# nomic-ai/contrastors

Measured on AMD Instinct MI355X. Metric: query-doc pairs/sec (whole node), nomic-bert-2048 seq128 global-batch 16384, higher is better.
Workload: dtype bf16

## Files before the change

contrastors_amd/_C.py:

```python
from __future__ import annotations

import ctypes as C
import os
from pathlib import Path

_PKG = Path(__file__).resolve().parent
LIB_PATH = Path(os.environ.get("CONTRASTORS_HIP_LIB", _PKG / "lib" / "libcontrastors_hip.so"))

CX_OK = 0
_ERR = {-1: "CX_ERR_SHAPE", -2: "CX_ERR_ALIGN", -3: "CX_ERR_ARG", -4: "CX_ERR_LAUNCH"}

vp = C.c_void_p
i32 = C.c_int
i64 = C.c_long
f32 = C.c_float
u64 = C.c_ulonglong
u32 = C.c_uint


class CxLayerWeights(C.Structure):
    _fields_ = (
        [(n, vp) for n in ("Wqkv", "Wout", "Wfc1", "Wfc2", "WqkvT", "WoutT", "Wfc1T", "Wfc2T")]
        + [(n, vp) for n in ("bqkv", "bout", "bfc1", "bfc2")]
        + [(n, vp) for n in ("ln1_g", "ln1_b", "ln2_g", "ln2_b")]
        + [(n, vp) for n in ("gWqkv", "gWout", "gWfc1", "gWfc2")]
        + [(n, vp) for n in ("gbqkv", "gbout", "gbfc1", "gbfc2")]
        + [(n, vp) for n in ("gln1_g", "gln1_b", "gln2_g", "gln2_b")]
    )


class CxEncoderDesc(C.Structure):
    _fields_ = [
        ("n_layer", i32), ("d", i32), ("n_head", i32), ("d_inner", i32), ("gated", i32),
        ("vocab", i32), ("max_pos", i32), ("padding_idx", i32),
        ("ln_eps", f32), ("softmax_scale", f32),
        ("word_emb", vp), ("type_emb", vp), ("pos_emb", vp),
        ("emb_ln_g", vp), ("emb_ln_b", vp),
        ("gword_emb", vp), ("gtype_emb", vp), ("gpos_emb", vp), ("gemb_ln_g", vp), ("gemb_ln_b", vp),
        ("rot_cos", vp), ("rot_sin", vp),
        ("layers", C.POINTER(CxLayerWeights)),
        ("pool_mode", i32), ("normalize", i32),
        ("prenorm", i32),
        ("lnf_g", vp), ("lnf_b", vp), ("glnf_g", vp), ("glnf_b", vp),
        ("Wpatch", vp), ("bpatch", vp), ("cls_token", vp), ("vit_pos", vp),
        ("gWpatch", vp), ("gbpatch", vp), ("gcls_token", vp), ("gvit_pos", vp),
        ("patch_dim", i32),
        ("resid_pdrop", f32), ("embd_pdrop", f32), ("attn_pdrop", f32),
        ("mlp_act", i32), ("lnpre_g", vp), ("lnpre_b", vp), ("glnpre_g", vp), ("glnpre_b", vp),
    ]


class CxChunkBuffers(C.Structure):
    _fields_ = [("T_cap", i64)] + [
        (n, vp)
        for n in (
            "h0", "emb_mean", "emb_rstd", "qkv", "ctx", "lse", "z1", "h1", "mean1", "rstd1", "yg", "act", "z2",
            "h2", "mean2", "rstd2", "pool_norm", "g_a", "g_b", "g_c", "g_wide", "g_act", "tr_a", "tr_b", "delta",
            "ws_f32",
        )
    ] + [("ws_floats", i64)] + [(n, vp) for n in ("zf", "hf", "meanf", "rstdf", "patch_in", "patch_proj")] + [("checkpoint", i32), ("drop_active", i32), ("drop_seed", C.c_ulonglong), ("drop_offset", C.c_ulonglong), ("g_d", vp), ("layer_events", C.POINTER(vp)), ("zpre", vp), ("ckpt_keep", i32), ("patch_keep", vp), ("patch_inv", vp), ("n_keep", i32), ("n_patch_all", i32)]



class CxVitSubLN(C.Structure):
    _fields_ = [(n, vp) for n in ("norm_g", "norm_b", "gnorm_g", "gnorm_b")]


class CxVitExt(C.Structure):
    _fields_ = [("rope_cos", vp), ("rope_sin", vp), ("n_rope", i32), ("n_prefix", i32), ("no_final_ln", i32),
                ("subln_eps", f32), ("sub_ln", C.POINTER(CxVitSubLN)), ("z", vp), ("zmean", vp), ("zrstd", vp),
                ("yg_wide", vp)]


_SIGS = {
    "cx_abi_version": (i32, []),
    "cx_build_info": (C.c_char_p, []),
    "cx_error_string": (C.c_char_p, [i32]),
    "cx_gemm_bf16_nt": (i32, [vp, vp, vp, vp, i32, i32, i32, i32, i32, i32, i32, i32, f32, vp]),
    "cx_gemm_bf16_nt_accum": (i32, [vp, vp, vp, vp, i64, i32, i32, i32, i32, i32, vp]),
    "cx_gemm_bf16_tn_accum": (i32, [vp, vp, vp, vp, i64, i32, i32, i32, i32, i32, vp]),
    "cx_prof_gemm_config": (i32, [i32, i32]),
    "cx_prof_gemm_collect": (i32, [C.POINTER(C.c_double), C.POINTER(C.c_double), C.POINTER(i64), C.POINTER(i64)]),
    "cx_calib_mfma_bf16": (i32, [vp, i32, i32, vp, vp, vp]),
    "cx_calib_copy": (i32, [vp, vp, i64, vp]),
    "cx_transpose_bf16": (i32, [vp, vp, i32, i32, i32, i32, i32, vp]),
    "cx_cast_f32_to_bf16": (i32, [vp, vp, i64, vp]),
    "cx_cast_transpose_f32_to_bf16": (i32, [vp, vp, i32, i32, vp]),
    "cx_cast_transpose_f32_to_bf16_batched": (i32, [vp, i32, i32, vp]),
    "cx_cast_bf16_to_f32": (i32, [vp, vp, i64, vp]),
    "cx_layernorm_fwd": (i32, [vp, vp, vp, vp, vp, vp, vp, vp, i32, i32, f32, vp]),
    "cx_layernorm_bwd": (i32, [vp, vp, vp, vp, vp, vp, vp, vp, vp, vp, vp, i64, i32, i32, vp]),
    "cx_layernorm_bwd_pooled": (i32, [vp, vp, vp, vp, i32, i32, i32, vp, vp, vp, vp, vp, vp, vp, vp, vp, i64, i32, i32, vp]),
    "cx_layernorm_bwd_colsum": (i32, [vp, vp, vp, vp, vp, vp, vp, vp, vp, vp, vp, vp, i64, i32, i32, vp]),
    "cx_dropout_add_layernorm_fwd": (i32, [vp, vp, vp, vp, vp, vp, vp, vp, i32, i32, f32, f32, C.c_ulonglong, C.c_ulonglong,
                                           C.c_uint, vp]),
    "cx_dropout_add_layernorm_bwd": (i32, [vp, vp, vp, vp, vp, vp, vp, vp, vp, vp, vp, i64, i32, i32, f32, C.c_ulonglong,
                                           C.c_ulonglong, C.c_uint, vp]),
    "cx_dropout_add_layernorm_bwd_colsum": (i32, [vp, vp, vp, vp, vp, vp, vp, vp, vp, vp, vp, vp, i64, i32, i32, f32, C.c_ulonglong,
                                                  C.c_ulonglong, C.c_uint, vp]),
    "cx_dropout_scale": (i32, [vp, i64, f32, C.c_ulonglong, C.c_ulonglong, C.c_uint, vp]),
    "cx_layernorm_fwd_mixed": (i32, [vp, vp, vp, vp, vp, vp, vp, vp, i32, i32, f32, i32, vp]),
    "cx_layernorm_bwd_mixed": (i32, [vp, vp, vp, vp, vp, vp, vp, vp, vp, vp, i32, i32, i32, vp]),
    "cx_embed_ln_fwd": (i32, [vp, vp, vp, vp, vp, vp, vp, vp, vp, vp, i32, i32, i32, f32, vp]),
    "cx_embed_ln_bwd": (i32, [vp] * 15 + [i32, i32, i32, i32, vp]),
    "cx_embed_ln_bwd_sorted": (i32, [vp] * 15 + [i32, i32, i32, i32, i32, vp, vp, vp, vp]),
    "cx_swiglu_fwd": (i32, [vp, vp, i32, i32, i32, vp]),
    "cx_swiglu_bwd": (i32, [vp, vp, vp, i32, i32, i32, vp]),
    "cx_gemm_bf16_swiglu": (i32, [vp, vp, vp, vp, i32, i32, i32, i32, i32, i32, i32, vp]),
    "cx_gemm_bf16_nt_residual": (i32, [vp, vp, vp, vp, vp, i32, i32, i32, i32, i32, i32, i32, vp]),
    "cx_gemm_bf16_swiglu_bwd": (i32, [vp, vp, vp, vp, i32, i32, i32, i32, i32, i32, vp]),
    "cx_gemm_bf16_nt_splitk": (i32, [vp, vp, vp, vp, vp, vp, i64, i32, i32, i32, i32, i32, i32, i32, vp]),
    "cx_gemm_bf16_swiglu_gate": (i32, [vp, vp, vp, vp, i32, i32, i32, i32, i32, i32, i32, vp]),
    "cx_gemm_bf16_swiglu_bwd_gate": (i32, [vp, vp, vp, vp, vp, i32, i32, i32, i32, i32, i32, i32, vp]),
    "cx_swiglu_bwd_gate": (i32, [vp, vp, vp, vp, i32, i32, vp]),
    "cx_gemm_bf16_bias_gelu": (i32, [vp, vp, vp, vp, vp, i32, i32, i32, i32, i32, i32, i32, vp]),
    "cx_gemm_bf16_bias_act": (i32, [vp, vp, vp, vp, vp, i32, i32, i32, i32, i32, i32, i32, i32, vp]),
    "cx_bias_gelu_fwd": (i32, [vp, vp, vp, i32, i32, vp]),
    "cx_bias_gelu_bwd": (i32, [vp, vp, vp, vp, i32, i32, vp]),
    "cx_bias_grad": (i32, [vp, vp, i32, i32, i32, vp]),
    "cx_bias_gelu_bwd_colsum": (i32, [vp, vp, vp, vp, vp, i32, i32, vp]),
    "cx_bias_act_fwd": (i32, [vp, vp, vp, i32, i32, i32, vp]),
    "cx_bias_act_bwd_colsum": (i32, [vp, vp, vp, vp, vp, i32, i32, i32, vp]),
    "cx_gemm_bf16_act_bwd": (i32, [vp, vp, vp, vp, vp, vp, i64, i32, i32, i32, i32, i32, i32, i32, i32, vp]),
    "cx_attn_varlen_fwd": (i32, [vp, vp, vp, vp, vp, vp, i32, i32, i32, i32, f32, vp]),
    "cx_attn_varlen_bwd": (i32, [vp] * 9 + [i32, i32, i32, i32, f32, vp]),
    "cx_attn_varlen_bwd_prerotated": (i32, [vp] * 9 + [i32, i32, i32, i32, f32, vp]),
    "cx_attn_varlen_dropout_fwd": (i32, [vp] * 6 + [i32, i32, i32, i32, f32, f32, u64, u64, u32, vp]),
    "cx_attn_varlen_dropout_bwd": (i32, [vp] * 9 + [i32, i32, i32, i32, f32, f32, u64, u64, u32, vp]),
    "cx_ipc_alloc": (i32, [C.POINTER(vp), i64, i32]),
    "cx_ipc_free": (i32, [vp]),
    "cx_ipc_export": (i32, [vp, vp]),
    "cx_ipc_open": (i32, [vp, C.POINTER(vp)]),
    "cx_ipc_close": (i32, [vp]),
    "cx_xgmi_push": (i32, [vp, vp, i64, i64, i32, vp]),
    "cx_xgmi_scatter": (i32, [vp, vp, i32, i64, i32, vp]),
    "cx_xgmi_signal_wait": (i32, [vp, vp, i32, i32, u32, i64, vp, vp]),
    "cx_sum_slots_f32": (i32, [vp, vp, i64, i32, vp]),
    "cx_attn_varlen_kvpacked_fwd": (i32, [vp] * 6 + [i32, i32, i32, i32, i32, f32, vp]),
    "cx_attn_varlen_kvpacked_bwd": (i32, [vp] * 10 + [i32, i32, i32, i32, i32, f32, vp]),
    "cx_rotary_qkv_inplace": (i32, [vp, vp, vp, vp, i32, i32, i32, i32, i32, vp]),
    "cx_rotary_apply": (i32, [vp, i64, vp, vp, vp, i32, i32, i32, i32, i32, vp]),
    "cx_pool_normalize_fwd": (i32, [vp, vp, vp, vp, i32, i32, i32, i32, vp]),
    "cx_pool_normalize_bwd": (i32, [vp, vp, vp, vp, vp, i32, i32, i32, i32, vp]),
    "cx_vit_patchify": (i32, [vp, i32, vp, i32, i32, i32, i32, i32, vp]),
    "cx_vit_assemble_fwd": (i32, [vp, vp, vp, vp, i32, i32, i32, vp]),
    "cx_vit_assemble_bwd": (i32, [vp, vp, vp, vp, i32, i32, i32, vp]),
    "cx_vit_patchify_gather": (i32, [vp, i32, vp, i32, i32, i32, i32, i32, vp, i32, vp]),
    "cx_vit_assemble_fwd_gather": (i32, [vp, vp, vp, vp, i32, i32, i32, vp, vp]),
    "cx_vit_assemble_bwd_gather": (i32, [vp, vp, vp, vp, i32, i32, i32, vp, i32, vp]),
    "cx_vit_forward": (i32, [C.POINTER(CxEncoderDesc), C.POINTER(CxChunkBuffers), vp, i32, vp, i32, i32, i32, i32, i32,
                             i32, vp, vp]),
    "cx_vit_backward": (i32, [C.POINTER(CxEncoderDesc), C.POINTER(CxChunkBuffers), vp, i32, i32, vp, vp, vp]),
    "cx_vit_forward_hidden": (i32, [C.POINTER(CxEncoderDesc), C.POINTER(CxChunkBuffers), vp, i32, vp, i32, i32, i32, i32, i32,
                                    i32, vp, vp]),
    "cx_vit_backward_hidden": (i32, [C.POINTER(CxEncoderDesc), C.POINTER(CxChunkBuffers), vp, i32, i32, vp, vp]),
    "cx_rope2d_qkv_inplace": (i32, [vp, vp, vp, vp, i32, i32, i32, i32, i32, i32, vp]),
    "cx_swiglu_subln_fwd": (i32, [vp, vp, vp, vp, vp, vp, vp, vp, i32, i32, f32, vp]),
    "cx_swiglu_subln_bwd": (i32, [vp] * 11 + [i64, i32, i32, vp]),
    "cx_vit_forward_ex": (i32, [C.POINTER(CxEncoderDesc), C.POINTER(CxChunkBuffers), C.POINTER(CxVitExt), vp, i32, vp, i32, i32,
                                i32, i32, i32, i32, vp, vp]),
    "cx_vit_backward_ex": (i32, [C.POINTER(CxEncoderDesc), C.POINTER(CxChunkBuffers), C.POINTER(CxVitExt), vp, i32, i32, vp, vp,
                                 vp]),
    "cx_vit_forward_hidden_ex": (i32, [C.POINTER(CxEncoderDesc), C.POINTER(CxChunkBuffers), C.POINTER(CxVitExt), vp, i32, vp, i32,
                                       i32, i32, i32, i32, i32, vp, vp]),
    "cx_vit_backward_hidden_ex": (i32, [C.POINTER(CxEncoderDesc), C.POINTER(CxChunkBuffers), C.POINTER(CxVitExt), vp, i32, i32,
                                        vp, vp]),
    "cx_xent_fwd": (i32, [vp, i32, vp, vp, vp, i32, i32, i64, f32, i64, vp]),
    "cx_xent_bwd": (i32, [vp, vp, i32, vp, vp, vp, i32, i32, i64, i64, f32, i64, vp]),
    "cx_grad_sq_norm": (i32, [vp, i64, vp, vp]),
    "cx_adamw_clip_step": (i32, [vp, vp, vp, vp, i64, f32, f32, f32, f32, f32, i64, vp, f32, vp]),
    "cx_ema_update": (i32, [vp, vp, i64, f32, vp]),
    "cx_infonce_ws_floats": (i64, [i32, i32]),
    "cx_infonce_fwd": (i32, [vp, vp, vp, f32, vp, vp, vp, i32, i32, i32, i32, i32, vp]),
    "cx_infonce_argmax_ws_floats": (i64, [i32, i32]),
    "cx_infonce_fwd_argmax": (i32, [vp, vp, vp, f32, vp, vp, vp, vp, i32, i32, i32, i32, i32, vp]),
    "cx_infonce_bwd": (i32, [vp, vp, vp, vp, f32, f32, vp, vp, vp, vp, vp, vp, vp, i32, i32, i32, i32, i32, vp]),
    "cx_search_ws_bytes": (i64, [i32, i64, i32, i32]),
    "cx_search_topk": (i32, [vp, vp, i32, i64, i32, i64, i64, i32, vp, vp, vp, i32, vp, vp, vp, vp]),
    "cx_infonce_fp8_ws_floats": (i64, [i32, i32]),
    "cx_infonce_fp8_fwd": (i32, [vp, vp, vp, f32, vp, vp, vp, vp, vp, vp, vp, i32, i32, i32, i32, i32, vp]),
    "cx_infonce_fp8_bwd": (i32, [vp, vp, vp, vp, f32, f32, vp, vp, vp, vp, vp, vp, vp, vp, vp, i64, vp, vp, vp, i32, i32, i32,
                                 i32, i32, vp]),
    "cx_sgemm_nt": (i32, [vp, vp, vp, i32, i32, i32, i32, i32, i32, vp]),
    "cx_transpose_f32": (i32, [vp, vp, i32, i32, i32, i32, vp]),
    "cx_encoder_forward": (i32, [C.POINTER(CxEncoderDesc), C.POINTER(CxChunkBuffers), vp, vp, vp, i32, i32, i32,
                                 i32, i32, vp, vp]),
    "cx_encoder_forward_hidden": (i32, [C.POINTER(CxEncoderDesc), C.POINTER(CxChunkBuffers), vp, vp, vp, i32, i32, i32,
                                        i32, i32, vp, vp]),
    "cx_encoder_backward_hidden": (i32, [C.POINTER(CxEncoderDesc), C.POINTER(CxChunkBuffers), vp, vp, vp, i32, i32, i32,
                                         i32, vp, vp, vp, vp]),
    "cx_encoder_backward": (i32, [C.POINTER(CxEncoderDesc), C.POINTER(CxChunkBuffers), vp, vp, vp, i32, i32, i32,
                                  i32, vp, vp, vp, vp, vp]),
}

_DEV_SIGS = {
    "cx_gemm_set_variant": (None, [i32]),
    "cx_gemm_get_variant": (i32, []),
    "cx_gemm_set_debug": (None, [i32]),
    "cx_gemm_set_trace": (None, [vp]),
    "cx_gemm_v6_ablate": (None, [i32]),
    "cx_gemm_v6_trace": (None, [vp]),
    "cx_gemm_v7_mode": (None, [i32]),
    "cx_gemm_v7_trace": (None, [vp]),
    "cx_gemm_v7_occupancy": (i32, []),
    "cx_gemm_v7_ablate": (None, [i32]),
    "cx_gemm_v7_flags": (None, [i32]),
    "cx_gemm_v7_period": (None, [i32]),
    "cx_gemm_set_glds": (None, [i32]),
    "cx_gemm_get_glds": (i32, []),
    "cx_attn_set_bwd_s128": (None, [i32]),
    "cx_attn_set_prio": (None, [i32]),
    "cx_attn_set_fwd_s128": (None, [i32]),
    "cx_attn_set_fwd_long": (None, [i32]),
    "cx_attn_set_bwd_long": (None, [i32]),
    "cx_probe_mfma_layout": (i32, [vp, vp]),
    "cx_probe_ds_read_tr16": (i32, [vp, vp, vp]),
    "cx_probe_mfma_rate": (i32, [vp, i32, i32, i32, vp, vp, vp]),
    "cx_attn_dropout_keep_mask": (i32, [vp, i32, i32, i32, f32, u64, u64, u32, vp]),
    "cx_probe_rmw": (i32, [vp, i64, i32, i32, i32, vp]),
    "cx_probe_mfma_rate16": (i32, [vp, i32, i32, i32, vp, vp, vp]),
    "cx_probe_dma_bw": (i32, [vp, i64, i64, i64, i32, i32, i32, i32, vp, vp]),
}

EXPORTED_SYMBOLS = tuple(_SIGS)
DEV_EXPORTED_SYMBOLS = tuple(_DEV_SIGS)
DEV_LIB_PATH = Path(os.environ.get("CONTRASTORS_HIP_DEV_LIB", _PKG / "lib" / "libcontrastors_hip_dev.so"))

_lib = None
_dev_lib = None


def lib() -> C.CDLL:
    global _lib
    if _lib is None:
        if not LIB_PATH.exists():
            raise ImportError(
                f"{LIB_PATH} not found: build it with `python -m contrastors_amd.build` "
                "(hipcc --offload-arch=gfx950).  There is no CPU fallback."
            )
        import torch

        h = C.CDLL(str(LIB_PATH))
        for name, (res, args) in _SIGS.items():
            fn = getattr(h, name)
            fn.restype = res
            fn.argtypes = args
        _lib = h
    return _lib


def dev_lib() -> C.CDLL:
    global _dev_lib
    if _dev_lib is None:
        if not DEV_LIB_PATH.exists():
            raise ImportError(f"{DEV_LIB_PATH} not found: build it with `python -m contrastors_amd.build`")
        import torch

        h = C.CDLL(str(DEV_LIB_PATH))
        for name, (res, args) in {**_SIGS, **_DEV_SIGS}.items():
            fn = getattr(h, name)
            fn.restype = res
            fn.argtypes = args
# ... 18 lines not shown
```

contrastors_amd/csrc/engine.hip:

```cpp
#include <hip/hip_runtime.h>
#include "../../include/contrastors_hip.h"

namespace {

#define CX_TRY(expr)              \
    do {                          \
        int rc__ = (expr);        \
        if (rc__ != CX_OK) return rc__; \
    } while (0)

inline long round_up(long v, long m) { return (v + m - 1) / m * m; }

inline int mark_grads_done(const CxChunkBuffers* buf, int idx, void* stream) {
    if (!buf->layer_events || !buf->layer_events[idx]) return CX_OK;
    return hipEventRecord((hipEvent_t)buf->layer_events[idx], (hipStream_t)stream) == hipSuccess ? CX_OK : CX_ERR_LAUNCH;
}

struct Slots {
    const CxChunkBuffers* b;
    const CxEncoderDesc* e;
    long T_cap;
    int d, I, wfc1;
    int mode;
    int first_kept;
    bool kept(int s) const { return mode == 1 || (mode == 2 && s >= first_kept); }
    int sl(int s) const { return mode == 1 ? s : (mode == 2 && s >= first_kept) ? 1 + s - first_kept : 0; }
    int sl_in(int s) const { return mode == 0 ? 0 : s; }
    uint16_t* qkv(int s) const { return b->qkv + (size_t)sl(s) * T_cap * 3 * d; }
    uint16_t* ctx(int s) const { return b->ctx + (size_t)sl(s) * T_cap * d; }
    float* lse(int s) const { return b->lse + (size_t)sl(s) * T_cap * e->n_head; }
    uint16_t* z1(int s) const { return b->z1 + (size_t)(e->prenorm ? sl_in(s) : sl(s)) * T_cap * d; }
    uint16_t* h1(int s) const { return b->h1 + (size_t)sl(s) * T_cap * d; }
    float* mean1(int s) const { return b->mean1 + (size_t)sl(s) * T_cap; }
    float* rstd1(int s) const { return b->rstd1 + (size_t)sl(s) * T_cap; }
    uint16_t* yg(int s) const { return b->yg + (size_t)sl(s) * T_cap * I; }
    uint16_t* act(int s) const { return b->act + (size_t)sl(s) * T_cap * I; }
    uint16_t* z2(int s) const { return b->z2 + (size_t)sl(s) * T_cap * d; }
    uint16_t* h2(int s) const { return b->h2 + (size_t)(e->prenorm ? sl(s) : sl_in(s)) * T_cap * d; }
    float* mean2(int s) const { return b->mean2 + (size_t)sl(s) * T_cap; }
    float* rstd2(int s) const { return b->rstd2 + (size_t)sl(s) * T_cap; }
    uint16_t* ez(const CxVitExt* x, int s) const { return x->z + (size_t)sl(s) * T_cap * I; }
    float* ezmean(const CxVitExt* x, int s) const { return x->zmean + (size_t)sl(s) * T_cap; }
    float* ezrstd(const CxVitExt* x, int s) const { return x->zrstd + (size_t)sl(s) * T_cap; }
};

inline bool ext_rope(const CxVitExt* x) { return x && x->rope_cos; }
inline bool ext_subln(const CxVitExt* x) { return x && x->sub_ln; }
inline bool ext_no_lnf(const CxVitExt* x) { return x && x->no_final_ln; }
int check_ext(const CxVitExt* x, const CxEncoderDesc* e, const CxChunkBuffers* b) {
    if (!x) return CX_OK;
    if (x->rope_cos && (!x->rope_sin || x->n_rope <= 0 || x->n_prefix < 0)) return CX_ERR_ARG;
    if (x->sub_ln) {
        if (!e->gated || !x->z || !x->zmean || !x->zrstd || (!x->yg_wide && !b->g_wide)) return CX_ERR_ARG;
        for (int l = 0; l < e->n_layer; ++l)
            if (!x->sub_ln[l].norm_g || !x->sub_ln[l].norm_b) return CX_ERR_ARG;
    }
    return CX_OK;
}

Slots make_slots(const CxEncoderDesc* enc, const CxChunkBuffers* buf, int save) {
    const int L = enc->n_layer;
    int keep = buf->ckpt_keep < 0 ? 0 : buf->ckpt_keep > L ? L : buf->ckpt_keep;
    return Slots{buf, enc, buf->T_cap, enc->d, enc->d_inner, enc->gated ? 2 * enc->d_inner : enc->d_inner,
                 save ? (buf->checkpoint ? 2 : 1) : 0, L - keep};
}

int check_desc(const CxEncoderDesc* e, const CxChunkBuffers* b, int T) {
    if (!e || !b || !e->layers) return CX_ERR_ARG;
    if (e->n_layer <= 0 || e->d <= 0 || e->n_head <= 0) return CX_ERR_ARG;
    if (e->d != e->n_head * 64) return CX_ERR_SHAPE;
    if ((e->d % 64) != 0 || (e->d_inner % 64) != 0) return CX_ERR_SHAPE;
    if (b->T_cap < round_up(T, 64)) return CX_ERR_SHAPE;
    return CX_OK;
}

int wgrad_split(int out_f, int in_f, long Tp) {
    const long tiles = (long)((out_f + 127) / 128) * ((in_f + 127) / 128);
    const long nk = Tp / 64;
    long s = (512 + tiles - 1) / tiles;
    if (s > nk / 2) s = nk / 2;
    if (s < 1) s = 1;
    return (int)s;
}

int wgrad(const uint16_t* dY, int out_f, const uint16_t* X, int in_f, float* gW, const CxChunkBuffers* b, int T,
          void* stream) {
    if (!gW) return CX_OK;
    const int rc = cx_gemm_bf16_tn_accum(dY, X, gW, b->ws_f32, b->ws_floats, T, out_f, in_f, out_f, in_f, stream);
    if (rc != CX_ERR_SHAPE) return rc;
    if (!b->tr_a || !b->tr_b) return CX_ERR_ARG;
    const int Tp = (int)round_up(T, 64);
    CX_TRY(cx_transpose_bf16(dY, b->tr_a, T, out_f, out_f, Tp, Tp, stream));
    CX_TRY(cx_transpose_bf16(X, b->tr_b, T, in_f, in_f, Tp, Tp, stream));
    return cx_gemm_bf16_nt_accum(b->tr_a, b->tr_b, gW, b->ws_f32, b->ws_floats, out_f, in_f, Tp, Tp, Tp, stream);
}

int proj_residual(const uint16_t* x, const uint16_t* W, const float* bias, const uint16_t* residual, uint16_t* out, int T,
                  int N, int K, bool* folded, void* stream, const CxChunkBuffers* buf = nullptr) {
    *folded = false;
    if (buf && buf->ws_f32 && (long)((T + 255) / 256) * ((N + 255) / 256) <= 64 && K >= 1536) {
        const int rc = cx_gemm_bf16_nt_splitk(x, W, out, bias, residual, buf->ws_f32, buf->ws_floats, T, N, K, K, K, N, N, stream);
        if (rc != CX_ERR_SHAPE) {
            *folded = residual != nullptr && rc == CX_OK;
            return rc;
        }
    }
    if (residual) {
        const int rc = cx_gemm_bf16_nt_residual(x, W, out, bias, residual, T, N, K, K, K, N, N, stream);
        if (rc != CX_ERR_SHAPE) {
            *folded = rc == CX_OK;
            return rc;
        }
    }
    return cx_gemm_bf16_nt(x, W, out, bias, T, N, K, K, K, N, 0, 1, 1.f, stream);
}

bool gelu_fused_shape(int T, int N, int K) {
    return T > 0 && (K % 64) == 0 && (N % 8) == 0;
}

struct BlockRunner {
    const CxEncoderDesc* enc;
    const CxChunkBuffers* buf;
    const Slots& s;
    const int32_t* cu_seqlens;
    int Bc, T, max_seqlen;
    void* stream;
    const CxVitExt* ext = nullptr;

    int mlp_up(const CxLayerWeights& w, const uint16_t* x, int l, bool keep) const {
        const int d = enc->d, I = enc->d_inner;
        if (ext_subln(ext)) {
            uint16_t* yg = ext->yg_wide ? ext->yg_wide : buf->g_wide;
            CX_TRY(cx_gemm_bf16_nt(x, w.Wfc1, yg, w.bfc1, T, 2 * I, d, d, d, 2 * I, 0, 1, 1.f, stream));
            const CxVitSubLN& n = ext->sub_ln[l];
            return cx_swiglu_subln_fwd(yg, n.norm_g, n.norm_b, keep ? s.yg(l) : nullptr, s.act(l), s.ez(ext, l), s.ezmean(ext, l),
                                       s.ezrstd(ext, l), T, I, ext->subln_eps, stream);
        }
        if (enc->gated) {
            return cx_gemm_bf16_swiglu_gate(x, w.Wfc1, keep ? s.yg(l) : nullptr, s.act(l), T, I, d, d, d, I, I, stream);
        }
        const int rc = cx_gemm_bf16_bias_act(x, w.Wfc1, w.bfc1, keep ? s.yg(l) : nullptr, s.act(l), T, s.wfc1, d, d, d, s.wfc1,
                                             I, enc->mlp_act, stream);
        if (rc != CX_ERR_SHAPE) return rc;
        CX_TRY(cx_gemm_bf16_nt(x, w.Wfc1, s.yg(l), nullptr, T, s.wfc1, d, d, d, s.wfc1, 0, 1, 1.f, stream));
        return cx_bias_act_fwd(s.yg(l), w.bfc1, s.act(l), T, I, enc->mlp_act, stream);
    }
    int mlp(const CxLayerWeights& w, const uint16_t* x, int l, uint16_t* out, const uint16_t* residual, bool keep,
            bool* folded) const {
        CX_TRY(mlp_up(w, x, l, keep));
        return proj_residual(ext_subln(ext) ? s.ez(ext, l) : s.act(l), w.Wfc2, w.bfc2, residual, out, T, enc->d, enc->d_inner, folded, stream, buf);
    }
    int attn(const CxLayerWeights& w, const uint16_t* x, int l, uint16_t* out, const uint16_t* residual, bool* folded) const {
        const int d = enc->d;
        CX_TRY(cx_gemm_bf16_nt(x, w.Wqkv, s.qkv(l), w.bqkv, T, 3 * d, d, d, d, 3 * d, 0, 1, 1.f, stream));
        if (ext_rope(ext))
            CX_TRY(cx_rope2d_qkv_inplace(s.qkv(l), cu_seqlens, ext->rope_cos, ext->rope_sin, ext->n_rope, Bc, enc->n_head, T,
                                         ext->n_prefix, 1, stream));
        if (buf->drop_active && enc->attn_pdrop > 0.f) {
            CX_TRY(cx_attn_varlen_dropout_fwd(s.qkv(l), cu_seqlens, enc->rot_cos, enc->rot_sin, s.ctx(l), s.lse(l), Bc,
                                              enc->n_head, T, max_seqlen, enc->softmax_scale, enc->attn_pdrop, buf->drop_seed,
                                              buf->drop_offset, (unsigned)(2 * enc->n_layer + 1 + l), stream));
        } else if (enc->rot_cos && max_seqlen > 128) {
            CX_TRY(cx_rotary_qkv_inplace(s.qkv(l), cu_seqlens, enc->rot_cos, enc->rot_sin, Bc, enc->n_head, T, max_seqlen, 1,
                                         stream));
            CX_TRY(cx_attn_varlen_fwd(s.qkv(l), cu_seqlens, nullptr, nullptr, s.ctx(l), s.lse(l), Bc, enc->n_head, T, max_seqlen,
                                      enc->softmax_scale, stream));
        } else {
            CX_TRY(cx_attn_varlen_fwd(s.qkv(l), cu_seqlens, enc->rot_cos, enc->rot_sin, s.ctx(l), s.lse(l), Bc, enc->n_head, T,
                                      max_seqlen, enc->softmax_scale, stream));
        }
        return proj_residual(s.ctx(l), w.Wout, w.bout, residual, out, T, d, d, folded, stream);
    }
    int post_block(int l, const uint16_t* h_in, bool keep) const {
        const CxLayerWeights& w = enc->layers[l];
        const int d = enc->d;
        bool f1 = false, f2 = false;
        if (drop()) {
            const float p = enc->resid_pdrop;
            CX_TRY(attn(w, h_in, l, s.z1(l), nullptr, &f1));
            CX_TRY(cx_dropout_add_layernorm_fwd(s.z1(l), h_in, w.ln1_g, w.ln1_b, s.h1(l), keep ? s.z1(l) : nullptr, s.mean1(l),
                                                s.rstd1(l), T, d, enc->ln_eps, p, buf->drop_seed, buf->drop_offset, 2 * l, stream));
            CX_TRY(mlp(w, s.h1(l), l, s.z2(l), nullptr, keep, &f2));
            return cx_dropout_add_layernorm_fwd(s.z2(l), s.h1(l), w.ln2_g, w.ln2_b, s.h2(l), keep ? s.z2(l) : nullptr, s.mean2(l),
                                                s.rstd2(l), T, d, enc->ln_eps, p, buf->drop_seed, buf->drop_offset, 2 * l + 1,
                                                stream);
        }
        CX_TRY(attn(w, h_in, l, s.z1(l), h_in, &f1));
        CX_TRY(cx_layernorm_fwd(s.z1(l), f1 ? nullptr : h_in, w.ln1_g, w.ln1_b, s.h1(l), (keep && !f1) ? s.z1(l) : nullptr,
                                s.mean1(l), s.rstd1(l), T, d, enc->ln_eps, stream));
        CX_TRY(mlp(w, s.h1(l), l, s.z2(l), s.h1(l), keep, &f2));
        return cx_layernorm_fwd(s.z2(l), f2 ? nullptr : s.h1(l), w.ln2_g, w.ln2_b, s.h2(l), (keep && !f2) ? s.z2(l) : nullptr,
                                s.mean2(l), s.rstd2(l), T, d, enc->ln_eps, stream);
    }
    bool drop() const { return buf->drop_active && enc->resid_pdrop > 0.f; }
    int pre_block(int l, const uint16_t* x, const uint16_t* r, bool r_folded, bool keep, bool up_only, const uint16_t** x_out,
                  const uint16_t** r_out, bool* folded_out) const {
        const CxLayerWeights& w = enc->layers[l];
        const int d = enc->d, L = enc->n_layer;
        CX_TRY(cx_layernorm_fwd(x, r, w.ln1_g, w.ln1_b, s.h1(l), (r_folded && x == s.z1(l)) ? nullptr : s.z1(l), s.mean1(l),
                                s.rstd1(l), T, d, enc->ln_eps, stream));
        bool f1 = false, f2 = false;
        CX_TRY(attn(w, s.h1(l), l, s.z2(l), s.z1(l), &f1));
        CX_TRY(cx_layernorm_fwd(s.z2(l), f1 ? nullptr : s.z1(l), w.ln2_g, w.ln2_b, s.h2(l), f1 ? nullptr : s.z2(l), s.mean2(l),
                                s.rstd2(l), T, d, enc->ln_eps, stream));
        if (up_only) return mlp_up(w, s.h2(l), l, keep);
        uint16_t* nxt = (l + 1 < L) ? s.z1(l + 1) : buf->zf;
        CX_TRY(mlp(w, s.h2(l), l, nxt, s.z2(l), keep, &f2));
        *x_out = nxt;
        *r_out = f2 ? nullptr : s.z2(l);
        *folded_out = f2;
        return CX_OK;
    }
};

int blocks_forward(const CxEncoderDesc* enc, const CxChunkBuffers* buf, const Slots& s, const uint16_t* h0,
                   const int32_t* cu_seqlens, int Bc, int T, int max_seqlen, int save, const uint16_t** h_final,
                   void* stream, const CxVitExt* ext = nullptr) {
    const int d = enc->d, L = enc->n_layer;
    const BlockRunner run{enc, buf, s, cu_seqlens, Bc, T, max_seqlen, stream, ext};
    if (!enc->prenorm) {
        const uint16_t* h_in = h0;
        for (int l = 0; l < L; ++l) {
            CX_TRY(run.post_block(l, h_in, save != 0 && s.kept(l)));
            h_in = s.h2(l);
        }
        *h_final = h_in;
        return CX_OK;
    }
    if (!buf->zf || !buf->hf || !buf->meanf || !buf->rstdf || (!ext_no_lnf(ext) && (!enc->lnf_g || !enc->lnf_b))) return CX_ERR_ARG;
    if (buf->drop_active && enc->resid_pdrop > 0.f) return CX_ERR_ARG;
    const uint16_t* x = h0;
    const uint16_t* r = nullptr;
    bool r_folded = false;
    for (int l = 0; l < L; ++l) {
        CX_TRY(run.pre_block(l, x, r, r_folded, save != 0 && s.kept(l), false, &x, &r, &r_folded));
        if (save == 2 && !r_folded) return CX_ERR_SHAPE;
    }
    if (ext_no_lnf(ext)) {
        if (!r_folded || x != buf->zf) return CX_ERR_SHAPE;
        *h_final = buf->zf;
        return CX_OK;
    }
    CX_TRY(cx_layernorm_fwd(x, r, enc->lnf_g, enc->lnf_b, buf->hf, r_folded ? nullptr : buf->zf, buf->meanf, buf->rstdf, T,
                            d, enc->ln_eps, stream));
    *h_final = buf->hf;
    return CX_OK;
}

int check_bwd_buffers(const CxChunkBuffers* buf) {
    return (!buf->g_a || !buf->g_b || !buf->g_c || !buf->g_wide || !buf->g_act || !buf->delta ||
            !buf->ws_f32) ? CX_ERR_ARG : CX_OK;
}

int clear_pad_rows(const CxEncoderDesc* enc, const CxChunkBuffers* buf, const Slots& s, int T, void* stream,
                   const CxVitExt* ext = nullptr) {
    const int Tp = (int)round_up(T, 64);
    if (Tp == T) return CX_OK;
    const int d = enc->d, I = enc->d_inner, L = enc->n_layer;
    auto clear = [&](uint16_t* base, int width) {
        return hipMemsetAsync(base + (size_t)T * width, 0, (size_t)(Tp - T) * width * sizeof(uint16_t),
                              (hipStream_t)stream) == hipSuccess ? CX_OK : CX_ERR_LAUNCH;
    };
    CX_TRY(clear(buf->g_a, d));
    CX_TRY(clear(buf->g_b, d));
    CX_TRY(clear(buf->g_c, d));
    if (buf->g_d) CX_TRY(clear(buf->g_d, d));
    CX_TRY(clear(buf->g_wide, 3 * d));
    CX_TRY(clear(buf->g_wide, s.wfc1));
    CX_TRY(clear(buf->h0, d));
    for (int l = 0; l < L; ++l) {
        CX_TRY(clear(s.act(l), I));
        CX_TRY(clear(s.h1(l), d));
        CX_TRY(clear(s.ctx(l), d));
        CX_TRY(clear(s.h2(l), d));
        if (ext_subln(ext)) CX_TRY(clear(s.ez(ext, l), I));
    }
    return CX_OK;
}

struct PooledGrad {
    const float* demb;
    const float* emb;
    const float* norm;
    int pool_mode, normalize;
};

int blocks_backward(const CxEncoderDesc* enc, const CxChunkBuffers* buf, const Slots& s, const int32_t* cu_seqlens, int Bc,
                    int T, int max_seqlen, const PooledGrad* pg, const uint16_t** da_out, const uint16_t** db_out, void* stream,
                    const CxVitExt* ext = nullptr) {
    const int d = enc->d, I = enc->d_inner, H = enc->n_head, L = enc->n_layer;
    auto mlp_bwd = [&](const CxLayerWeights& w, int l, const uint16_t* dm, const uint16_t* mlp_in, const uint16_t* add,
                       bool* folded, bool bias_done) -> int {
        if (w.gbfc2 && !bias_done) CX_TRY(cx_bias_grad(dm, w.gbfc2, T, d, d, stream));
        if (ext_subln(ext)) {
            CX_TRY(wgrad(dm, d, s.ez(ext, l), I, w.gWfc2, buf, T, stream));
            CX_TRY(cx_gemm_bf16_nt(dm, w.Wfc2T, buf->g_act, nullptr, T, I, d, d, d, I, 0, 1, 1.f, stream));
            const CxVitSubLN& n = ext->sub_ln[l];
            CX_TRY(cx_swiglu_subln_bwd(buf->g_act, s.act(l), s.yg(l), s.ezmean(ext, l), s.ezrstd(ext, l), n.norm_g, buf->g_wide,
                                       n.gnorm_g, n.gnorm_b, w.gbfc1, buf->ws_f32, buf->ws_floats, T, I, stream));
            CX_TRY(wgrad(buf->g_wide, s.wfc1, mlp_in, d, w.gWfc1, buf, T, stream));
            return proj_residual(buf->g_wide, w.Wfc1T, nullptr, add, buf->g_b, T, d, s.wfc1, folded, stream, buf);
        }
        CX_TRY(wgrad(dm, d, s.act(l), I, w.gWfc2, buf, T, stream));
        int fused = CX_ERR_SHAPE;
        if (enc->gated)
            fused = cx_gemm_bf16_swiglu_bwd_gate(dm, w.Wfc2T, s.act(l), s.yg(l), buf->g_wide, T, I, d, d, d, I, s.wfc1, stream);
#ifndef CX_AB_R5_ROUTES
        if (!enc->gated && gelu_fused_shape(T, s.wfc1, d))
            fused = cx_gemm_bf16_act_bwd(dm, w.Wfc2T, s.yg(l), buf->g_wide, w.gbfc1, buf->ws_f32, buf->ws_floats, T, I, d, d, d, I, I,
                                         enc->mlp_act, stream);
#endif
        if (fused != CX_ERR_SHAPE) {
            CX_TRY(fused);
        } else {
            CX_TRY(cx_gemm_bf16_nt(dm, w.Wfc2T, buf->g_act, nullptr, T, I, d, d, d, I, 0, 1, 1.f, stream));
        }
        if (enc->gated) {
            if (fused == CX_ERR_SHAPE)
                CX_TRY(cx_swiglu_bwd_gate(buf->g_act, s.act(l), s.yg(l), buf->g_wide, T, I, stream));
        } else if (fused == CX_ERR_SHAPE) {
            CX_TRY(cx_bias_act_bwd_colsum(buf->g_act, s.yg(l), gelu_fused_shape(T, s.wfc1, d) ? nullptr : w.bfc1, buf->g_wide,
                                          w.gbfc1, T, I, enc->mlp_act, stream));
        }
        CX_TRY(wgrad(buf->g_wide, s.wfc1, mlp_in, d, w.gWfc1, buf, T, stream));
        return proj_residual(buf->g_wide, w.Wfc1T, nullptr, add, buf->g_b, T, d, s.wfc1, folded, stream, buf);
    };
    auto attn_bwd = [&](const CxLayerWeights& w, int l, const uint16_t* dx, const uint16_t* attn_in, const uint16_t* add,
                        bool* folded, bool bias_done) -> int {
        if (w.gbout && !bias_done) CX_TRY(cx_bias_grad(dx, w.gbout, T, d, d, stream));
        CX_TRY(wgrad(dx, d, s.ctx(l), d, w.gWout, buf, T, stream));
        CX_TRY(cx_gemm_bf16_nt(dx, w.WoutT, buf->g_b, nullptr, T, d, d, d, d, d, 0, 1, 1.f, stream));
        if (buf->drop_active && enc->attn_pdrop > 0.f) {
            CX_TRY(cx_attn_varlen_dropout_bwd(buf->g_b, s.qkv(l), s.ctx(l), s.lse(l), cu_seqlens, enc->rot_cos, enc->rot_sin,
                                              buf->delta, buf->g_wide, Bc, H, T, max_seqlen, enc->softmax_scale, enc->attn_pdrop,
                                              buf->drop_seed, buf->drop_offset, (unsigned)(2 * enc->n_layer + 1 + l), stream));
        } else if (enc->rot_cos && max_seqlen > 128) {
            CX_TRY(cx_attn_varlen_bwd_prerotated(buf->g_b, s.qkv(l), s.ctx(l), s.lse(l), cu_seqlens, enc->rot_cos, enc->rot_sin,
                                                 buf->delta, buf->g_wide, Bc, H, T, max_seqlen, enc->softmax_scale, stream));
        } else {
            CX_TRY(cx_attn_varlen_bwd(buf->g_b, s.qkv(l), s.ctx(l), s.lse(l), cu_seqlens, enc->rot_cos, enc->rot_sin,
                                      buf->delta, buf->g_wide, Bc, H, T, max_seqlen, enc->softmax_scale, stream));
        }
        if (ext_rope(ext))
            CX_TRY(cx_rope2d_qkv_inplace(buf->g_wide, cu_seqlens, ext->rope_cos, ext->rope_sin, ext->n_rope, Bc, H, T, ext->n_prefix,
                                         -1, stream));
        if (w.gbqkv) CX_TRY(cx_bias_grad(buf->g_wide, w.gbqkv, T, 3 * d, 3 * d, stream));
        CX_TRY(wgrad(buf->g_wide, 3 * d, attn_in, d, w.gWqkv, buf, T, stream));
        return proj_residual(buf->g_wide, w.WqkvT, nullptr, add, buf->g_b, T, d, 3 * d, folded, stream, buf);
    };
    auto ln_bwd = [&](const uint16_t* a, const uint16_t* b2, const uint16_t* z, const float* g, const float* mean,
                      const float* rstd, const uint16_t* dz_extra, uint16_t* dz, float* gg, float* gb, float* gbias,
                      bool* done) -> int {
        *done = false;
        if (gbias) {
            const int rc = cx_layernorm_bwd_colsum(a, b2, z, g, mean, rstd, dz_extra, dz, gg, gb, gbias, buf->ws_f32,
                                                   buf->ws_floats, T, d, stream);
            if (rc != CX_ERR_ARG) {
                *done = rc == CX_OK;
                return rc;
            }
        }
        return cx_layernorm_bwd(a, b2, z, g, mean, rstd, dz_extra, dz, gg, gb, buf->ws_f32, buf->ws_floats, T, d, stream);
    };
    const BlockRunner run{enc, buf, s, cu_seqlens, Bc, T, max_seqlen, stream, ext};
    if (!enc->prenorm) {
        const uint16_t* da = buf->g_a;
        const uint16_t* db = nullptr;
        for (int l = L - 1; l >= 0; --l) {
            const CxLayerWeights& w = enc->layers[l];
            const uint16_t* h_in = (l == 0) ? buf->h0 : s.h2(l - 1);
            if (!s.kept(l)) CX_TRY(run.post_block(l, h_in, true));
            if (run.drop()) {
                if (!buf->g_d) return CX_ERR_ARG;
                const float p = enc->resid_pdrop;
                bool f1 = false, f2 = false;
#ifdef CX_AB_R5_ROUTES
                const bool cs = false;
#else
                const bool cs = buf->ws_f32 && buf->ws_floats >= 3L * d * 256;
#endif
                CX_TRY(cx_dropout_add_layernorm_bwd_colsum(da, db, s.z2(l), w.ln2_g, s.mean2(l), s.rstd2(l), buf->g_c, buf->g_d, w.gln2_g,
                                                           w.gln2_b, cs ? w.gbfc2 : nullptr, buf->ws_f32, buf->ws_floats, T, d, p,
                                                           buf->drop_seed, buf->drop_offset, 2 * l + 1, stream));
                CX_TRY(mlp_bwd(w, l, buf->g_d, s.h1(l), buf->g_c, &f1, cs));
                CX_TRY(cx_dropout_add_layernorm_bwd_colsum(f1 ? buf->g_b : buf->g_c, f1 ? nullptr : buf->g_b, s.z1(l), w.ln1_g, s.mean1(l),
                                                           s.rstd1(l), buf->g_a, buf->g_d, w.gln1_g, w.gln1_b, cs ? w.gbout : nullptr,
                                                           buf->ws_f32, buf->ws_floats, T, d, p, buf->drop_seed, buf->drop_offset, 2 * l,
                                                           stream));
// ... 350 lines not shown
```

contrastors_amd/csrc/gemm_api.hip:

```cpp
#include "cx_common.h"
#include "../../include/contrastors_hip.h"
#include "gemm_params.h"
#include <mutex>

namespace {

constexpr int BK = 64;

__global__ __launch_bounds__(256) void splitk_reduce_kernel(const float* __restrict__ part, float* __restrict__ out, long n4,
                                                            long slab, int splits) {
    const long stride = (long)gridDim.x * blockDim.x;
    for (long i = (long)blockIdx.x * blockDim.x + threadIdx.x; i < n4; i += stride) {
        float4 a = reinterpret_cast<const float4*>(out)[i];
        for (int s = 0; s < splits; ++s) {
            const float4 v = reinterpret_cast<const float4*>(part + s * slab)[i];
            a.x += v.x; a.y += v.y; a.z += v.z; a.w += v.w;
        }
        reinterpret_cast<float4*>(out)[i] = a;
    }
}

int reduce_slabs(const float* ws, float* out, long slab, int split, hipStream_t s) {
    const long n4 = slab / 4;
    long g = (n4 + 255) / 256;
// ... 13 lines not shown
        if (score > best_score + 1e-9) {
            best_score = score;
            best = s;
        }
    }
    return best;
}

struct GemmProf {
    std::mutex mu;
    bool enabled = false;
    int stride = 1;
    long launches = 0;
    static constexpr int CAP = 8192;
    hipEvent_t ev0[CAP], ev1[CAP];
    double flop[CAP];
    int created = 0, used = 0;
} g_prof;

struct ProfScope {
    int slot = -1;
    hipStream_t s;
    ProfScope(double flop, hipStream_t stream) : s(stream) {
        if (!g_prof.enabled) return;
        std::lock_guard<std::mutex> lk(g_prof.mu);
        if ((g_prof.launches % g_prof.stride) == 0 && g_prof.used < GemmProf::CAP) {
            const int sl = g_prof.used;
            if (sl >= g_prof.created) {
                if (hipEventCreate(&g_prof.ev0[sl]) != hipSuccess || hipEventCreate(&g_prof.ev1[sl]) != hipSuccess) return;
                g_prof.created = sl + 1;
            }
            slot = g_prof.used++;
            g_prof.flop[slot] = flop;
            (void)hipEventRecord(g_prof.ev0[slot], s);
        }
        ++g_prof.launches;
    }
    ~ProfScope() {
        if (slot >= 0) (void)hipEventRecord(g_prof.ev1[slot], s);
    }
};

GemmParams base_params(const uint16_t* X, const uint16_t* W, void* Out, const float* bias, int M, int N, int K, int ldx,
                       int ldw, int ldo) {
    GemmParams p = {};
    p.X = X; p.W = W; p.Out = Out; p.bias = bias;
    p.M = M; p.N = N; p.K = K; p.ldx = ldx; p.ldw = ldw; p.ldo = ldo;
    p.split_k = 1; p.alpha = 1.f;
    return p;
}

}

extern "C" {

int cx_gemm_bf16_nt(const uint16_t* X, const uint16_t* W, void* Out, const float* bias, int M, int N, int K, int ldx,
                    int ldw, int ldo, int out_mode, int split_k, float alpha, void* stream) {
    if (M <= 0 || N <= 0) return CX_OK;
    if (K <= 0 || (K % BK) != 0 || (N % 4) != 0) return CX_ERR_SHAPE;
    if ((ldx % 8) != 0 || (ldw % 8) != 0 || (ldo % 4) != 0) return CX_ERR_ALIGN;
    if (out_mode < 0 || out_mode > 1) return CX_ERR_ARG;
    (void)split_k;
    GemmParams p = base_params(X, W, Out, bias, M, N, K, ldx, ldw, ldo);
    p.alpha = alpha;
    ProfScope prof(2.0 * (double)M * (double)N * (double)K, (hipStream_t)stream);
    hipError_t e;
    if (out_mode == 0 && (N % 8) == 0 && (ldo % 8) == 0)
        e = cx_launch_gemm_v6(p, GEMM_EPI_NONE, (hipStream_t)stream);
    else
        e = cx_launch_gemm_v5(p, 0, out_mode == 0 ? GEMM_OUT_BF16 : GEMM_OUT_F32, GEMM_EPI_NONE, (hipStream_t)stream);
    return e == hipSuccess ? CX_OK : CX_ERR_LAUNCH;
}

int cx_gemm_bf16_nt_accum(const uint16_t* X, const uint16_t* W, float* Out, float* ws, long ws_floats, int M, int N, int K,
                          int ldx, int ldw, void* stream) {
    if (M <= 0 || N <= 0) return CX_OK;
    if (K <= 0 || (K % BK) != 0 || (N % 4) != 0) return CX_ERR_SHAPE;
    if ((ldx % 8) != 0 || (ldw % 8) != 0) return CX_ERR_ALIGN;
    if (!ws || !Out) return CX_ERR_ARG;
    const long slab = (long)M * N;
    if (ws_floats < slab) return CX_ERR_SHAPE;
    const long tiles = (long)((M + 255) / 256) * ((N + 255) / 256), nk = K / BK;
    long max_split = nk / 4;
    if (max_split > ws_floats / slab) max_split = ws_floats / slab;
    if (max_split > 16) max_split = 16;
    GemmParams p = base_params(X, W, ws, nullptr, M, N, K, ldx, ldw, N);
    p.split_k = (int)choose_split(tiles, max_split);
    if (p.split_k > nk) p.split_k = (int)nk;
    if (cx_launch_gemm_v5(p, 0, GEMM_OUT_F32_PARTIAL, GEMM_EPI_NONE, (hipStream_t)stream) != hipSuccess) return CX_ERR_LAUNCH;
    return reduce_slabs(ws, Out, slab, p.split_k, (hipStream_t)stream);
}

int cx_gemm_bf16_tn_accum(const uint16_t* dY, const uint16_t* A, float* G, float* ws, long ws_floats, int T, int O, int I,
                          int ld_dy, int ld_a, void* stream) {
    if (T <= 0 || O <= 0 || I <= 0) return CX_OK;
    if ((O % 256) != 0 || (I % 256) != 0) return CX_ERR_SHAPE;
    if ((ld_dy % 8) != 0 || (ld_a % 8) != 0) return CX_ERR_ALIGN;
    if (!ws || !G) return CX_ERR_ARG;
    const long slab = (long)O * I;
    if (ws_floats < slab) return CX_ERR_SHAPE;
    const int Tp = (T + BK - 1) / BK * BK;
    GemmParams p = base_params(dY, A, ws, nullptr, O, I, Tp, ld_dy, ld_a, I);
    const long tiles = (long)(O / 256) * (I / 256), nk = Tp / BK;
    long max_split = nk / 4;
    if (max_split > ws_floats / slab) max_split = ws_floats / slab;
    if (max_split > 32) max_split = 32;
    p.split_k = (int)choose_split(tiles, max_split);
    {
        ProfScope prof(2.0 * (double)T * (double)O * (double)I, (hipStream_t)stream);
        if (cx_launch_gemm_v6_tn(p, (hipStream_t)stream) != hipSuccess) return CX_ERR_LAUNCH;
    }
    return reduce_slabs(ws, G, slab, p.split_k, (hipStream_t)stream);
}

int cx_gemm_bf16_swiglu(const uint16_t* X, const uint16_t* W, uint16_t* YG, uint16_t* Act, int M, int I, int K, int ldx,
                        int ldw, int ld_yg, int ld_act, void* stream) {
    if (M <= 0 || I <= 0) return CX_OK;
    if (K <= 0 || (K % BK) != 0 || (I % 32) != 0) return CX_ERR_SHAPE;
    if ((ldx % 8) != 0 || (ldw % 8) != 0 || (ld_yg % 4) != 0 || (ld_act % 4) != 0) return CX_ERR_ALIGN;
    if (!Act) return CX_ERR_ARG;
    GemmParams p = base_params(X, W, YG, nullptr, M, 2 * I, K, ldx, ldw, ld_yg);
    p.Out2 = Act; p.ldo2 = ld_act;
    ProfScope prof(2.0 * (double)M * (double)(2 * I) * (double)K, (hipStream_t)stream);
    const hipError_t e = ((ld_yg % 8) == 0 && (ld_act % 8) == 0)
                             ? cx_launch_gemm_v6(p, GEMM_EPI_SWIGLU, (hipStream_t)stream)
                             : cx_launch_gemm_v5(p, 0, GEMM_OUT_BF16, GEMM_EPI_SWIGLU, (hipStream_t)stream);
    return e == hipSuccess ? CX_OK : CX_ERR_LAUNCH;
}

int cx_gemm_bf16_swiglu_gate(const uint16_t* X, const uint16_t* W, uint16_t* G, uint16_t* Act, int M, int I, int K, int ldx,
                             int ldw, int ld_g, int ld_act, void* stream) {
    if (M <= 0 || I <= 0) return CX_OK;
    if (K <= 0 || (K % BK) != 0 || (I % 32) != 0 || (ld_g % 8) != 0 || (ld_act % 8) != 0) return CX_ERR_SHAPE;
    if ((ldx % 8) != 0 || (ldw % 8) != 0) return CX_ERR_ALIGN;
    if (!Act) return CX_ERR_ARG;
    GemmParams p = base_params(X, W, G, nullptr, M, 2 * I, K, ldx, ldw, ld_g);
    p.Out2 = Act; p.ldo2 = ld_act;
    ProfScope prof(2.0 * (double)M * (double)(2 * I) * (double)K, (hipStream_t)stream);
    return cx_launch_gemm_v6(p, GEMM_EPI_SWIGLU_G, (hipStream_t)stream) == hipSuccess ? CX_OK : CX_ERR_LAUNCH;
}

int cx_gemm_bf16_nt_residual(const uint16_t* X, const uint16_t* W, uint16_t* Out, const float* bias, const uint16_t* Residual,
                             int M, int N, int K, int ldx, int ldw, int ldo, int ldr, void* stream) {
    if (M <= 0 || N <= 0) return CX_OK;
    if (!Residual || !Out) return CX_ERR_ARG;
    if (K <= 0 || (K % 64) != 0 || (N % 8) != 0 || (ldo % 8) != 0 || (ldr % 8) != 0) return CX_ERR_SHAPE;
    if ((ldx % 8) != 0 || (ldw % 8) != 0) return CX_ERR_ALIGN;
    GemmParams p = base_params(X, W, Out, bias, M, N, K, ldx, ldw, ldo);
    p.Out2 = const_cast<uint16_t*>(Residual); p.ldo2 = ldr;
    ProfScope prof(2.0 * (double)M * (double)N * (double)K, (hipStream_t)stream);
    return cx_launch_gemm_v6(p, GEMM_EPI_NONE, (hipStream_t)stream) == hipSuccess ? CX_OK : CX_ERR_LAUNCH;
}

int cx_gemm_bf16_bias_gelu(const uint16_t* X, const uint16_t* W, const float* bias, uint16_t* Pre, uint16_t* Act, int M, int N,
                           int K, int ldx, int ldw, int ld_pre, int ld_act, void* stream) {
    return cx_gemm_bf16_bias_act(X, W, bias, Pre, Act, M, N, K, ldx, ldw, ld_pre, ld_act, 0, stream);
}

int cx_gemm_bf16_bias_act(const uint16_t* X, const uint16_t* W, const float* bias, uint16_t* Pre, uint16_t* Act, int M, int N,
                          int K, int ldx, int ldw, int ld_pre, int ld_act, int act, void* stream) {
    if (M <= 0 || N <= 0) return CX_OK;
    if (!Act || (act != 0 && act != 1)) return CX_ERR_ARG;
    if (K <= 0 || (K % 64) != 0 || (N % 8) != 0 || (ld_act % 8) != 0 || (Pre && (ld_pre % 8) != 0)) return CX_ERR_SHAPE;
    if ((ldx % 8) != 0 || (ldw % 8) != 0) return CX_ERR_ALIGN;
    GemmParams p = base_params(X, W, Pre, bias, M, N, K, ldx, ldw, ld_pre);
    p.Out2 = Act; p.ldo2 = ld_act;
    p.act = act;
    ProfScope prof(2.0 * (double)M * (double)N * (double)K, (hipStream_t)stream);
    return cx_launch_gemm_v6(p, act == 1 ? GEMM_EPI_QGELU : GEMM_EPI_GELU, (hipStream_t)stream) == hipSuccess ? CX_OK : CX_ERR_LAUNCH;
}

int cx_gemm_bf16_swiglu_bwd(const uint16_t* dY, const uint16_t* W, const uint16_t* YG, uint16_t* dYG, int M, int I, int K,
                            int ldx, int ldw, int ld_yg, void* stream) {
    if (M <= 0 || I <= 0) return CX_OK;
    if (!dY || !W || !YG || !dYG) return CX_ERR_ARG;
    if (K <= 0 || (K % 64) != 0 || (I % 256) != 0 || (ld_yg % 8) != 0 || ld_yg < 2 * I) return CX_ERR_SHAPE;
    if ((ldx % 8) != 0 || (ldw % 8) != 0) return CX_ERR_ALIGN;
    GemmParams p = base_params(dY, W, dYG, nullptr, M, I, K, ldx, ldw, ld_yg);
    p.Out2 = const_cast<uint16_t*>(YG); p.ldo2 = ld_yg;
    ProfScope prof(2.0 * (double)M * (double)I * (double)K, (hipStream_t)stream);
    return cx_launch_gemm_v6(p, GEMM_EPI_SWIGLU_BWD, (hipStream_t)stream) == hipSuccess ? CX_OK : CX_ERR_LAUNCH;
}

int cx_gemm_bf16_swiglu_bwd_gate(const uint16_t* dY, const uint16_t* W, const uint16_t* Act, const uint16_t* G, uint16_t* dYG,
                                 int M, int I, int K, int ldx, int ldw, int ld_ag, int ld_dyg, void* stream) {
    if (M <= 0 || I <= 0) return CX_OK;
    if (!dY || !W || !Act || !G || !dYG) return CX_ERR_ARG;
    if (K <= 0 || (K % 64) != 0 || (I % 256) != 0 || (ld_dyg % 8) != 0 || ld_dyg < 2 * I || (ld_ag % 8) != 0 || ld_ag < I)
        return CX_ERR_SHAPE;
    if ((ldx % 8) != 0 || (ldw % 8) != 0) return CX_ERR_ALIGN;
    GemmParams p = base_params(dY, W, dYG, nullptr, M, I, K, ldx, ldw, ld_dyg);
    p.Out2 = const_cast<uint16_t*>(Act); p.ldo2 = ld_ag;
    p.In3 = G;
    ProfScope prof(2.0 * (double)M * (double)I * (double)K, (hipStream_t)stream);
    return cx_launch_gemm_v6(p, GEMM_EPI_SWIGLU_BWD_AG, (hipStream_t)stream) == hipSuccess ? CX_OK : CX_ERR_LAUNCH;
}

int cx_gemm_bf16_act_bwd(const uint16_t* dY, const uint16_t* W, const uint16_t* Pre, uint16_t* dPre, float* dbias, float* ws,
                         long ws_floats, int M, int N, int K, int ldx, int ldw, int ld_pre, int ld_dpre, int act, void* stream) {
    if (M <= 0 || N <= 0) return CX_OK;
    if (!dY || !W || !Pre || !dPre || (act != 0 && act != 1)) return CX_ERR_ARG;
    if (K <= 0 || (K % 64) != 0 || (N % 8) != 0 || (ld_pre % 8) != 0 || (ld_dpre % 8) != 0) return CX_ERR_SHAPE;
    if ((ldx % 8) != 0 || (ldw % 8) != 0) return CX_ERR_ALIGN;
    const int nblocks = (M + 127) / 128;
    if (dbias && (!ws || ws_floats < (long)nblocks * N)) return CX_ERR_SHAPE;
    GemmParams p = base_params(dY, W, dPre, nullptr, M, N, K, ldx, ldw, ld_dpre);
    p.Out2 = const_cast<uint16_t*>(Pre); p.ldo2 = ld_pre;
    p.act = act;
    p.colsum_part = dbias ? ws : nullptr;
    {
        ProfScope prof(2.0 * (double)M * (double)N * (double)K, (hipStream_t)stream);
        if (cx_launch_gemm_v6(p, GEMM_EPI_ACT_BWD, (hipStream_t)stream) != hipSuccess) return CX_ERR_LAUNCH;
    }
    if (dbias && cx_launch_colsum_part_reduce(ws, dbias, nblocks, N, (hipStream_t)stream) != hipSuccess) return CX_ERR_LAUNCH;
    return CX_OK;
}

int cx_prof_gemm_config(int enable, int stride) {
    std::lock_guard<std::mutex> lk(g_prof.mu);
    g_prof.enabled = enable != 0;
    g_prof.stride = stride > 0 ? stride : 1;
    g_prof.launches = 0;
    g_prof.used = 0;
    return CX_OK;
}

int cx_prof_gemm_collect(double* total_ms, double* total_flop, long* launches_timed, long* launches_total) {
    std::lock_guard<std::mutex> lk(g_prof.mu);
    double ms = 0.0, fl = 0.0;
    for (int i = 0; i < g_prof.used; ++i) {
        if (hipEventSynchronize(g_prof.ev1[i]) != hipSuccess) return CX_ERR_LAUNCH;
        float t = 0.f;
        if (hipEventElapsedTime(&t, g_prof.ev0[i], g_prof.ev1[i]) != hipSuccess) return CX_ERR_LAUNCH;
        ms += t;
        fl += g_prof.flop[i];
    }
    if (total_ms) *total_ms = ms;
    if (total_flop) *total_flop = fl;
    if (launches_timed) *launches_timed = g_prof.used;
    if (launches_total) *launches_total = g_prof.launches;
    return CX_OK;
}

}

#include "gemm_splitk_small.inc"
```

contrastors_amd/csrc/gemm_bf16.hip:

```cpp
#include "cx_common.h"
#include "../../include/contrastors_hip.h"
#include "gemm_params.h"

namespace {

constexpr int BM = 128, BN = 128, BK = 64;
constexpr int TILE_BYTES = 128 * BK * 2;

typedef __attribute__((address_space(3))) void* lds_void_ptr;
typedef const __attribute__((address_space(1))) void* glb_void_ptr;

enum OutMode { OUT_BF16 = GEMM_OUT_BF16, OUT_F32 = GEMM_OUT_F32, OUT_F32_ATOMIC = GEMM_OUT_F32_ATOMIC };

struct StageRegs { uint4 r0, r1, r2, r3; };

CX_DEVICE uint4 stage_load(const bf16_t* __restrict__ base, int ld, int row0, int nrows, int k0, int tid, int p) {
    const int r = p * 32 + (tid >> 3);
    int gr = row0 + r;
    gr = gr < nrows ? gr : nrows - 1;
    return *reinterpret_cast<const uint4*>(base + (size_t)gr * ld + k0 + (tid & 7) * 8);
}

template <bool GLDS>
CX_DEVICE void stage_tile(const bf16_t* __restrict__ base, int ld, int row0, int nrows, int k0, char* lds_tile,
// ... 613 lines not shown
                if (hipEventCreate(&g_prof.ev0[slot]) != hipSuccess || hipEventCreate(&g_prof.ev1[slot]) != hipSuccess)
                    return CX_ERR_LAUNCH;
                g_prof.created = slot + 1;
            }
            g_prof.flop[slot] = 2.0 * (double)M * (double)N * (double)K;
            (void)hipEventRecord(g_prof.ev0[slot], (hipStream_t)stream);
        }
        ++g_prof.launches;
    }
    hipError_t e = v5 ? cx_launch_gemm_v5(p, 0, out_mode, GEMM_EPI_NONE, (hipStream_t)stream)
                   : v2 ? launch_v2(p, out_mode, (hipStream_t)stream)
                      : (g_use_glds ? launch_mode<true>(p, out_mode, (hipStream_t)stream)
                                    : launch_mode<false>(p, out_mode, (hipStream_t)stream));
    if (slot >= 0) (void)hipEventRecord(g_prof.ev1[slot], (hipStream_t)stream);
    return e == hipSuccess ? CX_OK : CX_ERR_LAUNCH;
}

int cx_gemm_bf16_nt_accum(const uint16_t* X, const uint16_t* W, float* Out, float* ws, long ws_floats, int M, int N,
                          int K, int ldx, int ldw, void* stream) {
    if (M <= 0 || N <= 0) return CX_OK;
    if (K <= 0 || (K % BK) != 0 || (N % 4) != 0) return CX_ERR_SHAPE;
    if (!ws || !Out) return CX_ERR_ARG;
    const long slab = (long)M * N;
    if (ws_floats < slab) return CX_ERR_SHAPE;
    const bool v5 = (g_variant >= 3) && g_use_glds;
    const bool v2 = (g_variant == 2) && g_use_glds;
    const long tiles = v5 ? (long)((M + 255) / 256) * ((N + 255) / 256)
                     : v2 ? (long)((M + V2_BM - 1) / V2_BM) * ((N + V2_BN - 1) / V2_BN)
                          : (long)((M + BM - 1) / BM) * ((N + BN - 1) / BN);
    const long nk = K / BK;
    long max_split = nk / 4;
    if (max_split > ws_floats / slab) max_split = ws_floats / slab;
    if (max_split > 16) max_split = 16;
    long split = choose_split(tiles, max_split, (v2 || v5) ? 256 : 512);
    int rc;
    if (v5) {
        GemmParams p;
        p.X = X; p.W = W; p.Out = ws; p.bias = nullptr;
        p.M = M; p.N = N; p.K = K; p.ldx = ldx; p.ldw = ldw; p.ldo = N;
        p.tiles_m = p.tiles_n = 0; p.split_k = (int)split; p.alpha = 1.f; p.dbg = g_dbg; p.Out2 = nullptr; p.ldo2 = 0; p.sup_m = p.sup_n = 0;
        split = p.split_k;
        const hipError_t he = cx_launch_gemm_v5(p, 0, GEMM_OUT_F32_PARTIAL, GEMM_EPI_NONE, (hipStream_t)stream);
        rc = he == hipSuccess ? CX_OK : CX_ERR_LAUNCH;
    } else if (v2) {
        GemmParams p;
        p.X = X; p.W = W; p.Out = ws; p.bias = nullptr;
        p.M = M; p.N = N; p.K = K; p.ldx = ldx; p.ldw = ldw; p.ldo = N;
        p.tiles_m = (M + V2_BM - 1) / V2_BM; p.tiles_n = (N + V2_BN - 1) / V2_BN;
        p.split_k = (int)split; p.alpha = 1.f; p.dbg = g_dbg; p.Out2 = nullptr; p.ldo2 = 0; p.sup_m = p.sup_n = 0;
        rc = launch_v2(p, OUT_F32_PARTIAL, (hipStream_t)stream) == hipSuccess ? CX_OK : CX_ERR_LAUNCH;
    } else {
        rc = CX_OK;
        for (long s = 0; s < split && rc == CX_OK; ++s) {
            const long k0 = nk * s / split * BK, k1 = nk * (s + 1) / split * BK;
            rc = cx_gemm_bf16_nt(X + k0, W + k0, ws + s * slab, nullptr, M, N, (int)(k1 - k0), ldx, ldw, N, OUT_F32, 1,
                                 1.f, stream);
        }
    }
    if (rc != CX_OK) return rc;
    const long n4 = slab / 4;
    long g = (n4 + 255) / 256;
    if (g > 2048) g = 2048;
    hipLaunchKernelGGL(splitk_reduce_kernel, dim3((int)g), dim3(256), 0, (hipStream_t)stream, ws, Out, n4, slab,
                       (int)split);
    return hipGetLastError() == hipSuccess ? CX_OK : CX_ERR_LAUNCH;
}

int cx_gemm_bf16_tn_accum(const uint16_t* dY, const uint16_t* A, float* G, float* ws, long ws_floats, int T, int O, int I,
                          int ld_dy, int ld_a, void* stream) {
    if (T <= 0 || O <= 0 || I <= 0) return CX_OK;
    if ((O % V2_BM) != 0 || (I % V2_BN) != 0) return CX_ERR_SHAPE;
    const bool use_v5 = (g_variant == 5) && (I % 256) == 0;
    if ((ld_dy % 8) != 0 || (ld_a % 8) != 0) return CX_ERR_ALIGN;
    if (!ws || !G) return CX_ERR_ARG;
    const long slab = (long)O * I;
    if (ws_floats < slab) return CX_ERR_SHAPE;
    const int Tp = (T + BK - 1) / BK * BK;
    GemmParams p;
    p.X = dY; p.W = A; p.Out = ws; p.bias = nullptr;
    p.M = O; p.N = I; p.K = Tp; p.ldx = ld_dy; p.ldw = ld_a; p.ldo = I;
    p.tiles_m = O / V2_BM; p.tiles_n = use_v5 ? I / 256 : I / V2_BN;
    const long tiles = (long)p.tiles_m * p.tiles_n, nk = Tp / BK;
    long max_split = nk / 4;
    if (max_split > ws_floats / slab) max_split = ws_floats / slab;
    if (max_split > 32) max_split = 32;
    const long split = choose_split(tiles, max_split);
    p.split_k = (int)split; p.alpha = 1.f; p.dbg = g_dbg; p.Out2 = nullptr; p.ldo2 = 0; p.sup_m = p.sup_n = 0;
    static bool attr_set = false;
    if (!attr_set) {
        if (hipFuncSetAttribute(reinterpret_cast<const void*>(&gemm_bf16_tn_kernel),
                                hipFuncAttributeMaxDynamicSharedMemorySize, V2_NSTAGE * V2_STAGE) != hipSuccess)
            return CX_ERR_LAUNCH;
        attr_set = true;
    }
    int slot = -1;
    if (g_prof.enabled) {
        if ((g_prof.launches % g_prof.stride) == 0 && g_prof.used < GemmProf::CAP) {
            slot = g_prof.used++;
            if (slot >= g_prof.created) {
                if (hipEventCreate(&g_prof.ev0[slot]) != hipSuccess || hipEventCreate(&g_prof.ev1[slot]) != hipSuccess)
                    return CX_ERR_LAUNCH;
                g_prof.created = slot + 1;
            }
            g_prof.flop[slot] = 2.0 * (double)T * (double)O * (double)I;
            (void)hipEventRecord(g_prof.ev0[slot], (hipStream_t)stream);
        }
        ++g_prof.launches;
    }
    if (use_v5) {
        if (cx_launch_gemm_v5(p, 1, GEMM_OUT_F32_PARTIAL, GEMM_EPI_NONE, (hipStream_t)stream) != hipSuccess) return CX_ERR_LAUNCH;
    } else {
        hipLaunchKernelGGL(gemm_bf16_tn_kernel, dim3((int)(tiles * split)), dim3(512), V2_NSTAGE * V2_STAGE,
                           (hipStream_t)stream, p);
    }
    if (slot >= 0) (void)hipEventRecord(g_prof.ev1[slot], (hipStream_t)stream);
    if (hipGetLastError() != hipSuccess) return CX_ERR_LAUNCH;
    const long n4 = slab / 4;
    long g = (n4 + 255) / 256;
    if (g > 2048) g = 2048;
    hipLaunchKernelGGL(splitk_reduce_kernel, dim3((int)g), dim3(256), 0, (hipStream_t)stream, ws, G, n4, slab, (int)split);
    return hipGetLastError() == hipSuccess ? CX_OK : CX_ERR_LAUNCH;
}

int cx_gemm_bf16_swiglu(const uint16_t* X, const uint16_t* W, uint16_t* YG, uint16_t* Act, int M, int I, int K, int ldx,
                        int ldw, int ld_yg, int ld_act, void* stream) {
    if (M <= 0 || I <= 0) return CX_OK;
    if (K <= 0 || (K % BK) != 0 || (I % 32) != 0) return CX_ERR_SHAPE;
    if ((ldx % 8) != 0 || (ldw % 8) != 0 || (ld_yg % 4) != 0 || (ld_act % 4) != 0) return CX_ERR_ALIGN;
    if (!Act) return CX_ERR_ARG;
    GemmParams p;
    p.X = X; p.W = W; p.Out = YG; p.bias = nullptr;
    p.M = M; p.N = 2 * I; p.K = K; p.ldx = ldx; p.ldw = ldw; p.ldo = ld_yg;
    p.tiles_m = p.tiles_n = 0; p.split_k = 1; p.alpha = 1.f; p.dbg = g_dbg;
    p.Out2 = Act; p.ldo2 = ld_act; p.sup_m = p.sup_n = 0;
    int slot = -1;
    if (g_prof.enabled) {
        if ((g_prof.launches % g_prof.stride) == 0 && g_prof.used < GemmProf::CAP) {
            slot = g_prof.used++;
            if (slot >= g_prof.created) {
                if (hipEventCreate(&g_prof.ev0[slot]) != hipSuccess || hipEventCreate(&g_prof.ev1[slot]) != hipSuccess)
                    return CX_ERR_LAUNCH;
                g_prof.created = slot + 1;
            }
            g_prof.flop[slot] = 2.0 * (double)M * (double)(2 * I) * (double)K;
            (void)hipEventRecord(g_prof.ev0[slot], (hipStream_t)stream);
        }
        ++g_prof.launches;
    }
    hipError_t e = cx_launch_gemm_v5(p, 0, GEMM_OUT_BF16, GEMM_EPI_SWIGLU, (hipStream_t)stream);
    if (slot >= 0) (void)hipEventRecord(g_prof.ev1[slot], (hipStream_t)stream);
    return e == hipSuccess ? CX_OK : CX_ERR_LAUNCH;
}

int cx_gemm_bf16_nt_residual(const uint16_t* X, const uint16_t* W, uint16_t* Out, const float* bias,
                             const uint16_t* Residual, int M, int N, int K, int ldx, int ldw, int ldo, int ldr,
                             void* stream) {
    if (M <= 0 || N <= 0) return CX_OK;
    if (!Residual || !Out) return CX_ERR_ARG;
    if (K <= 0 || (K % 64) != 0 || (N % 8) != 0 || (ldo % 8) != 0 || (ldr % 8) != 0) return CX_ERR_SHAPE;
    if ((ldx % 8) != 0 || (ldw % 8) != 0) return CX_ERR_ALIGN;
    if (cx_gemm_get_variant() != 6) return CX_ERR_SHAPE;
    GemmParams p;
    p.X = X; p.W = W; p.Out = Out; p.bias = bias;
    p.M = M; p.N = N; p.K = K; p.ldx = ldx; p.ldw = ldw; p.ldo = ldo;
    p.tiles_m = p.tiles_n = 0; p.split_k = 1; p.alpha = 1.f; p.dbg = g_dbg;
    p.Out2 = const_cast<uint16_t*>(Residual); p.ldo2 = ldr; p.sup_m = p.sup_n = 0; p.trace = nullptr;
    int slot = -1;
    if (g_prof.enabled) {
        if ((g_prof.launches % g_prof.stride) == 0 && g_prof.used < GemmProf::CAP) {
            slot = g_prof.used++;
            if (slot >= g_prof.created) {
                if (hipEventCreate(&g_prof.ev0[slot]) != hipSuccess || hipEventCreate(&g_prof.ev1[slot]) != hipSuccess)
                    return CX_ERR_LAUNCH;
                g_prof.created = slot + 1;
            }
            g_prof.flop[slot] = 2.0 * (double)M * (double)N * (double)K;
            (void)hipEventRecord(g_prof.ev0[slot], (hipStream_t)stream);
        }
        ++g_prof.launches;
    }
    const hipError_t e = cx_launch_gemm_v6(p, GEMM_EPI_NONE, (hipStream_t)stream);
    if (slot >= 0) (void)hipEventRecord(g_prof.ev1[slot], (hipStream_t)stream);
    return e == hipSuccess ? CX_OK : CX_ERR_LAUNCH;
}

int cx_gemm_bf16_bias_gelu(const uint16_t* X, const uint16_t* W, const float* bias, uint16_t* Pre, uint16_t* Act, int M,
                           int N, int K, int ldx, int ldw, int ld_pre, int ld_act, void* stream) {
    return cx_gemm_bf16_bias_act(X, W, bias, Pre, Act, M, N, K, ldx, ldw, ld_pre, ld_act, 0, stream);
}

int cx_gemm_bf16_bias_act(const uint16_t* X, const uint16_t* W, const float* bias, uint16_t* Pre, uint16_t* Act, int M,
                          int N, int K, int ldx, int ldw, int ld_pre, int ld_act, int act, void* stream) {
    if (M <= 0 || N <= 0) return CX_OK;
    if (!Act || (act != 0 && act != 1)) return CX_ERR_ARG;
    if (K <= 0 || (K % 64) != 0 || (N % 8) != 0 || (ld_act % 8) != 0 || (Pre && (ld_pre % 8) != 0)) return CX_ERR_SHAPE;
    if ((ldx % 8) != 0 || (ldw % 8) != 0) return CX_ERR_ALIGN;
    if (cx_gemm_get_variant() != 6) return CX_ERR_SHAPE;
    GemmParams p;
    p.X = X; p.W = W; p.Out = Pre; p.bias = bias;
    p.M = M; p.N = N; p.K = K; p.ldx = ldx; p.ldw = ldw; p.ldo = ld_pre;
    p.tiles_m = p.tiles_n = 0; p.split_k = 1; p.alpha = 1.f; p.dbg = g_dbg;
    p.Out2 = Act; p.ldo2 = ld_act; p.sup_m = p.sup_n = 0; p.trace = nullptr;
    p.act = act;
    int slot = -1;
    if (g_prof.enabled) {
        if ((g_prof.launches % g_prof.stride) == 0 && g_prof.used < GemmProf::CAP) {
            slot = g_prof.used++;
            if (slot >= g_prof.created) {
                if (hipEventCreate(&g_prof.ev0[slot]) != hipSuccess || hipEventCreate(&g_prof.ev1[slot]) != hipSuccess)
                    return CX_ERR_LAUNCH;
                g_prof.created = slot + 1;
            }
            g_prof.flop[slot] = 2.0 * (double)M * (double)N * (double)K;
            (void)hipEventRecord(g_prof.ev0[slot], (hipStream_t)stream);
        }
        ++g_prof.launches;
    }
    const hipError_t e = cx_launch_gemm_v6(p, act == 1 ? GEMM_EPI_QGELU : GEMM_EPI_GELU, (hipStream_t)stream);
    if (slot >= 0) (void)hipEventRecord(g_prof.ev1[slot], (hipStream_t)stream);
    return e == hipSuccess ? CX_OK : CX_ERR_LAUNCH;
}

int cx_gemm_bf16_swiglu_bwd(const uint16_t* dY, const uint16_t* W, const uint16_t* YG, uint16_t* dYG, int M, int I, int K,
                            int ldx, int ldw, int ld_yg, void* stream) {
    if (M <= 0 || I <= 0) return CX_OK;
    if (!dY || !W || !YG || !dYG) return CX_ERR_ARG;
    if (K <= 0 || (K % 64) != 0 || (I % 256) != 0 || (ld_yg % 8) != 0 || ld_yg < 2 * I) return CX_ERR_SHAPE;
    if ((ldx % 8) != 0 || (ldw % 8) != 0) return CX_ERR_ALIGN;
    if (cx_gemm_get_variant() != 6) return CX_ERR_SHAPE;
    GemmParams p;
    p.X = dY; p.W = W; p.Out = dYG; p.bias = nullptr;
    p.M = M; p.N = I; p.K = K; p.ldx = ldx; p.ldw = ldw; p.ldo = ld_yg;
    p.tiles_m = p.tiles_n = 0; p.split_k = 1; p.alpha = 1.f; p.dbg = g_dbg;
    p.Out2 = const_cast<uint16_t*>(YG); p.ldo2 = ld_yg; p.sup_m = p.sup_n = 0; p.trace = nullptr;
    int slot = -1;
    if (g_prof.enabled) {
        if ((g_prof.launches % g_prof.stride) == 0 && g_prof.used < GemmProf::CAP) {
            slot = g_prof.used++;
            if (slot >= g_prof.created) {
                if (hipEventCreate(&g_prof.ev0[slot]) != hipSuccess || hipEventCreate(&g_prof.ev1[slot]) != hipSuccess)
                    return CX_ERR_LAUNCH;
                g_prof.created = slot + 1;
            }
            g_prof.flop[slot] = 2.0 * (double)M * (double)I * (double)K;
            (void)hipEventRecord(g_prof.ev0[slot], (hipStream_t)stream);
        }
        ++g_prof.launches;
    }
    const hipError_t e = cx_launch_gemm_v6(p, GEMM_EPI_SWIGLU_BWD, (hipStream_t)stream);
    if (slot >= 0) (void)hipEventRecord(g_prof.ev1[slot], (hipStream_t)stream);
    return e == hipSuccess ? CX_OK : CX_ERR_LAUNCH;
}

int cx_prof_gemm_config(int enable, int stride) {
    g_prof.enabled = enable != 0;
    g_prof.stride = stride > 0 ? stride : 1;
    g_prof.launches = 0;
    g_prof.used = 0;
    return CX_OK;
}

int cx_prof_gemm_collect(double* total_ms, double* total_flop, long* launches_timed, long* launches_total) {
    double ms = 0.0, fl = 0.0;
    for (int i = 0; i < g_prof.used; ++i) {
        if (hipEventSynchronize(g_prof.ev1[i]) != hipSuccess) return CX_ERR_LAUNCH;
        float t = 0.f;
        if (hipEventElapsedTime(&t, g_prof.ev0[i], g_prof.ev1[i]) != hipSuccess) return CX_ERR_LAUNCH;
        ms += t;
        fl += g_prof.flop[i];
    }
    if (total_ms) *total_ms = ms;
    if (total_flop) *total_flop = fl;
    if (launches_timed) *launches_timed = g_prof.used;
    if (launches_total) *launches_total = g_prof.launches;
    return CX_OK;
}

}

int cx_gemm_bf16_swiglu_gate(const uint16_t* X, const uint16_t* W, uint16_t* G, uint16_t* Act, int M, int I, int K, int ldx,
                             int ldw, int ld_g, int ld_act, void* stream) {
    if (M <= 0 || I <= 0) return CX_OK;
    if (K <= 0 || (K % BK) != 0 || (I % 32) != 0 || (ld_g % 8) != 0 || (ld_act % 8) != 0) return CX_ERR_SHAPE;
    if ((ldx % 8) != 0 || (ldw % 8) != 0) return CX_ERR_ALIGN;
    if (!Act) return CX_ERR_ARG;
    GemmParams p;
    p.X = X; p.W = W; p.Out = G; p.bias = nullptr;
    p.M = M; p.N = 2 * I; p.K = K; p.ldx = ldx; p.ldw = ldw; p.ldo = ld_g;
    p.tiles_m = p.tiles_n = 0; p.split_k = 1; p.alpha = 1.f; p.dbg = 0; p.act = 0;
    p.Out2 = Act; p.ldo2 = ld_act; p.In3 = nullptr; p.sup_m = p.sup_n = 0; p.trace = nullptr;
    return cx_launch_gemm_v6(p, GEMM_EPI_SWIGLU_G, (hipStream_t)stream) == hipSuccess ? CX_OK : CX_ERR_LAUNCH;
}

int cx_gemm_bf16_swiglu_bwd_gate(const uint16_t* dY, const uint16_t* W, const uint16_t* Act, const uint16_t* G, uint16_t* dYG,
                                 int M, int I, int K, int ldx, int ldw, int ld_ag, int ld_dyg, void* stream) {
    if (M <= 0 || I <= 0) return CX_OK;
    if (!dY || !W || !Act || !G || !dYG) return CX_ERR_ARG;
    if (K <= 0 || (K % 64) != 0 || (I % 256) != 0 || (ld_dyg % 8) != 0 || ld_dyg < 2 * I || (ld_ag % 8) != 0 || ld_ag < I)
        return CX_ERR_SHAPE;
    if ((ldx % 8) != 0 || (ldw % 8) != 0) return CX_ERR_ALIGN;
    GemmParams p;
    p.X = dY; p.W = W; p.Out = dYG; p.bias = nullptr;
    p.M = M; p.N = I; p.K = K; p.ldx = ldx; p.ldw = ldw; p.ldo = ld_dyg;
    p.tiles_m = p.tiles_n = 0; p.split_k = 1; p.alpha = 1.f; p.dbg = 0; p.act = 0;
    p.Out2 = const_cast<uint16_t*>(Act); p.ldo2 = ld_ag; p.In3 = G; p.sup_m = p.sup_n = 0; p.trace = nullptr;
    return cx_launch_gemm_v6(p, GEMM_EPI_SWIGLU_BWD_AG, (hipStream_t)stream) == hipSuccess ? CX_OK : CX_ERR_LAUNCH;
// ... 24 lines not shown
```

contrastors_amd/csrc/gemm_bf16_v6.hip:

```cpp
#include "cx_common.h"
#include "../../include/contrastors_hip.h"
#include "gemm_params.h"
#include <type_traits>

namespace {

#ifndef CX_V6_HI_EARLY
#define CX_V6_HI_EARLY 1
#endif
#ifndef CX_V6_OPAQUE
#define CX_V6_OPAQUE 1
#endif
#ifndef CX_V6_NT
#define CX_V6_NT 3
#endif
template <int J>
__device__ __forceinline__ void v6_dma_m0(uint32_t slot_base) {
    asm volatile("s_add_u32 m0, %0, %1" ::"s"(slot_base), "n"(J * 4096) : "memory", "scc");
}
__device__ __forceinline__ void v6_dma_ld(uint32_t off, const bf16_t* base) {
    asm volatile("global_load_lds_dwordx4 %0, %1" ::"v"(off), "s"(base) : "memory");
}
template <int J>
__device__ __forceinline__ void v6_dma_full(uint32_t slot_base, uint32_t off, const bf16_t* base) {
    asm volatile("s_add_u32 m0, %0, %1\n\ts_nop 0\n\tglobal_load_lds_dwordx4 %2, %3" ::"s"(slot_base), "n"(J * 4096), "v"(off),
                 "s"(base) : "memory", "scc");
}
typedef unsigned int cx_u32x4 __attribute__((ext_vector_type(4)));
__device__ __forceinline__ void gst_nt(void* ptr, uint4 v) {
    cx_u32x4 t = {v.x, v.y, v.z, v.w};
    __builtin_nontemporal_store(t, reinterpret_cast<cx_u32x4*>(ptr));
}
__device__ __forceinline__ uint4 gld_nt(const void* ptr) {
    const cx_u32x4 t = __builtin_nontemporal_load(reinterpret_cast<const cx_u32x4*>(ptr));
    return make_uint4(t.x, t.y, t.z, t.w);
}
#if CX_V6_NT & 1
#define gst(ptr, v) gst_nt((ptr), (v))
#else
#define gst(ptr, v) (*reinterpret_cast<uint4*>(ptr) = (v))
#endif
#if CX_V6_NT & 2
#define gld(ptr) gld_nt(ptr)
#else
#define gld(ptr) (*reinterpret_cast<const uint4*>(ptr))
#endif

typedef __attribute__((address_space(3))) void* lds_void_ptr;
typedef const __attribute__((address_space(1))) void* glb_void_ptr;

constexpr int BM6 = 256, BN6 = 256, BK6 = 64;
constexpr int XS6 = 32768;
constexpr int LDS6 = 5 * XS6;

struct Frags6 {
    bf16x8_t w[8], x[8];
};

#include "gemm_v6_acc.inc"

template <int I0, int I1, class F>
CX_DEVICE void v6_static_for(F&& f) {
    if constexpr (I0 < I1) {
        f(std::integral_constant<int, I0>{});
        v6_static_for<I0 + 1, I1>(f);
    }
}

template <int EPI, int DBG = 0>
__global__ __launch_bounds__(256, 1) __attribute__((amdgpu_waves_per_eu(1, 1))) void gemm_bf16_v6_kernel(GemmParams p) {
    extern __shared__ __attribute__((aligned(16))) char dsm[];
    constexpr bool IS_SWIGLU_BWD = EPI == GEMM_EPI_SWIGLU_BWD || EPI == GEMM_EPI_SWIGLU_BWD_AG;
    constexpr bool AG = EPI == GEMM_EPI_SWIGLU_BWD_AG;
    constexpr bool SAVEG = EPI == GEMM_EPI_SWIGLU_G;
    long long t_begin = 0, n_ktiles = 0;
    if constexpr (DBG != 0) t_begin = (long long)__builtin_amdgcn_s_memtime();
    long long ph[9] = {0, 0, 0, 0, 0, 0, 0, 0, 0}, t_last = t_begin, kt0_cyc = 0;
#define CX_PH(i_)                                                              \
    do {                                                                       \
        if constexpr ((DBG & 128) != 0) {                                      \
            const long long now_ = (long long)__builtin_amdgcn_s_memtime();    \
            ph[(i_)] += now_ - t_last;                                         \
            t_last = now_;                                                     \
        }                                                                      \
    } while (0)
    const int tid = threadIdx.x;
    const int lane = tid & 63;
    const int wave = __builtin_amdgcn_readfirstlane(tid >> 6);
    const int l15 = lane & 15, g4 = lane >> 4;
    const int wm = wave >> 1, wn = wave & 1;
    const int nk = p.K / BK6;
    const int per_xcd = gridDim.x >> 3;
    const int xcd = blockIdx.x & 7, idx = blockIdx.x >> 3;
    const int gn = p.sup_n > 0 ? p.sup_n : 1, gm = 8 / gn;
    const int xi = xcd / gn, xj = xcd - xi * gn;
    const int m_lo = p.tiles_m * xi / gm, m_hi = p.tiles_m * (xi + 1) / gm;
    const int n_lo = p.tiles_n * xj / gn, n_wd = p.tiles_n * (xj + 1) / gn - n_lo;
    const int nloc = (m_hi - m_lo) * n_wd;
    auto tile_of = [&](int round) {
        const int l = round * per_xcd + idx;
        if (l >= nloc) return -1;
        const int q = l / n_wd;
        return ((m_lo + q) << 8) | (n_lo + (l - q * n_wd));
    };

    uint32_t xoff[8], woff[8];
    const bf16_t* xbase = p.X;
    const bf16_t* wbase = p.W;
    int lx_round = 0, lx_kt = 0, lx_slot = 0;
    int lw_round = 0, lw_kt = 0, lw_slot = 0;
    bool lx_live, lw_live;
    const int first_tile = tile_of(0);
    bool x_clamped = true, w_clamped = true;
    auto x_setup = [&](int tile) {
        const int tm = tile >> 8;
        xbase = p.X + (size_t)tm * BM6 * p.ldx;
        const int rows = p.M - tm * BM6;
        if (rows < BM6 || x_clamped) {
            x_clamped = rows < BM6;
#pragma unroll
            for (int j = 0; j < 8; ++j) {
                const int r = (j * 4 + wave) * 8 + (lane >> 3);
                const int c = (lane & 7) ^ ((r >> 1) & 7);
                const int rr = r < rows ? r : rows - 1;
                xoff[j] = (uint32_t)rr * (uint32_t)p.ldx * 2u + c * 16;
            }
        }
    };
    auto w_setup = [&](int tile) {
        const int tn = tile & 255;
        wbase = p.W + (size_t)tn * BN6 * p.ldw;
        const int rows = p.N - tn * BN6;
        if (rows < BN6 || w_clamped) {
            w_clamped = rows < BN6;
#pragma unroll
            for (int j = 0; j < 8; ++j) {
                const int r = (j * 4 + wave) * 8 + (lane >> 3);
                const int c = (lane & 7) ^ ((r >> 1) & 7);
                const int rr = r < rows ? r : rows - 1;
                woff[j] = (uint32_t)rr * (uint32_t)p.ldw * 2u + c * 16;
            }
        }
    };
    const uint32_t lds0 = (uint32_t)(uintptr_t)(lds_void_ptr)dsm;
    const uint32_t lds_wave = lds0 + wave * 1024;
    uint32_t x_m0 = lds_wave, w_m0 = lds_wave + 3 * XS6;
    auto issue_x_tile = [&]() {
        if constexpr ((DBG & 1) != 0) return;
        v6_dma_full<0>(x_m0, xoff[0], xbase); v6_dma_full<1>(x_m0, xoff[1], xbase); v6_dma_full<2>(x_m0, xoff[2], xbase);
        v6_dma_full<3>(x_m0, xoff[3], xbase); v6_dma_full<4>(x_m0, xoff[4], xbase); v6_dma_full<5>(x_m0, xoff[5], xbase);
        v6_dma_full<6>(x_m0, xoff[6], xbase); v6_dma_full<7>(x_m0, xoff[7], xbase);
    };
    auto issue_w_tile = [&]() {
        if constexpr ((DBG & 1) != 0) return;
        v6_dma_full<0>(w_m0, woff[0], wbase); v6_dma_full<1>(w_m0, woff[1], wbase); v6_dma_full<2>(w_m0, woff[2], wbase);
        v6_dma_full<3>(w_m0, woff[3], wbase); v6_dma_full<4>(w_m0, woff[4], wbase); v6_dma_full<5>(w_m0, woff[5], wbase);
        v6_dma_full<6>(w_m0, woff[6], wbase); v6_dma_full<7>(w_m0, woff[7], wbase);
    };
    auto x_advance = [&]() {
        xbase += BK6;
        lx_slot = lx_slot == 2 ? 0 : lx_slot + 1;
        x_m0 = lds_wave + lx_slot * XS6;
        if (++lx_kt == nk) {
            lx_kt = 0;
            const int t = tile_of(++lx_round);
            lx_live = t >= 0;
            x_setup(lx_live ? t : first_tile);
        }
    };
    auto w_advance = [&]() {
        wbase += BK6;
        lw_slot ^= 1;
        w_m0 = lds_wave + (3 + lw_slot) * XS6;
        if (++lw_kt == nk) {
            lw_kt = 0;
            const int t = tile_of(++lw_round);
            lw_live = t >= 0;
            w_setup(lw_live ? t : first_tile);
        }
    };


    int cp_round = 0;
    int cp_tile = first_tile;
    lx_live = lw_live = cp_tile >= 0;
    if (cp_tile < 0) return;
    x_setup(cp_tile);
    w_setup(cp_tile);
    issue_x_tile();
    x_advance();
    issue_w_tile();
    w_advance();
    issue_x_tile();
    x_advance();
    int xs_slot = 0, ws_slot = 0;

    Frags6 F0, F1;
    auto read_one = [&](Frags6& f, const char* xs, const char* ws, int kk, int i) {
        if constexpr ((DBG & 4) != 0) return;
        if (i < 8)
            f.w[i] = lds_read_frag(ws, tile64_off(wn * 128 + i * 16 + l15, kk * 4 + g4));
        else
            f.x[i - 8] = lds_read_frag(xs, tile64_off(wm * 128 + (i - 8) * 16 + l15, kk * 4 + g4));
    };
    auto mma1 = [&](const Frags6& f, int i) {
        if constexpr ((DBG & 8) != 0) return;
        v6_mfma(i, f.w[i & 7], f.x[i >> 3]);
    };
    auto mma1z = [&](const Frags6& f, int i) {
        if constexpr ((DBG & 8) != 0) return;
        v6_mfma_z(i, f.w[i & 7], f.x[i >> 3]);
    };

#ifndef CX_V6_DMA_SPREAD
#define CX_V6_DMA_SPREAD 4
#endif
#ifndef CX_V6_RD_SPREAD
#define CX_V6_RD_SPREAD 2
#endif
#define CX_SEG(MMA, f, i0, i1, nxt, rxs, rws, rkk, R0, RSP, kind, D0, DSP, J0, ND)                     \
    do {                                                                                              \
        v6_static_for<(i0), (i1)>([&](auto ic_) __attribute__((always_inline)) {                      \
            constexpr int I_ = decltype(ic_)::value;                                                  \
            constexpr bool RD_ = (RSP) > 0 && I_ >= (R0) && (I_ - (R0)) % ((RSP) > 0 ? (RSP) : 1) == 0 && (I_ - (R0)) / ((RSP) > 0 ? (RSP) : 1) < 16; \
            constexpr bool DM_ = (ND) > 0 && I_ >= (D0) && (I_ - (D0)) % (DSP) == 0 && (I_ - (D0)) / (DSP) < (ND); \
            constexpr int J_ = DM_ ? (J0) + (I_ - (D0)) / (DSP) : 0;                                  \
            if constexpr (RD_) read_one(nxt, rxs, rws, rkk, (I_ - (R0)) / ((RSP) > 0 ? (RSP) : 1));   \
            if constexpr (DM_) CX_DMA_M0(kind, J_);                                                   \
            MMA(f, I_);                                                                               \
            if constexpr (DM_) CX_DMA_LD(kind, J_);                                                   \
            __builtin_amdgcn_sched_barrier(0);                                                        \
        });                                                                                           \
    } while (0)
#define CX_DMA_M0(kind, J)                                                       \
    do {                                                                         \
        if constexpr ((kind) == 1 && (DBG & 1) == 0) v6_dma_m0<(J)>(w_m0);        \
        if constexpr ((kind) == 2 && (DBG & 1) == 0) v6_dma_m0<(J)>(x_m0);        \
    } while (0)
#define CX_DMA_LD(kind, J)                                                       \
    do {                                                                         \
        if constexpr ((kind) == 1 && (DBG & 1) == 0) v6_dma_ld(woff[(J)], wbase); \
        if constexpr ((kind) == 2 && (DBG & 1) == 0) v6_dma_ld(xoff[(J)], xbase); \
    } while (0)

    {
        asm volatile("s_waitcnt vmcnt(8)" ::: "memory");
        __builtin_amdgcn_s_barrier();
#pragma unroll
        for (int i = 0; i < 16; ++i) read_one(F0, dsm, dsm + 3 * XS6, 0, i);
    }

    int cp_kt = 0;
    int pxs_slot = 0, pws_slot = 0;
    auto kt_body = [&](auto first) {
        if constexpr (DBG != 0) ++n_ktiles;
        constexpr int RS_ = CX_V6_RD_SPREAD, DS_ = CX_V6_DMA_SPREAD;
        const char* xs = dsm + xs_slot * XS6;
        const char* ws = dsm + (3 + ws_slot) * XS6;
        const int nxs_slot = xs_slot == 2 ? 0 : xs_slot + 1, nws_slot = ws_slot ^ 1;
        if constexpr (decltype(first)::value) {
            CX_SEG(mma1z, F0, 0, 64, F1, xs, ws, 1, RS_ == 2 ? 0 : 1, RS_, 1, RS_ == 2 ? 1 : 17, DS_, 0, 8);
        } else {
            CX_SEG(mma1, F0, 0, 64, F1, xs, ws, 1, RS_ == 2 ? 0 : 1, RS_, 1, RS_ == 2 ? 1 : 17, DS_, 0, 8);
        }
        w_advance();
        CX_SEG(mma1, F1, 0, 32, F0, xs, ws, 0, 0, 0, 2, 0, RS_ == 2 ? 8 : DS_, 0, 4);
        asm volatile("s_waitcnt lgkmcnt(0)" ::: "memory");
        if constexpr ((DBG & 128) != 0) {
            const long long w0_ = (long long)__builtin_amdgcn_s_memtime();
            asm volatile("s_waitcnt vmcnt(4)" ::: "memory");
            const long long w1_ = (long long)__builtin_amdgcn_s_memtime();
            ph[decltype(first)::value ? 0 : 1] += w1_ - w0_;
        } else if constexpr ((DBG & 32) == 0) {
            asm volatile("s_waitcnt vmcnt(4)" ::: "memory");
        }
        if constexpr ((DBG & 2) == 0) __builtin_amdgcn_s_barrier();
        const char* nxs = dsm + nxs_slot * XS6;
        const char* nws = dsm + (3 + nws_slot) * XS6;
        CX_SEG(mma1, F1, 32, 64, F0, nxs, nws, 0, RS_ == 2 ? 32 : 33, RS_, 2, RS_ == 2 ? 33 : 49, RS_ == 2 ? 8 : DS_, 4, 4);
        x_advance();
        if constexpr ((DBG & 128) != 0 && decltype(first)::value) {
            const long long now_ = (long long)__builtin_amdgcn_s_memtime();
            kt0_cyc += now_ - t_last;
        }
        ++cp_kt;
        pxs_slot = xs_slot;
        pws_slot = ws_slot;
        xs_slot = nxs_slot;
        ws_slot = nws_slot;
    };

#pragma unroll 1
    while (cp_tile >= 0) {
        cp_kt = 0;
        kt_body(std::true_type{});
#pragma unroll 1
        while (cp_kt < nk) kt_body(std::false_type{});

        {
            CX_PH(2);
            asm volatile("s_nop 7\n\ts_nop 7\n\ts_nop 7" ::: "memory");
            const int tn = cp_tile & 255, tm = cp_tile >> 8;
            const int m0 = tm * BM6 + wm * 128, n0 = tn * BN6 + wn * 128;
            char* my = ((wave < 2) ? dsm + pxs_slot * XS6 : dsm + (3 + pws_slot) * XS6) + (wave & 1) * 16384;
            constexpr int ROWB = 272;
            auto prow = [&](int q) { return (q >> 1) * 16 + l15; };
            auto pcol = [&](int q) { return (q & 1) * 16 + 4 * g4; };
            auto qoff = [](int q, int rowb) { return (q >> 1) * 16 * rowb + (q & 1) * 32; };
            if constexpr ((DBG & 16) != 0) {
            } else if constexpr (EPI == GEMM_EPI_NONE || EPI == GEMM_EPI_ACT_BWD || EPI == GEMM_EPI_QACT_BWD) {
                constexpr bool ACTB = EPI == GEMM_EPI_ACT_BWD || EPI == GEMM_EPI_QACT_BWD;
                float cs0 = 0.f, cs1 = 0.f, cs2 = 0.f, cs3 = 0.f, cs4 = 0.f, cs5 = 0.f, cs6 = 0.f, cs7 = 0.f;
                constexpr int act_kind = EPI == GEMM_EPI_QACT_BWD ? CX_ACT_QUICK_GELU : CX_ACT_GELU;
                auto mul_grad = [&](uint4& v, const uint4& r) {
#define CX_MG(w_, ca, cb)                                                                              \
    {                                                                                                 \
        const float o0 = bf16lo_to_f32(v.w_) * act_grad(bf16lo_to_f32(r.w_), act_kind);               \
        const float o1 = bf16hi_to_f32(v.w_) * act_grad(bf16hi_to_f32(r.w_), act_kind);               \
        v.w_ = pack_bf16x2(o0, o1);                                                                   \
        ca += bf16lo_to_f32(v.w_);                                                                    \
        cb += bf16hi_to_f32(v.w_);                                                                    \
    }
                    CX_MG(x, cs0, cs1) CX_MG(y, cs2, cs3) CX_MG(z, cs4, cs5) CX_MG(w, cs6, cs7)
#undef CX_MG
                };
                auto flush_colsum = [&]() {
                    if constexpr (ACTB) {
                        float c[8] = {cs0, cs1, cs2, cs3, cs4, cs5, cs6, cs7};
#pragma unroll
                        for (int e = 0; e < 8; ++e) {
                            c[e] += __shfl_xor(c[e], 16, 64);
                            c[e] += __shfl_xor(c[e], 32, 64);
                        }
                        const int n = n0 + (lane & 15) * 8;
                        if (p.colsum_part && lane < 16 && m0 < p.M && n + 8 <= p.N) {
                            float* dst = p.colsum_part + (size_t)(m0 >> 7) * p.N + n;
                            *reinterpret_cast<float4*>(dst) = make_float4(c[0], c[1], c[2], c[3]);
                            *reinterpret_cast<float4*>(dst + 4) = make_float4(c[4], c[5], c[6], c[7]);
                        }
                    }
                };
                const bool add_bias = p.bias != nullptr;
                const bf16_t* resid = reinterpret_cast<const bf16_t*>(p.Out2);
                auto fast_tile = [&](auto with_resid) {
                    constexpr bool RES = decltype(with_resid)::value;
                    const int rrow = lane >> 4, rch = lane & 15;
                    bf16_t* outp = reinterpret_cast<bf16_t*>(p.Out) + (size_t)(m0 + rrow) * p.ldo + n0 + rch * 8;
                    const bf16_t* resp = RES ? resid + (size_t)(m0 + rrow) * p.ldo2 + n0 + rch * 8 : nullptr;
                    const char* rd = my + rrow * ROWB + rch * 16;
                    char* wr = my + prow(0) * ROWB + pcol(0) * 2;
                    uint2 pk[16];
                    auto pack_pass = [&](int b) {
#pragma unroll
                        for (int a = 0; a < 4; ++a) {
                            float blk[16];
                            v6_read_block(4 * b + a, blk);
#pragma unroll
                            for (int q = 0; q < 4; ++q) {
                                pk[a * 4 + q].x = pack_bf16x2(blk[4 * q], blk[4 * q + 1]);
                                pk[a * 4 + q].y = pack_bf16x2(blk[4 * q + 2], blk[4 * q + 3]);
                            }
                        }
                    };
                    auto stage = [&]() {
#pragma unroll
                        for (int a = 0; a < 4; ++a)
#pragma unroll
                            for (int q = 0; q < 4; ++q) *reinterpret_cast<uint2*>(wr + a * 64 + qoff(q, ROWB)) = pk[a * 4 + q];
                    };
                    uint4 r0 = {}, r1 = {}, r2 = {}, r3 = {}, r4 = {}, r5 = {}, r6 = {}, r7 = {};
#define CX_RES_ROWS(b_)                                                                                   \
    r0 = gld(resp + (size_t)((b_) * 32 + 0) * p.ldo2);                          \
    r1 = gld(resp + (size_t)((b_) * 32 + 4) * p.ldo2);                          \
    r2 = gld(resp + (size_t)((b_) * 32 + 8) * p.ldo2);                          \
    r3 = gld(resp + (size_t)((b_) * 32 + 12) * p.ldo2);                         \
    r4 = gld(resp + (size_t)((b_) * 32 + 16) * p.ldo2);                         \
    r5 = gld(resp + (size_t)((b_) * 32 + 20) * p.ldo2);                         \
    r6 = gld(resp + (size_t)((b_) * 32 + 24) * p.ldo2);                         \
    r7 = gld(resp + (size_t)((b_) * 32 + 28) * p.ldo2);
                    auto add_res = [&](uint4& v, const uint4& r) {
                        v.x = pack_bf16x2(bf16lo_to_f32(v.x) + bf16lo_to_f32(r.x), bf16hi_to_f32(v.x) + bf16hi_to_f32(r.x));
                        v.y = pack_bf16x2(bf16lo_to_f32(v.y) + bf16lo_to_f32(r.y), bf16hi_to_f32(v.y) + bf16hi_to_f32(r.y));
                        v.z = pack_bf16x2(bf16lo_to_f32(v.z) + bf16lo_to_f32(r.z), bf16hi_to_f32(v.z) + bf16hi_to_f32(r.z));
                        v.w = pack_bf16x2(bf16lo_to_f32(v.w) + bf16lo_to_f32(r.w), bf16hi_to_f32(v.w) + bf16hi_to_f32(r.w));
                    };
                    auto one_pass = [&](auto bc) {
                        constexpr int b = decltype(bc)::value;
                        uint4 v0 = *reinterpret_cast<const uint4*>(rd + 0 * ROWB), v1 = *reinterpret_cast<const uint4*>(rd + 4 * ROWB),
                              v2 = *reinterpret_cast<const uint4*>(rd + 8 * ROWB), v3 = *reinterpret_cast<const uint4*>(rd + 12 * ROWB),
                              v4 = *reinterpret_cast<const uint4*>(rd + 16 * ROWB), v5 = *reinterpret_cast<const uint4*>(rd + 20 * ROWB),
                              v6 = *reinterpret_cast<const uint4*>(rd + 24 * ROWB), v7 = *reinterpret_cast<const uint4*>(rd + 28 * ROWB);
                        __builtin_amdgcn_sched_barrier(0);
                        if constexpr (b < 3) pack_pass(b + 1);
                        __builtin_amdgcn_sched_barrier(0);
                        if constexpr (RES) {
                            add_res(v0, r0); add_res(v1, r1); add_res(v2, r2); add_res(v3, r3);
                            add_res(v4, r4); add_res(v5, r5); add_res(v6, r6); add_res(v7, r7);
                            if constexpr (b < 3) {
                                __builtin_amdgcn_sched_barrier(0);
                                CX_RES_ROWS(b + 1)
                                __builtin_amdgcn_sched_barrier(0);
                            }
                        }
                        if constexpr (b < 3) stage();
                        bf16_t* o = outp + (size_t)(b * 32) * p.ldo;
                        if constexpr ((DBG & 64) != 0) {
                            const uint4 vs[8] = {v0, v1, v2, v3, v4, v5, v6, v7};
#pragma unroll
                            for (int i = 0; i < 8; ++i) asm volatile("" ::"v"(vs[i].x), "v"(vs[i].y), "v"(vs[i].z), "v"(vs[i].w));
                            asm volatile("" ::"v"(o));
                            return;
                        }
                        gst(o, v0);
                        gst(o + (size_t)4 * p.ldo, v1);
                        gst(o + (size_t)8 * p.ldo, v2);
                        gst(o + (size_t)12 * p.ldo, v3);
                        gst(o + (size_t)16 * p.ldo, v4);
                        gst(o + (size_t)20 * p.ldo, v5);
                        gst(o + (size_t)24 * p.ldo, v6);
                        gst(o + (size_t)28 * p.ldo, v7);
                    };
                    if constexpr (RES) { CX_RES_ROWS(0) }
                    pack_pass(0);
                    stage();
                    one_pass(std::integral_constant<int, 0>{});
                    one_pass(std::integral_constant<int, 1>{});
                    one_pass(std::integral_constant<int, 2>{});
                    one_pass(std::integral_constant<int, 3>{});
#undef CX_RES_ROWS
                };
                auto fast_tile_actb = [&]() {
                    const int rrow = lane >> 4, rch = lane & 15;
                    bf16_t* outp = reinterpret_cast<bf16_t*>(p.Out) + (size_t)(m0 + rrow) * p.ldo + n0 + rch * 8;
                    const bf16_t* resp = resid + (size_t)(m0 + rrow) * p.ldo2 + n0 + rch * 8;
                    const char* rd = my + rrow * ROWB + rch * 16;
                    char* wr = my + prow(0) * ROWB + pcol(0) * 2;
                    auto stage_pass = [&](int b) {
#pragma unroll
                        for (int a = 0; a < 4; ++a) {
                            float blk[16];
                            v6_read_block(4 * b + a, blk);
#pragma unroll
                            for (int q = 0; q < 4; ++q) {
                                uint2 pk2;
                                pk2.x = pack_bf16x2(blk[4 * q], blk[4 * q + 1]);
                                pk2.y = pack_bf16x2(blk[4 * q + 2], blk[4 * q + 3]);
                                *reinterpret_cast<uint2*>(wr + a * 64 + qoff(q, ROWB)) = pk2;
                            }
                            __builtin_amdgcn_sched_barrier(0);
                        }
                    };
                    uint4 r0, r1, r2, r3;
#define CX_PRE_ROWS(hh_)                                                        \
    r0 = gld(resp + (size_t)((hh_) * 16 + 0) * p.ldo2);                         \
    r1 = gld(resp + (size_t)((hh_) * 16 + 4) * p.ldo2);                         \
    r2 = gld(resp + (size_t)((hh_) * 16 + 8) * p.ldo2);                         \
    r3 = gld(resp + (size_t)((hh_) * 16 + 12) * p.ldo2);
                    auto half_pass = [&](auto hc) {
                        constexpr int hh = decltype(hc)::value;
                        constexpr int h = hh & 1;
                        uint4 v0 = *reinterpret_cast<const uint4*>(rd + (h * 16 + 0) * ROWB), v1 = *reinterpret_cast<const uint4*>(rd + (h * 16 + 4) * ROWB),
                              v2 = *reinterpret_cast<const uint4*>(rd + (h * 16 + 8) * ROWB), v3 = *reinterpret_cast<const uint4*>(rd + (h * 16 + 12) * ROWB);
                        __builtin_amdgcn_sched_barrier(0);
                        mul_grad(v0, r0); __builtin_amdgcn_sched_barrier(0);
                        mul_grad(v1, r1); __builtin_amdgcn_sched_barrier(0);
                        mul_grad(v2, r2); __builtin_amdgcn_sched_barrier(0);
                        mul_grad(v3, r3); __builtin_amdgcn_sched_barrier(0);
                        if constexpr (hh < 7) { CX_PRE_ROWS(hh + 1) }
                        __builtin_amdgcn_sched_barrier(0);
                        bf16_t* o = outp + (size_t)(hh * 16) * p.ldo;
                        gst(o, v0);
                        gst(o + (size_t)4 * p.ldo, v1);
                        gst(o + (size_t)8 * p.ldo, v2);
                        gst(o + (size_t)12 * p.ldo, v3);
                        if constexpr (h == 1 && hh < 7) stage_pass((hh >> 1) + 1);
                    };
                    CX_PRE_ROWS(0)
                    stage_pass(0);
                    half_pass(std::integral_constant<int, 0>{}); half_pass(std::integral_constant<int, 1>{});
                    half_pass(std::integral_constant<int, 2>{}); half_pass(std::integral_constant<int, 3>{});
                    half_pass(std::integral_constant<int, 4>{}); half_pass(std::integral_constant<int, 5>{});
                    half_pass(std::integral_constant<int, 6>{}); half_pass(std::integral_constant<int, 7>{});
#undef CX_PRE_ROWS
                };
                const bool fast = p.alpha == 1.f && !add_bias && m0 + 128 <= p.M && n0 + 128 <= p.N;
                auto store_tile = [&](auto plain) {
#pragma unroll
                    for (int b = 0; b < 4; ++b) {
                        uint4 r0 = {}, r1 = {}, r2 = {}, r3 = {}, r4 = {}, r5 = {}, r6 = {}, r7 = {};
                        if (resid) {
#define CX_RES_LOAD(ps, dst)                                                                              \
    {                                                                                                 \
        int m_ = m0 + b * 32 + (ps) * 4 + (lane >> 4);                                                \
        m_ = m_ < p.M ? m_ : p.M - 1;                                                                 \
        int n_ = n0 + (lane & 15) * 8;                                                                \
        n_ = n_ + 8 <= p.N ? n_ : 0;                                                                  \
        dst = gld(resid + (size_t)m_ * p.ldo2 + n_);                      \
    }
                            CX_RES_LOAD(0, r0) CX_RES_LOAD(1, r1) CX_RES_LOAD(2, r2) CX_RES_LOAD(3, r3)
                            CX_RES_LOAD(4, r4) CX_RES_LOAD(5, r5) CX_RES_LOAD(6, r6) CX_RES_LOAD(7, r7)
#undef CX_RES_LOAD
                        }
#pragma unroll
                        for (int a = 0; a < 4; ++a) {
                            float blk[16];
                            v6_read_block(4 * b + a, blk);
#pragma unroll
                            for (int q = 0; q < 4; ++q) {
                                const int nl = a * 32 + pcol(q);
                                float v[4];
#pragma unroll
                                for (int e = 0; e < 4; ++e) v[e] = blk[4 * q + e];
                                if constexpr (!decltype(plain)::value) {
#pragma unroll
                                    for (int e = 0; e < 4; ++e) v[e] *= p.alpha;
                                    if (add_bias) {
                                        const int n = n0 + nl;
                                        if (n < p.N) {
                                            const float4 bv = *reinterpret_cast<const float4*>(p.bias + n);
                                            v[0] += bv.x; v[1] += bv.y; v[2] += bv.z; v[3] += bv.w;
                                        }
                                    }
                                }
                                uint2 pk;
                                pk.x = pack_bf16x2(v[0], v[1]);
                                pk.y = pack_bf16x2(v[2], v[3]);
                                *reinterpret_cast<uint2*>(my + prow(q) * ROWB + nl * 2) = pk;
                            }
                        }
#pragma unroll
                        for (int ps = 0; ps < 8; ++ps) {
                            const int row = ps * 4 + (lane >> 4), ch = lane & 15;
                            const int m = m0 + b * 32 + row, n = n0 + ch * 8;
                            uint4 vv = *reinterpret_cast<const uint4*>(my + row * ROWB + ch * 16);
                            if (resid && ACTB) {
                                const uint4 rr = ps == 0 ? r0 : ps == 1 ? r1 : ps == 2 ? r2 : ps == 3 ? r3 : ps == 4 ? r4 : ps == 5 ? r5
                                                 : ps == 6 ? r6 : r7;
                                if (m < p.M && n + 8 <= p.N) mul_grad(vv, rr);
                            } else if (resid) {
                                const uint4 rr = ps == 0 ? r0 : ps == 1 ? r1 : ps == 2 ? r2 : ps == 3 ? r3 : ps == 4 ? r4 : ps == 5 ? r5
                                                 : ps == 6 ? r6 : r7;
                                vv.x = pack_bf16x2(bf16lo_to_f32(vv.x) + bf16lo_to_f32(rr.x), bf16hi_to_f32(vv.x) + bf16hi_to_f32(rr.x));
                                vv.y = pack_bf16x2(bf16lo_to_f32(vv.y) + bf16lo_to_f32(rr.y), bf16hi_to_f32(vv.y) + bf16hi_to_f32(rr.y));
                                vv.z = pack_bf16x2(bf16lo_to_f32(vv.z) + bf16lo_to_f32(rr.z), bf16hi_to_f32(vv.z) + bf16hi_to_f32(rr.z));
                                vv.w = pack_bf16x2(bf16lo_to_f32(vv.w) + bf16lo_to_f32(rr.w), bf16hi_to_f32(vv.w) + bf16hi_to_f32(rr.w));
                            }
                            if (m < p.M && n + 8 <= p.N)
                                gst(reinterpret_cast<bf16_t*>(p.Out) + (size_t)m * p.ldo + n, vv);
                        }
                    }
                };
                if constexpr (ACTB) {
                    if (fast) {
                        fast_tile_actb();
                    } else {
                        store_tile(std::true_type{});
                    }
                    flush_colsum();
                } else if (fast) {
                    if (resid) {
                        fast_tile(std::true_type{});
                    } else {
                        fast_tile(std::false_type{});
                    }
                } else if (p.alpha == 1.f && !add_bias) {
                    store_tile(std::true_type{});
                } else {
                    store_tile(std::false_type{});
                }
            } else if constexpr (IS_SWIGLU_BWD) {
                const bf16_t* yg_in = reinterpret_cast<const bf16_t*>(p.Out2);
                const bf16_t* g_in = reinterpret_cast<const bf16_t*>(p.In3);
                bf16_t* dyg = reinterpret_cast<bf16_t*>(p.Out);
                const int c0 = 2 * n0;
                auto bwd_elem = [&](float yv, float gv, float dv, float& dyo, float& dgo) {
                    if constexpr (AG) {
                        swiglu_bwd_from_act(dv, yv, gv, dyo, dgo);
                    } else {
                        const float sg = __builtin_amdgcn_rcpf(1.f + __builtin_amdgcn_exp2f(-1.4426950408889634f * gv));
                        const float gs = gv * sg;
                        dyo = gs * dv;
                        dgo = (sg + gs * (1.f - sg)) * dv * yv;
                    }
                };
                auto bwd_quad = [&](const float (&yv)[4], const float (&gv)[4], const float* dv, float (&dyo)[4], float (&dgo)[4]) {
                    if constexpr (AG) {
#pragma unroll
                        for (int h = 0; h < 2; ++h) {
                            cx_f2 y2, g2;
                            swiglu_bwd_from_act2(cx_f2{dv[2 * h], dv[2 * h + 1]}, cx_f2{yv[2 * h], yv[2 * h + 1]},
                                                 cx_f2{gv[2 * h], gv[2 * h + 1]}, y2, g2);
                            dyo[2 * h] = y2.x; dyo[2 * h + 1] = y2.y;
                            dgo[2 * h] = g2.x; dgo[2 * h + 1] = g2.y;
                        }
                    } else {
#pragma unroll
                        for (int e = 0; e < 4; ++e) bwd_elem(yv[e], gv[e], dv[e], dyo[e], dgo[e]);
                    }
                };
                auto cell = [&](int row, int colbyte) { return my + row * 512 + ((((colbyte >> 4) ^ row) & 31) << 4) + (colbyte & 15); };
                const bool fast_bwd = m0 + 128 <= p.M && n0 + 128 <= p.N;
                if (fast_bwd) {
                    int lane_e = lane;
#if CX_V6_OPAQUE >= 1
                    asm volatile("" : "+v"(lane_e));
#endif
                    const int lrow = lane_e >> 5, lch = lane_e & 31;
                    const bf16_t* src = AG ? ((lch & 4) ? g_in : yg_in) + (size_t)(m0 + lrow) * p.ldo2 + n0 + (lch >> 3) * 32 + (lch & 3) * 8
                                           : yg_in + (size_t)(m0 + lrow) * p.ldo2 + c0 + lch * 8;
                    bf16_t* dst = dyg + (size_t)(m0 + lrow) * p.ldo + c0 + lch * 8;
                    uint4 t0, t1, t2, t3, t4, t5, t6, t7, t8, t9, t10, t11, t12, t13, t14, t15;
#define CX_L(i, b_) t##i = gld(src + (size_t)((b_) * 32 + (i) * 2) * p.ldo2);
#define CX_LOAD_LO(b_) CX_L(0, b_) CX_L(1, b_) CX_L(2, b_) CX_L(3, b_) CX_L(4, b_) CX_L(5, b_) CX_L(6, b_) CX_L(7, b_)
#define CX_LOAD_HI(b_) CX_L(8, b_) CX_L(9, b_) CX_L(10, b_) CX_L(11, b_) CX_L(12, b_) CX_L(13, b_) CX_L(14, b_) CX_L(15, b_)
#define CX_S(i) *reinterpret_cast<uint4*>(cell((i) * 2 + lrow, lch * 16)) = t##i;
#define CX_STAGE_ALL CX_S(0) CX_S(1) CX_S(2) CX_S(3) CX_S(4) CX_S(5) CX_S(6) CX_S(7) CX_S(8) CX_S(9) CX_S(10) CX_S(11) CX_S(12) CX_S(13) CX_S(14) CX_S(15)
                    auto one_pass = [&](auto bc) {
                        constexpr int b = decltype(bc)::value;
                        int lane_p = lane_e;
#if CX_V6_OPAQUE >= 2
                        asm volatile("" : "+v"(lane_p));
#endif
                        const int lrow = lane_p >> 5, lch = lane_p & 31, l15 = lane_p & 15, g4 = lane_p >> 4;
                        CX_STAGE_ALL
                        __builtin_amdgcn_sched_barrier(0);
                        CX_PH(4);
                        if constexpr (b < 3) { CX_LOAD_LO(b + 1) }
#if CX_V6_HI_EARLY
                        if constexpr (b < 3) { CX_LOAD_HI(b + 1) }
#endif
                        __builtin_amdgcn_sched_barrier(0);
                        CX_PH(5);
#pragma unroll
                        for (int a = 0; a < 4; ++a) {
                            float da[16];
                            v6_read_block(4 * b + a, da);
                            uint2 yy[4], gg[4];
#pragma unroll
                            for (int q = 0; q < 4; ++q) {
                                yy[q] = *reinterpret_cast<const uint2*>(cell((q >> 1) * 16 + l15, (a * 64 + (q & 1) * 16 + 4 * g4) * 2));
                                gg[q] = *reinterpret_cast<const uint2*>(cell((q >> 1) * 16 + l15, (a * 64 + 32 + (q & 1) * 16 + 4 * g4) * 2));
                            }
#pragma unroll
                            for (int q = 0; q < 4; ++q) {
                                char* py = cell((q >> 1) * 16 + l15, (a * 64 + (q & 1) * 16 + 4 * g4) * 2);
                                char* pg = cell((q >> 1) * 16 + l15, (a * 64 + 32 + (q & 1) * 16 + 4 * g4) * 2);
                                const float y[4] = {bf16lo_to_f32(yy[q].x), bf16hi_to_f32(yy[q].x), bf16lo_to_f32(yy[q].y), bf16hi_to_f32(yy[q].y)};
                                const float g[4] = {bf16lo_to_f32(gg[q].x), bf16hi_to_f32(gg[q].x), bf16lo_to_f32(gg[q].y), bf16hi_to_f32(gg[q].y)};
                                float dy[4], dg[4];
                                bwd_quad(y, g, &da[4 * q], dy, dg);
                                uint2 o;
                                o.x = pack_bf16x2(dy[0], dy[1]); o.y = pack_bf16x2(dy[2], dy[3]);
                                *reinterpret_cast<uint2*>(py) = o;
                                o.x = pack_bf16x2(dg[0], dg[1]); o.y = pack_bf16x2(dg[2], dg[3]);
                                *reinterpret_cast<uint2*>(pg) = o;
                            }
                            __builtin_amdgcn_sched_barrier(0);
                        }
#if !CX_V6_HI_EARLY
                        if constexpr (b < 3) { CX_LOAD_HI(b + 1) }
#endif
                        __builtin_amdgcn_sched_barrier(0);
                        CX_PH(6);
#pragma unroll
                        for (int h = 0; h < 4; ++h) {
                            const uint4 v0 = *reinterpret_cast<const uint4*>(cell((h * 4 + 0) * 2 + lrow, lch * 16));
                            const uint4 v1 = *reinterpret_cast<const uint4*>(cell((h * 4 + 1) * 2 + lrow, lch * 16));
                            const uint4 v2 = *reinterpret_cast<const uint4*>(cell((h * 4 + 2) * 2 + lrow, lch * 16));
                            const uint4 v3 = *reinterpret_cast<const uint4*>(cell((h * 4 + 3) * 2 + lrow, lch * 16));
                            bf16_t* o = dst + (size_t)(b * 32 + h * 8) * p.ldo;
                            gst(o, v0);
                            gst(o + (size_t)2 * p.ldo, v1);
                            gst(o + (size_t)4 * p.ldo, v2);
                            gst(o + (size_t)6 * p.ldo, v3);
                        }
                        __builtin_amdgcn_sched_barrier(0);
                        CX_PH(7);
                    };
                    CX_LOAD_LO(0) CX_LOAD_HI(0)
                    __builtin_amdgcn_sched_barrier(0);
                    CX_PH(3);
                    one_pass(std::integral_constant<int, 0>{});
                    one_pass(std::integral_constant<int, 1>{});
                    one_pass(std::integral_constant<int, 2>{});
                    one_pass(std::integral_constant<int, 3>{});
#undef CX_L
#undef CX_LOAD_LO
#undef CX_LOAD_HI
#undef CX_S
#undef CX_STAGE_ALL
                } else
#pragma unroll 1
                for (int b = 0; b < 4; ++b) {
                    int lane_c = lane;
                    asm volatile("" : "+v"(lane_c));
                    const int lrow = lane_c >> 5, lch = lane_c & 31, l15 = lane_c & 15, g4 = lane_c >> 4;
#define CX_YG_LOAD(i)                                                                                   \
    uint4 in##i;                                                                                      \
    {                                                                                                 \
        int m_ = m0 + b * 32 + (i) * 2 + lrow;                                                        \
        m_ = m_ < p.M ? m_ : p.M - 1;                                                                 \
// ... 246 lines not shown
#pragma unroll
                            for (int a = 0; a < 4; ++a)
#pragma unroll
                                for (int q = 0; q < 4; ++q) *reinterpret_cast<uint2*>(wry + a * 64 + qoff(q, ROWB)) = pky[a * 4 + q];
                        }
                        if constexpr (SAVE_G) {
#pragma unroll
                            for (int pr = 0; pr < 2; ++pr)
#pragma unroll
                                for (int q = 0; q < 4; ++q) *reinterpret_cast<uint2*>(wrg + pr * 64 + qoff(q, AROWB)) = pkg[pr * 4 + q];
                        }
#pragma unroll
                        for (int pr = 0; pr < 2; ++pr)
#pragma unroll
                            for (int q = 0; q < 4; ++q) *reinterpret_cast<uint2*>(wra + pr * 64 + qoff(q, AROWB)) = pka[pr * 4 + q];
                    };
                    auto one_pass = [&](auto bc) {
                        constexpr int b = decltype(bc)::value;
                        uint4 v0 = {}, v1 = {}, v2 = {}, v3 = {}, v4 = {}, v5 = {}, v6 = {}, v7 = {};
                        if constexpr (SAVE_YG) {
                            v0 = *reinterpret_cast<const uint4*>(rdy + 0 * ROWB); v1 = *reinterpret_cast<const uint4*>(rdy + 4 * ROWB);
                            v2 = *reinterpret_cast<const uint4*>(rdy + 8 * ROWB); v3 = *reinterpret_cast<const uint4*>(rdy + 12 * ROWB);
                            v4 = *reinterpret_cast<const uint4*>(rdy + 16 * ROWB); v5 = *reinterpret_cast<const uint4*>(rdy + 20 * ROWB);
                            v6 = *reinterpret_cast<const uint4*>(rdy + 24 * ROWB); v7 = *reinterpret_cast<const uint4*>(rdy + 28 * ROWB);
                        }
                        if constexpr (SAVE_G) {
                            v0 = *reinterpret_cast<const uint4*>(rdg + 0 * AROWB); v1 = *reinterpret_cast<const uint4*>(rdg + 8 * AROWB);
                            v2 = *reinterpret_cast<const uint4*>(rdg + 16 * AROWB); v3 = *reinterpret_cast<const uint4*>(rdg + 24 * AROWB);
                        }
                        const uint4 a0 = *reinterpret_cast<const uint4*>(rda + 0 * AROWB), a1 = *reinterpret_cast<const uint4*>(rda + 8 * AROWB),
                                    a2 = *reinterpret_cast<const uint4*>(rda + 16 * AROWB), a3 = *reinterpret_cast<const uint4*>(rda + 24 * AROWB);
                        __builtin_amdgcn_sched_barrier(0);
                        CX_PH(4);
                        if constexpr (b < 3) compute_pass(b + 1);
                        __builtin_amdgcn_sched_barrier(0);
                        CX_PH(5);
                        if constexpr (b < 3) stage();
                        __builtin_amdgcn_sched_barrier(0);
                        CX_PH(6);
                        if constexpr (SAVE_YG) {
                            bf16_t* o = ygp + (size_t)(b * 32) * p.ldo;
                            gst(o, v0);
                            gst(o + (size_t)4 * p.ldo, v1);
                            gst(o + (size_t)8 * p.ldo, v2);
                            gst(o + (size_t)12 * p.ldo, v3);
                            gst(o + (size_t)16 * p.ldo, v4);
                            gst(o + (size_t)20 * p.ldo, v5);
                            gst(o + (size_t)24 * p.ldo, v6);
                            gst(o + (size_t)28 * p.ldo, v7);
                        }
                        if constexpr (SAVE_G) {
                            bf16_t* o = gp + (size_t)(b * 32) * p.ldo;
                            gst(o, v0);
                            gst(o + (size_t)8 * p.ldo, v1);
                            gst(o + (size_t)16 * p.ldo, v2);
                            gst(o + (size_t)24 * p.ldo, v3);
                        }
                        bf16_t* oa = actp + (size_t)(b * 32) * p.ldo2;
                        gst(oa, a0);
                        gst(oa + (size_t)8 * p.ldo2, a1);
                        gst(oa + (size_t)16 * p.ldo2, a2);
                        gst(oa + (size_t)24 * p.ldo2, a3);
                        __builtin_amdgcn_sched_barrier(0);
                        CX_PH(7);
                    };
                    compute_pass(0);
                    stage();
                    __builtin_amdgcn_sched_barrier(0);
                    CX_PH(3);
                    one_pass(std::integral_constant<int, 0>{});
                    one_pass(std::integral_constant<int, 1>{});
                    one_pass(std::integral_constant<int, 2>{});
                    one_pass(std::integral_constant<int, 3>{});
                };
                if (m0 + 128 <= p.M && n0 + 128 <= p.N) {
                    if (p.Out) {
                        fast_swiglu(std::true_type{});
                    } else {
                        fast_swiglu(std::false_type{});
                    }
                } else
#pragma unroll
                for (int b = 0; b < 4; ++b) {
#pragma unroll
                    for (int pr = 0; pr < 2; ++pr) {
                        float yb[16], gb[16];
                        v6_read_block(4 * b + 2 * pr, yb);
                        v6_read_block(4 * b + 2 * pr + 1, gb);
                        if (p.Out) {
#pragma unroll
                            for (int q = 0; q < 4; ++q) {
                                uint2 pk;
                                if constexpr (SAVEG) {
                                    pk.x = pack_bf16x2(gb[4 * q], gb[4 * q + 1]);
                                    pk.y = pack_bf16x2(gb[4 * q + 2], gb[4 * q + 3]);
                                    *reinterpret_cast<uint2*>(my + prow(q) * AROWB + (pr * 32 + pcol(q)) * 2) = pk;
                                } else {
                                    pk.x = pack_bf16x2(yb[4 * q], yb[4 * q + 1]);
                                    pk.y = pack_bf16x2(yb[4 * q + 2], yb[4 * q + 3]);
                                    *reinterpret_cast<uint2*>(my + prow(q) * ROWB + (2 * pr * 32 + pcol(q)) * 2) = pk;
                                    pk.x = pack_bf16x2(gb[4 * q], gb[4 * q + 1]);
                                    pk.y = pack_bf16x2(gb[4 * q + 2], gb[4 * q + 3]);
                                    *reinterpret_cast<uint2*>(my + prow(q) * ROWB + ((2 * pr + 1) * 32 + pcol(q)) * 2) = pk;
                                }
                            }
                        }
#pragma unroll
                        for (int q = 0; q < 4; ++q) {
                            float o[4];
#pragma unroll
                            for (int e = 0; e < 4; ++e) {
                                const float yy = bf16_to_f32(f32_to_bf16(yb[4 * q + e]));
                                const float gg = bf16_to_f32(f32_to_bf16(gb[4 * q + e]));
                                o[e] = gg * yy * __builtin_amdgcn_rcpf(1.f + __expf(-gg));
                            }
                            uint2 pk;
                            pk.x = pack_bf16x2(o[0], o[1]); pk.y = pack_bf16x2(o[2], o[3]);
                            *reinterpret_cast<uint2*>(mya + prow(q) * AROWB + (pr * 32 + pcol(q)) * 2) = pk;
                        }
                    }
                    if (p.Out) {
                        if constexpr (SAVEG) {
#pragma unroll
                            for (int ps = 0; ps < 4; ++ps) {
                                const int row = ps * 8 + (lane >> 3), ch = lane & 7;
                                const int m = m0 + b * 32 + row;
                                const int col = (n0 >> 1) + ch * 8;
                                const uint4 vv = *reinterpret_cast<const uint4*>(my + row * AROWB + ch * 16);
                                if (m < p.M && 2 * col < p.N)
                                    gst(reinterpret_cast<bf16_t*>(p.Out) + (size_t)m * p.ldo + col, vv);
                            }
                        } else {
#pragma unroll
                            for (int ps = 0; ps < 8; ++ps) {
                                const int row = ps * 4 + (lane >> 4), ch = lane & 15;
                                const int m = m0 + b * 32 + row, n = n0 + ch * 8;
                                const uint4 vv = *reinterpret_cast<const uint4*>(my + row * ROWB + ch * 16);
                                if (m < p.M && n < p.N)
                                    gst(reinterpret_cast<bf16_t*>(p.Out) + (size_t)m * p.ldo + n, vv);
                            }
                        }
                    }
#pragma unroll
                    for (int ps = 0; ps < 4; ++ps) {
                        const int row = ps * 8 + (lane >> 3), ch = lane & 7;
                        const int m = m0 + b * 32 + row;
                        const int col = (n0 >> 1) + ch * 8;
                        const uint4 vv = *reinterpret_cast<const uint4*>(mya + row * AROWB + ch * 16);
                        if (m < p.M && 2 * col < p.N)
                            gst(reinterpret_cast<bf16_t*>(p.Out2) + (size_t)m * p.ldo2 + col, vv);
                    }
                }
            }
            cp_tile = tile_of(++cp_round);
            {
                asm volatile("" : "=v"(F0.w[0]), "=v"(F0.w[1]), "=v"(F0.w[2]), "=v"(F0.w[3]), "=v"(F0.w[4]), "=v"(F0.w[5]), "=v"(F0.w[6]), "=v"(F0.w[7]));
                asm volatile("" : "=v"(F0.x[0]), "=v"(F0.x[1]), "=v"(F0.x[2]), "=v"(F0.x[3]), "=v"(F0.x[4]), "=v"(F0.x[5]), "=v"(F0.x[6]), "=v"(F0.x[7]));
                if constexpr (IS_SWIGLU_BWD) {
                    asm volatile("" : "=v"(xoff[0]), "=v"(xoff[1]), "=v"(xoff[2]), "=v"(xoff[3]), "=v"(xoff[4]), "=v"(xoff[5]), "=v"(xoff[6]), "=v"(xoff[7]));
                    asm volatile("" : "=v"(woff[0]), "=v"(woff[1]), "=v"(woff[2]), "=v"(woff[3]), "=v"(woff[4]), "=v"(woff[5]), "=v"(woff[6]), "=v"(woff[7]));
                    x_clamped = w_clamped = true;
                    x_setup(lx_live ? tile_of(lx_round) : first_tile);
                    xbase += lx_kt * BK6;
                    w_setup(lw_live ? tile_of(lw_round) : first_tile);
                    wbase += lw_kt * BK6;
                }
                if (cp_tile >= 0) {
#pragma unroll
                    for (int i = 0; i < 16; ++i) read_one(F0, dsm + xs_slot * XS6, dsm + (3 + ws_slot) * XS6, 0, i);
                }
            }
            __builtin_amdgcn_s_barrier();
            CX_PH(8);
        }
    }
#undef CX_PH
#undef CX_DMA_M0
#undef CX_DMA_LD
    asm volatile("s_waitcnt vmcnt(0)" ::: "memory");
    if constexpr (DBG != 0) {
        if (p.trace && tid == 0) {
            p.trace[16 * blockIdx.x] = (long long)__builtin_amdgcn_s_memtime() - t_begin;
            p.trace[16 * blockIdx.x + 1] = n_ktiles;
            if constexpr ((DBG & 128) != 0) {
#pragma unroll
                for (int i = 2; i < 9; ++i) p.trace[16 * blockIdx.x + i] = ph[i];
                p.trace[16 * blockIdx.x + 9] = ph[0];
                p.trace[16 * blockIdx.x + 10] = ph[1];
                p.trace[16 * blockIdx.x + 11] = kt0_cyc;
            }
        }
    }
}

template <int EPI, int DBG = 0>
hipError_t launch6(const GemmParams& p, hipStream_t stream) {
    static CxLdsOptIn lds;
    if (!lds.ensure(reinterpret_cast<const void*>(&gemm_bf16_v6_kernel<EPI, DBG>), LDS6)) return hipErrorInvalidValue;
    const int ntiles = p.tiles_m * p.tiles_n;
    const int grid = ntiles < 256 ? (ntiles + 7) / 8 * 8 : 256;
    hipLaunchKernelGGL((gemm_bf16_v6_kernel<EPI, DBG>), dim3(grid), dim3(256), LDS6, stream, p);
    return hipGetLastError();
}

typedef __attribute__((address_space(3))) bf16x4_t* lds_b4_ptr6;
constexpr int TNROW6 = 512;

CX_DEVICE int tn_swz(int t) { return ((t & 3) << 2) ^ (((t >> 3) & 1) << 1); }

__global__ __launch_bounds__(256, 1) __attribute__((amdgpu_waves_per_eu(1, 1))) void gemm_bf16_v6tn_kernel(GemmParams p) {
    extern __shared__ __attribute__((aligned(16))) char dsm[];
    const int tid = threadIdx.x;
    const int lane = tid & 63;
    const int wave = __builtin_amdgcn_readfirstlane(tid >> 6);
    const int l15 = lane & 15, g4 = lane >> 4;
    const int wm = wave >> 1, wn = wave & 1;
    const int nwg = p.tiles_m * p.tiles_n * p.split_k;
    int lid = xcd_remap(blockIdx.x, nwg);
    int tm, tn;
    if (p.tiles_m < p.tiles_n) {
        tm = lid % p.tiles_m;
        lid /= p.tiles_m;
        tn = lid % p.tiles_n;
        lid /= p.tiles_n;
    } else {
        tn = lid % p.tiles_n;
        lid /= p.tiles_n;
        tm = lid % p.tiles_m;
        lid /= p.tiles_m;
    }
    const int sk = lid;
    const int m0 = tm * BM6, n0 = tn * BN6;
    const int nk_total = p.K / BK6;
    const int kt_begin = (int)(((long)nk_total * sk) / p.split_k);
    const int kt_end = (int)(((long)nk_total * (sk + 1)) / p.split_k);
    const int nk = kt_end - kt_begin;
    if (nk <= 0) return;

    uint32_t xo[8], wo[8];
#pragma unroll
    for (int j = 0; j < 8; ++j) {
        const int t = (j * 4 + wave) * 2 + (lane >> 5);
        const int c = (lane & 31) ^ tn_swz(t);
        xo[j] = (uint32_t)t * (uint32_t)p.ldx * 2u + c * 16;
        wo[j] = (uint32_t)t * (uint32_t)p.ldw * 2u + c * 16;
    }
    const bf16_t* xb = p.X + (size_t)kt_begin * BK6 * p.ldx + m0;
    const bf16_t* wb = p.W + (size_t)kt_begin * BK6 * p.ldw + n0;
    const size_t xstep = (size_t)BK6 * p.ldx, wstep = (size_t)BK6 * p.ldw;
    int lx_slot = 0, lw_slot = 0;
    const uint32_t lds0 = (uint32_t)(uintptr_t)(lds_void_ptr)dsm;
    const uint32_t lds_wave = lds0 + wave * 1024;
    uint32_t x_m0 = lds_wave, w_m0 = lds_wave + 3 * XS6;
    auto issue_x_tile = [&]() {
        v6_dma_full<0>(x_m0, xo[0], xb); v6_dma_full<1>(x_m0, xo[1], xb); v6_dma_full<2>(x_m0, xo[2], xb); v6_dma_full<3>(x_m0, xo[3], xb);
        v6_dma_full<4>(x_m0, xo[4], xb); v6_dma_full<5>(x_m0, xo[5], xb); v6_dma_full<6>(x_m0, xo[6], xb); v6_dma_full<7>(x_m0, xo[7], xb);
    };
    auto issue_w_tile = [&]() {
        v6_dma_full<0>(w_m0, wo[0], wb); v6_dma_full<1>(w_m0, wo[1], wb); v6_dma_full<2>(w_m0, wo[2], wb); v6_dma_full<3>(w_m0, wo[3], wb);
        v6_dma_full<4>(w_m0, wo[4], wb); v6_dma_full<5>(w_m0, wo[5], wb); v6_dma_full<6>(w_m0, wo[6], wb); v6_dma_full<7>(w_m0, wo[7], wb);
    };
    auto x_advance = [&](int next) {
        xb += next < nk ? xstep : 0;
        lx_slot = lx_slot == 2 ? 0 : lx_slot + 1;
        x_m0 = lds_wave + lx_slot * XS6;
    };
    auto w_advance = [&](int next) {
        wb += next < nk ? wstep : 0;
        lw_slot ^= 1;
        w_m0 = lds_wave + (3 + lw_slot) * XS6;
    };

    Frags6 F0, F1;
    uint32_t woff[8], xoff[8];
    {
        const int tl = 8 * g4 + (l15 >> 2), fl = 4 * (l15 & 3);
#pragma unroll
        for (int i = 0; i < 8; ++i) {
            const int fw = wn * 128 + i * 16 + fl, fx = wm * 128 + i * 16 + fl;
            woff[i] = tl * TNROW6 + (((fw >> 3) ^ tn_swz(tl)) << 4) + (fw & 4) * 2;
            xoff[i] = tl * TNROW6 + (((fx >> 3) ^ tn_swz(tl)) << 4) + (fx & 4) * 2;
        }
    }
    auto tr_pair = [&](const char* base, int kk) -> bf16x8_t {
        union { bf16x4_t h[2]; bf16x8_t v; } u;
        u.h[0] = __builtin_amdgcn_ds_read_tr16_b64_v4bf16((lds_b4_ptr6)(base + kk * 16384));
        u.h[1] = __builtin_amdgcn_ds_read_tr16_b64_v4bf16((lds_b4_ptr6)(base + kk * 16384 + 2048));
        return u.v;
    };
    auto read_one = [&](Frags6& f, int xslot, int wslot, int kk, int i) {
        if (i < 8)
            f.w[i] = tr_pair(dsm + (3 + wslot) * XS6 + woff[i], kk);
        else
            f.x[i - 8] = tr_pair(dsm + xslot * XS6 + xoff[i - 8], kk);
    };
    auto mma1 = [&](const Frags6& f, int i) { v6_mfma(i, f.w[i & 7], f.x[i >> 3]); };
    auto mma1z = [&](const Frags6& f, int i) { v6_mfma_z(i, f.w[i & 7], f.x[i >> 3]); };
#define CX_DMA_M0(kind, J)                                  \
    do {                                                    \
        if constexpr ((kind) == 1) v6_dma_m0<(J)>(w_m0);     \
        if constexpr ((kind) == 2) v6_dma_m0<(J)>(x_m0);     \
    } while (0)
#define CX_DMA_LD(kind, J)                                  \
    do {                                                    \
        if constexpr ((kind) == 1) v6_dma_ld(wo[(J)], wb);   \
        if constexpr ((kind) == 2) v6_dma_ld(xo[(J)], xb);   \
    } while (0)

    issue_x_tile();
    x_advance(1);
    issue_w_tile();
    w_advance(1);
    issue_x_tile();
    x_advance(2);
    asm volatile("s_waitcnt vmcnt(8)" ::: "memory");
    __builtin_amdgcn_s_barrier();
#pragma unroll
    for (int i = 0; i < 16; ++i) read_one(F0, 0, 0, 0, i);

    int xs_slot = 0, ws_slot = 0;
    auto kt_body = [&](auto first, int t) {
        constexpr int RS_ = CX_V6_RD_SPREAD, DS_ = CX_V6_DMA_SPREAD;
        const int nxs_slot = xs_slot == 2 ? 0 : xs_slot + 1, nws_slot = ws_slot ^ 1;
        if constexpr (decltype(first)::value) {
            CX_SEG(mma1z, F0, 0, 64, F1, xs_slot, ws_slot, 1, RS_ == 2 ? 0 : 1, RS_, 1, RS_ == 2 ? 1 : 17, DS_, 0, 8);
        } else {
            CX_SEG(mma1, F0, 0, 64, F1, xs_slot, ws_slot, 1, RS_ == 2 ? 0 : 1, RS_, 1, RS_ == 2 ? 1 : 17, DS_, 0, 8);
        }
        w_advance(t + 2);
        CX_SEG(mma1, F1, 0, 32, F0, xs_slot, ws_slot, 0, 0, 0, 2, 0, RS_ == 2 ? 8 : DS_, 0, 4);
        asm volatile("s_waitcnt lgkmcnt(0)" ::: "memory");
        asm volatile("s_waitcnt vmcnt(4)" ::: "memory");
        __builtin_amdgcn_s_barrier();
        CX_SEG(mma1, F1, 32, 64, F0, nxs_slot, nws_slot, 0, RS_ == 2 ? 32 : 33, RS_, 2, RS_ == 2 ? 33 : 49, RS_ == 2 ? 8 : DS_, 4, 4);
        x_advance(t + 3);
        xs_slot = nxs_slot;
        ws_slot = nws_slot;
    };
    kt_body(std::true_type{}, 0);
#pragma unroll 1
    for (int t = 1; t < nk; ++t) kt_body(std::false_type{}, t);
#undef CX_SEG
#undef CX_DMA_M0
#undef CX_DMA_LD

    asm volatile("s_waitcnt vmcnt(0)\n\ts_nop 7\n\ts_nop 7\n\ts_nop 7" ::: "memory");
    float* part = reinterpret_cast<float*>(p.Out) + (size_t)sk * p.M * p.ldo;
#pragma unroll
    for (int b = 0; b < 4; ++b) {
        float* rowp = part + (size_t)(m0 + wm * 128 + b * 32 + l15) * p.ldo + n0 + wn * 128 + 4 * g4;
        float* rowq = rowp + (size_t)16 * p.ldo;
#pragma unroll
        for (int a = 0; a < 4; ++a) v6_store_block_f32(4 * b + a, rowp + a * 32, rowq + a * 32);
    }
}

#ifndef CX_V7_POLICY
#define CX_V7_POLICY 1
#endif
#ifndef CX_PRODUCT
int g_v7_mode = -1;
#else
constexpr int g_v7_mode = -1;
#endif
bool v7_takes(const GemmParams& p, int epi) {
    const int mode = g_v7_mode >= 0 ? (g_v7_mode ? 2 : 0) : CX_V7_POLICY;
    if (mode == 0 || !cx_gemm_v7_covers(p, epi)) return false;
    if (mode == 2) return true;
    if (epi == GEMM_EPI_SWIGLU_G) return false;
    const long tiles256 = (long)((p.M + BM6 - 1) / BM6) * ((p.N + BN6 - 1) / BN6);
    return tiles256 <= 400;
}

#ifndef CX_PRODUCT
int g_v6_dbg = 0;
long long* g_v6_trace = nullptr;
int g_v6_force_gn = 0;
#else
constexpr int g_v6_force_gn = 0;
#endif

int cx_gemm_v6_groups(int tiles_m, int tiles_n, int K) {
    if (g_v6_force_gn) return g_v6_force_gn;
    const double xb = (double)tiles_m * 256 * K * 2, wb = (double)tiles_n * 256 * K * 2;
    int best = 1;
    double best_cost = 0;
    for (int gn = 1; gn <= 8; gn *= 2) {
        const int gm = 8 / gn;
        if ((tiles_n % gn) != 0 || (tiles_m % gm) != 0) continue;
        const double slice = wb / gn;
        const double rounds = (double)tiles_m / gm * (tiles_n / gn) / 32.0;
        const double wcost = slice <= 2.5 * 1048576 ? gm * wb : (rounds < 1 ? 1 : rounds) * slice * 8;
        const double cost = gn * xb + wcost;
        if (gn == 1 || cost < best_cost) { best = gn; best_cost = cost; }
    }
    return best;
}

}

#ifndef CX_PRODUCT
void cx_gemm_v6_set_trace(long long* buf) { g_v6_trace = buf; }
void cx_gemm_v6_set_ablate(int mask) { g_v6_dbg = mask; }
void cx_gemm_v6_force_groups(int gn) { g_v6_force_gn = (gn == 1 || gn == 2 || gn == 4 || gn == 8) ? gn : 0; }
void cx_gemm_v7_set_mode(int mode) { g_v7_mode = mode < 0 ? -1 : (mode ? 1 : 0); }
#endif

hipError_t cx_launch_gemm_v6_tn(GemmParams p, hipStream_t stream) {
    static CxLdsOptIn lds;
    if (!lds.ensure(reinterpret_cast<const void*>(&gemm_bf16_v6tn_kernel), LDS6)) return hipErrorInvalidValue;
    p.tiles_m = p.M / BM6;
    p.tiles_n = p.N / BN6;
    hipLaunchKernelGGL(gemm_bf16_v6tn_kernel, dim3(p.tiles_m * p.tiles_n * p.split_k), dim3(256), LDS6, stream, p);
    return hipGetLastError();
}

namespace {
__global__ __launch_bounds__(256) void colsum_part_reduce_kernel(const float* __restrict__ part, float* dst, int nblocks, int N) {
    __shared__ float red[4][64];
    const int col = blockIdx.x * 64 + (threadIdx.x & 63), grp = threadIdx.x >> 6;
    float sacc = 0.f;
    if (col < N) {
#pragma unroll 4
        for (int b = grp; b < nblocks; b += 4) sacc += part[(size_t)b * N + col];
    }
    red[grp][threadIdx.x & 63] = sacc;
    __syncthreads();
    if (grp == 0 && col < N) dst[col] += (red[0][threadIdx.x] + red[1][threadIdx.x]) + (red[2][threadIdx.x] + red[3][threadIdx.x]);
}
}
hipError_t cx_launch_colsum_part_reduce(const float* part, float* dst, int nblocks, int N, hipStream_t stream) {
    hipLaunchKernelGGL(colsum_part_reduce_kernel, dim3((N + 63) / 64), dim3(256), 0, stream, part, dst, nblocks, N);
    return hipGetLastError();
}

hipError_t cx_launch_gemm_v6(GemmParams p, int epi, hipStream_t stream) {
    if (v7_takes(p, epi)) return cx_launch_gemm_v7(p, epi, g_v6_force_gn, stream);
    p.tiles_m = (p.M + BM6 - 1) / BM6;
    p.tiles_n = (p.N + BN6 - 1) / BN6;
    if (p.tiles_n > 256) return hipErrorInvalidValue;
    p.sup_n = cx_gemm_v6_groups(p.tiles_m, p.tiles_n, p.K);
#ifndef CX_PRODUCT
    if (epi == GEMM_EPI_NONE && g_v6_dbg) {
        p.trace = g_v6_trace;
        switch (g_v6_dbg) {
            case 1: return launch6<GEMM_EPI_NONE, 1>(p, stream);
            case 2: return launch6<GEMM_EPI_NONE, 2>(p, stream);
            case 4: return launch6<GEMM_EPI_NONE, 4>(p, stream);
            case 16: return launch6<GEMM_EPI_NONE, 16>(p, stream);
            case 32: return launch6<GEMM_EPI_NONE, 32>(p, stream);
            case 33: return launch6<GEMM_EPI_NONE, 33>(p, stream);
            case 35: return launch6<GEMM_EPI_NONE, 35>(p, stream);
            case 39: return launch6<GEMM_EPI_NONE, 39>(p, stream);
            case 55: return launch6<GEMM_EPI_NONE, 55>(p, stream);
            case 59: return launch6<GEMM_EPI_NONE, 59>(p, stream);
            case 64: return launch6<GEMM_EPI_NONE, 64>(p, stream);
            case 128: return launch6<GEMM_EPI_NONE, 128>(p, stream);
            default: break;
        }
    }
#endif
#ifndef CX_PRODUCT
    if (g_v6_dbg == 128 && (epi == GEMM_EPI_SWIGLU_G || epi == GEMM_EPI_SWIGLU || epi == GEMM_EPI_SWIGLU_BWD_AG)) {
        p.trace = g_v6_trace;
        return epi == GEMM_EPI_SWIGLU_G ? launch6<GEMM_EPI_SWIGLU_G, 128>(p, stream)
               : epi == GEMM_EPI_SWIGLU ? launch6<GEMM_EPI_SWIGLU, 128>(p, stream) : launch6<GEMM_EPI_SWIGLU_BWD_AG, 128>(p, stream);
    }
#endif
    return epi == GEMM_EPI_SWIGLU ? launch6<GEMM_EPI_SWIGLU>(p, stream)
           : epi == GEMM_EPI_SWIGLU_G ? launch6<GEMM_EPI_SWIGLU_G>(p, stream)
           : epi == GEMM_EPI_SWIGLU_BWD_AG ? launch6<GEMM_EPI_SWIGLU_BWD_AG>(p, stream)
           : epi == GEMM_EPI_GELU ? launch6<GEMM_EPI_GELU>(p, stream)
           : epi == GEMM_EPI_QGELU ? launch6<GEMM_EPI_QGELU>(p, stream)
           : epi == GEMM_EPI_SWIGLU_BWD ? launch6<GEMM_EPI_SWIGLU_BWD>(p, stream)
           : epi == GEMM_EPI_ACT_BWD ? (p.act == CX_ACT_QUICK_GELU ? launch6<GEMM_EPI_QACT_BWD>(p, stream) : launch6<GEMM_EPI_ACT_BWD>(p, stream))
                                  : launch6<GEMM_EPI_NONE>(p, stream);
}
```

contrastors_amd/csrc/gemm_params.h:

```cpp
#pragma once
#include <hip/hip_runtime.h>
#include <stdint.h>

enum { GEMM_OUT_BF16 = 0, GEMM_OUT_F32 = 1, GEMM_OUT_F32_ATOMIC = 2, GEMM_OUT_F32_PARTIAL = 3 };
enum { GEMM_EPI_NONE = 0, GEMM_EPI_SWIGLU = 1, GEMM_EPI_GELU = 2, GEMM_EPI_SWIGLU_BWD = 3,
       GEMM_EPI_QGELU = 4,
       GEMM_EPI_SWIGLU_G = 5,
       GEMM_EPI_SWIGLU_BWD_AG = 6,
       GEMM_EPI_QACT_BWD = 8,
       GEMM_EPI_ACT_BWD = 7 };

struct GemmParams {
    const uint16_t* X;
    const uint16_t* W;
    void* Out;
    const float* bias;
    int M, N, K;
    int ldx, ldw, ldo;
    int tiles_m, tiles_n, split_k;
    float alpha;
    int dbg;
    int act;
    void* Out2;
    int ldo2;
    const uint16_t* In3;
    float* colsum_part;
    int sup_m, sup_n;
    long long* trace;
};

hipError_t cx_launch_gemm_v5(GemmParams p, int form, int out_mode, int epi, hipStream_t stream);
hipError_t cx_launch_gemm_v6(GemmParams p, int epi, hipStream_t stream);
void cx_gemm_v6_force_groups(int gn);
void cx_gemm_v6_set_trace(long long* buf);
void cx_gemm_v6_set_ablate(int mask);
hipError_t cx_launch_gemm_v6_tn(GemmParams p, hipStream_t stream);
hipError_t cx_launch_colsum_part_reduce(const float* part, float* dst, int nblocks, int N, hipStream_t stream);
bool cx_gemm_v7_covers(const GemmParams& p, int epi);
hipError_t cx_launch_gemm_v7(GemmParams p, int epi, int force_gn, hipStream_t stream);
void cx_gemm_v7_set_trace(long long* buf);
int cx_gemm_v7_occupancy_query(void);
void cx_gemm_v7_set_ablate(int mask);
void cx_gemm_v7_set_flags(int f);
void cx_gemm_v7_set_period(int cycles);
void cx_gemm_v7_set_mode(int mode);
void cx_gemm_v5_set_persistent(bool on);
void cx_gemm_v5_set_use_v6(bool on);
bool cx_gemm_v5_get_use_v6(void);
void cx_gemm_v5_set_trace(long long* buf);
```

contrastors_amd/csrc/layernorm.hip:

```cpp
#include "cx_common.h"
#include "../../include/contrastors_hip.h"

namespace {

CX_DEVICE void load4_bf16(const bf16_t* p, float (&v)[4]) {
    const uint2 u = *reinterpret_cast<const uint2*>(p);
    v[0] = bf16lo_to_f32(u.x); v[1] = bf16hi_to_f32(u.x);
    v[2] = bf16lo_to_f32(u.y); v[3] = bf16hi_to_f32(u.y);
}
CX_DEVICE void store4_bf16(bf16_t* p, const float (&v)[4]) {
    uint2 u;
    u.x = pack_bf16x2(v[0], v[1]);
    u.y = pack_bf16x2(v[2], v[3]);
    *reinterpret_cast<uint2*>(p) = u;
}
CX_DEVICE void load4_f32(const float* p, float (&v)[4]) {
    const float4 u = *reinterpret_cast<const float4*>(p);
    v[0] = u.x; v[1] = u.y; v[2] = u.z; v[3] = u.w;
}

CX_DEVICE void unpack4_bf16(const uint2 u, float (&v)[4]) {
    v[0] = bf16lo_to_f32(u.x); v[1] = bf16hi_to_f32(u.x);
    v[2] = bf16lo_to_f32(u.y); v[3] = bf16hi_to_f32(u.y);
}
template <int NCH>
CX_DEVICE void fetch_row(const bf16_t* __restrict__ base, int row, int lane, uint2 (&raw)[NCH]) {
#pragma unroll
    for (int i = 0; i < NCH; ++i)
        raw[i] = *reinterpret_cast<const uint2*>(base + (size_t)row * (NCH * 256) + (i * 64 + lane) * 4);
}

template <int NCH>
CX_DEVICE void row_stats(const float (&z)[NCH][4], int d, float eps, float& mean, float& rstd) {
    float s = 0.f;
#pragma unroll
    for (int i = 0; i < NCH; ++i)
#pragma unroll
        for (int e = 0; e < 4; ++e) s += z[i][e];
    mean = wave_sum(s) / (float)d;
    float v = 0.f;
#pragma unroll
    for (int i = 0; i < NCH; ++i)
#pragma unroll
        for (int e = 0; e < 4; ++e) {
            const float c = z[i][e] - mean;
            v += c * c;
        }
    rstd = rsqrtf(wave_sum(v) / (float)d + eps);
}

template <int NCH>
__global__ __launch_bounds__(256) void ln_fwd_kernel(const bf16_t* __restrict__ x0, const bf16_t* __restrict__ res,
                                                     const float* __restrict__ gamma,
                                                     const float* __restrict__ beta, bf16_t* __restrict__ out,
                                                     bf16_t* z_out, float* __restrict__ mean_o,
                                                     float* __restrict__ rstd_o, int rows, float eps) {
    constexpr int D = NCH * 256;
    const int lane = threadIdx.x & 63, wave = threadIdx.x >> 6;
    float g[NCH][4], b[NCH][4];
#pragma unroll
    for (int i = 0; i < NCH; ++i) {
        load4_f32(gamma + (i * 64 + lane) * 4, g[i]);
        load4_f32(beta + (i * 64 + lane) * 4, b[i]);
    }
    const int stride = gridDim.x * 4;
    int row = blockIdx.x * 4 + wave;
    uint2 nx[NCH], nr[NCH];
    if (row < rows) {
        fetch_row<NCH>(x0, row, lane, nx);
        if (res) fetch_row<NCH>(res, row, lane, nr);
    }
    for (; row < rows; row += stride) {
        float z[NCH][4];
#pragma unroll
        for (int i = 0; i < NCH; ++i) {
            unpack4_bf16(nx[i], z[i]);
            if (res) {
                float r[4];
                unpack4_bf16(nr[i], r);
#pragma unroll
                for (int e = 0; e < 4; ++e) z[i][e] += r[e];
            }
        }
        if (row + stride < rows) {
            fetch_row<NCH>(x0, row + stride, lane, nx);
            if (res) fetch_row<NCH>(res, row + stride, lane, nr);
        }
        float mean, rstd;
        row_stats<NCH>(z, D, eps, mean, rstd);
#pragma unroll
        for (int i = 0; i < NCH; ++i) {
            const size_t off = (size_t)row * D + (i * 64 + lane) * 4;
            float o[4];
#pragma unroll
            for (int e = 0; e < 4; ++e) o[e] = (z[i][e] - mean) * rstd * g[i][e] + b[i][e];
            store4_bf16(out + off, o);
            if (z_out) store4_bf16(z_out + off, z[i]);
        }
        if (lane == 0) {
            mean_o[row] = mean;
            rstd_o[row] = rstd;
        }
    }
}

template <int NCH>
CX_DEVICE void store_param_partials(float (&dg)[NCH][4], float (&db)[NCH][4], float* part, float* smem) {
    constexpr int D = NCH * 256;
    const int lane = threadIdx.x & 63, wave = threadIdx.x >> 6;
#pragma unroll
    for (int i = 0; i < NCH; ++i)
#pragma unroll
        for (int e = 0; e < 4; ++e) {
            smem[(0 * 4 + wave) * D + (i * 64 + lane) * 4 + e] = dg[i][e];
            smem[(1 * 4 + wave) * D + (i * 64 + lane) * 4 + e] = db[i][e];
        }
    __syncthreads();
    float* mine = part + (size_t)blockIdx.x * 2 * D;
    for (int c = threadIdx.x; c < 2 * D; c += 256) {
        const int which = c / D, col = c - which * D;
        float sacc = 0.f;
#pragma unroll
        for (int w = 0; w < 4; ++w) sacc += smem[(which * 4 + w) * D + col];
        mine[c] = sacc;
    }
}
template <int NCH>
CX_DEVICE void store_colsum_partials(float (&dc)[NCH][4], float* part3, float* smem) {
    constexpr int D = NCH * 256;
    const int lane = threadIdx.x & 63, wave = threadIdx.x >> 6;
    __syncthreads();
#pragma unroll
    for (int i = 0; i < NCH; ++i)
#pragma unroll
        for (int e = 0; e < 4; ++e) smem[wave * D + (i * 64 + lane) * 4 + e] = dc[i][e];
    __syncthreads();
    float* mine = part3 + (size_t)blockIdx.x * D;
    for (int c = threadIdx.x; c < D; c += 256) mine[c] = smem[c] + smem[D + c] + smem[2 * D + c] + smem[3 * D + c];
}
__global__ __launch_bounds__(256) void colsum_reduce_kernel(const float* __restrict__ part3, float* dst, int nblocks, int D) {
    __shared__ float red[4][64];
    const int col = blockIdx.x * 64 + (threadIdx.x & 63), grp = threadIdx.x >> 6;
    float sacc = 0.f;
    if (col < D) {
#pragma unroll 4
        for (int b = grp; b < nblocks; b += 4) sacc += part3[(size_t)b * D + col];
    }
    red[grp][threadIdx.x & 63] = sacc;
    __syncthreads();
    if (grp == 0 && col < D) dst[col] += red[0][threadIdx.x] + red[1][threadIdx.x] + red[2][threadIdx.x] + red[3][threadIdx.x];
}

__global__ __launch_bounds__(256) void ln_param_reduce_kernel(const float* __restrict__ part, float* dgamma, float* dbeta,
                                                              int nblocks, int D) {
    __shared__ float red[4][64];
    const int col = blockIdx.x * 64 + (threadIdx.x & 63), grp = threadIdx.x >> 6;
    float sacc = 0.f;
    if (col < 2 * D) {
#pragma unroll 4
        for (int b = grp; b < nblocks; b += 4) sacc += part[(size_t)b * 2 * D + col];
    }
    red[grp][threadIdx.x & 63] = sacc;
    __syncthreads();
    if (grp == 0 && col < 2 * D) {
        const float tot = red[0][threadIdx.x] + red[1][threadIdx.x] + red[2][threadIdx.x] + red[3][threadIdx.x];
        float* dst = col < D ? dgamma : dbeta;
        if (dst) dst[col < D ? col : col - D] += tot;
    }
}

template <int NCH>
CX_DEVICE void flush_param_grads(float (&dg)[NCH][4], float (&db)[NCH][4], float* dgamma, float* dbeta,
                                 float* smem ) {
    constexpr int D = NCH * 256;
    const int lane = threadIdx.x & 63, wave = threadIdx.x >> 6;
#pragma unroll
    for (int i = 0; i < NCH; ++i)
#pragma unroll
        for (int e = 0; e < 4; ++e) {
            smem[(0 * 4 + wave) * D + (i * 64 + lane) * 4 + e] = dg[i][e];
            smem[(1 * 4 + wave) * D + (i * 64 + lane) * 4 + e] = db[i][e];
        }
    __syncthreads();
    for (int c = threadIdx.x; c < D; c += 256) {
        float sg = 0.f, sb = 0.f;
#pragma unroll
        for (int w = 0; w < 4; ++w) {
            sg += smem[(0 * 4 + w) * D + c];
            sb += smem[(1 * 4 + w) * D + c];
        }
        if (dgamma) unsafeAtomicAdd(dgamma + c, sg);
        if (dbeta) unsafeAtomicAdd(dbeta + c, sb);
    }
}

template <int NCH, bool CS>
__global__ __launch_bounds__(256, CS ? 3 : 4) void ln_bwd_kernel(const bf16_t* __restrict__ da, const bf16_t* __restrict__ dbb,
                                                     const bf16_t* __restrict__ z, const float* __restrict__ gamma,
                                                     const float* __restrict__ mean_i,
                                                     const float* __restrict__ rstd_i,
                                                     const bf16_t* __restrict__ dz_extra, bf16_t* __restrict__ dz,
                                                     float* dgamma, float* dbeta, float* part, float* part3, int rows) {
    constexpr int D = NCH * 256;
    extern __shared__ __attribute__((aligned(16))) float smem[];
    const int lane = threadIdx.x & 63, wave = threadIdx.x >> 6;
    float g[NCH][4], dg[NCH][4], db[NCH][4], dc[CS ? NCH : 1][4];
#pragma unroll
    for (int i = 0; i < NCH; ++i) {
        load4_f32(gamma + (i * 64 + lane) * 4, g[i]);
#pragma unroll
        for (int e = 0; e < 4; ++e) {
            dg[i][e] = db[i][e] = 0.f;
            if (CS) dc[i][e] = 0.f;
        }
    }
    const int stride = gridDim.x * 4;
    int row = blockIdx.x * 4 + wave;
    uint2 na[NCH], nb[NCH], nz[NCH];
    float nmean = 0.f, nrstd = 0.f;
    if (row < rows) {
        fetch_row<NCH>(da, row, lane, na);
        if (dbb) fetch_row<NCH>(dbb, row, lane, nb);
        fetch_row<NCH>(z, row, lane, nz);
        nmean = mean_i[row];
        nrstd = rstd_i[row];
    }
    for (; row < rows; row += stride) {
        const float mean = nmean, rstd = nrstd;
        float dy[NCH][4], xh[NCH][4];
        float s1 = 0.f, s2 = 0.f;
#pragma unroll
        for (int i = 0; i < NCH; ++i) {
            unpack4_bf16(na[i], dy[i]);
            if (dbb) {
                float t[4];
                unpack4_bf16(nb[i], t);
#pragma unroll
                for (int e = 0; e < 4; ++e) dy[i][e] += t[e];
            }
            float zz[4];
            unpack4_bf16(nz[i], zz);
#pragma unroll
            for (int e = 0; e < 4; ++e) {
                xh[i][e] = (zz[e] - mean) * rstd;
                const float wdy = g[i][e] * dy[i][e];
                s1 += wdy * xh[i][e];
                s2 += wdy;
                dg[i][e] += dy[i][e] * xh[i][e];
                db[i][e] += dy[i][e];
            }
        }
// ... 836 lines not shown
```

include/contrastors_hip.h:

```cpp
#ifndef CONTRASTORS_HIP_H
#define CONTRASTORS_HIP_H

#include <stdint.h>

#ifdef __cplusplus
extern "C" {
#endif

#define CX_OK 0
#define CX_ERR_SHAPE (-1)
#define CX_ERR_ALIGN (-2)
#define CX_ERR_ARG (-3)
#define CX_ERR_LAUNCH (-4)

int cx_abi_version(void);
const char* cx_build_info(void);
const char* cx_error_string(int code);

int cx_gemm_bf16_nt(const uint16_t* X, const uint16_t* W, void* Out, const float* bias, int M, int N, int K, int ldx,
                    int ldw, int ldo, int out_mode, int split_k, float alpha, void* stream);
int cx_gemm_bf16_nt_accum(const uint16_t* X, const uint16_t* W, float* Out, float* ws, long ws_floats, int M, int N,
                          int K, int ldx, int ldw, void* stream);
int cx_gemm_bf16_tn_accum(const uint16_t* dY, const uint16_t* A, float* G, float* ws, long ws_floats, int T, int O, int I,
                          int ld_dy, int ld_a, void* stream);
int cx_prof_gemm_config(int enable, int stride);
int cx_prof_gemm_collect(double* total_ms, double* total_flop, long* launches_timed, long* launches_total);
int cx_calib_mfma_bf16(const void* seed_1024x16B, int iters, int nwg, long long* cycles_nwg_x4, float* sink, void* stream);
int cx_calib_copy(const void* src, void* dst, long bytes, void* stream);

int cx_transpose_bf16(const uint16_t* In, uint16_t* Out, int rows, int cols, int ld_in, int ld_out, int rows_pad,
                      void* stream);
int cx_cast_f32_to_bf16(const float* In, uint16_t* Out, long n, void* stream);
int cx_cast_transpose_f32_to_bf16(const float* In, uint16_t* OutT, int rows, int cols, void* stream);
typedef struct {
    const float* in;
    uint16_t* out_t;
    int rows, cols;
} CxCastJob;
int cx_cast_transpose_f32_to_bf16_batched(const CxCastJob* jobs, int n_jobs, int max_tiles, void* stream);
int cx_cast_bf16_to_f32(const uint16_t* In, float* Out, long n, void* stream);

int cx_layernorm_fwd(const uint16_t* x0, const uint16_t* residual, const float* gamma, const float* beta,
                     uint16_t* out, uint16_t* z_out, float* mean, float* rstd, int rows, int d, float eps,
                     void* stream);
int cx_layernorm_bwd(const uint16_t* dout_a, const uint16_t* dout_b, const uint16_t* z, const float* gamma,
                     const float* mean, const float* rstd, const uint16_t* dz_extra, uint16_t* dz, float* dgamma,
                     float* dbeta, float* ws, long ws_floats, int rows, int d, void* stream);

int cx_layernorm_bwd_pooled(const float* demb, const float* emb, const float* norm, const int32_t* cu_seqlens, int B,
                            int pool_mode, int normalize, const uint16_t* z, const float* gamma, const float* mean,
                            const float* rstd, uint16_t* dz, float* dgamma, float* dbeta, float* dz_colsum, float* ws,
                            long ws_floats, int rows, int d, void* stream);
int cx_layernorm_bwd_colsum(const uint16_t* dout_a, const uint16_t* dout_b, const uint16_t* z, const float* gamma,
                            const float* mean, const float* rstd, const uint16_t* dz_extra, uint16_t* dz, float* dgamma,
                            float* dbeta, float* dz_colsum, float* ws, long ws_floats, int rows, int d, void* stream);

int cx_dropout_add_layernorm_fwd(const uint16_t* x0, const uint16_t* residual, const float* gamma, const float* beta,
                                 uint16_t* out, uint16_t* z_out, float* mean, float* rstd, int rows, int d, float eps,
                                 float p, unsigned long long seed, unsigned long long offset, unsigned int site,
                                 void* stream);
int cx_dropout_add_layernorm_bwd(const uint16_t* dout_a, const uint16_t* dout_b, const uint16_t* z, const float* gamma,
                                 const float* mean, const float* rstd, uint16_t* dz, uint16_t* dx0, float* dgamma,
                                 float* dbeta, float* ws, long ws_floats, int rows, int d, float p,
                                 unsigned long long seed, unsigned long long offset, unsigned int site, void* stream);
int cx_dropout_add_layernorm_bwd_colsum(const uint16_t* dout_a, const uint16_t* dout_b, const uint16_t* z, const float* gamma,
                                        const float* mean, const float* rstd, uint16_t* dz, uint16_t* dx0, float* dgamma, float* dbeta,
                                        float* dx0_colsum, float* ws, long ws_floats, int rows, int d, float p, unsigned long long seed,
                                        unsigned long long offset, unsigned int site, void* stream);
int cx_dropout_scale(uint16_t* x, long n, float p, unsigned long long seed, unsigned long long offset, unsigned int site,
                     void* stream);

int cx_layernorm_fwd_mixed(const void* x0, const void* residual, const float* gamma, const float* beta, void* out,
                           void* z_out, float* mean, float* rstd, int rows, int d, float eps, int flags, void* stream);
int cx_layernorm_bwd_mixed(const void* dout, const void* z, const float* gamma, const float* mean, const float* rstd,
                           const void* dz_extra, void* dx0, void* dres, float* dgamma, float* dbeta, int rows, int d,
                           int flags, void* stream);

int cx_embed_ln_fwd(const int64_t* input_ids, const int32_t* indices, const float* word, const float* type0,
                    const float* pos_emb, const float* gamma, const float* beta, uint16_t* out, float* mean,
                    float* rstd, int T, int S, int d, float eps, void* stream);
int cx_embed_ln_bwd(const uint16_t* dout_a, const uint16_t* dout_b, const int64_t* input_ids,
                    const int32_t* indices, const float* word, const float* type0, const float* pos_emb,
                    const float* gamma, const float* mean, const float* rstd, float* dword, float* dtype0,
                    float* dpos, float* dgamma, float* dbeta, int T, int S, int d, int padding_idx, void* stream);

int cx_embed_ln_bwd_sorted(const uint16_t* dout_a, const uint16_t* dout_b, const int64_t* input_ids,
                           const int32_t* indices, const float* word, const float* type0, const float* pos_emb,
                           const float* gamma, const float* mean, const float* rstd, float* dword, float* dtype0,
                           float* dpos, float* dgamma, float* dbeta, int T, int S, int d, int padding_idx, int vocab,
                           const int32_t* sorted_ids, const int32_t* perm, float* dz_scratch, void* stream);

int cx_swiglu_fwd(const uint16_t* yg, uint16_t* act, int T, int I, int layout, void* stream);
int cx_swiglu_bwd(const uint16_t* dact, const uint16_t* yg, uint16_t* dyg, int T, int I, int layout, void* stream);
int cx_gemm_bf16_nt_residual(const uint16_t* X, const uint16_t* W, uint16_t* Out, const float* bias,
                             const uint16_t* Residual, int M, int N, int K, int ldx, int ldw, int ldo, int ldr,
                             void* stream);
int cx_gemm_bf16_nt_splitk(const uint16_t* X, const uint16_t* W, uint16_t* Out, const float* bias, const uint16_t* Residual,
                           float* ws, long ws_floats, int M, int N, int K, int ldx, int ldw, int ldo, int ldr, void* stream);
int cx_gemm_bf16_swiglu(const uint16_t* X, const uint16_t* W, uint16_t* YG, uint16_t* Act, int M, int I, int K, int ldx,
                        int ldw, int ld_yg, int ld_act, void* stream);
int cx_gemm_bf16_bias_gelu(const uint16_t* X, const uint16_t* W, const float* bias, uint16_t* Pre, uint16_t* Act, int M,
                           int N, int K, int ldx, int ldw, int ld_pre, int ld_act, void* stream);
int cx_gemm_bf16_bias_act(const uint16_t* X, const uint16_t* W, const float* bias, uint16_t* Pre, uint16_t* Act, int M,
                          int N, int K, int ldx, int ldw, int ld_pre, int ld_act, int act, void* stream);
int cx_gemm_bf16_act_bwd(const uint16_t* dY, const uint16_t* W, const uint16_t* Pre, uint16_t* dPre, float* dbias, float* ws,
                         long ws_floats, int M, int N, int K, int ldx, int ldw, int ld_pre, int ld_dpre, int act, void* stream);
int cx_gemm_bf16_swiglu_bwd(const uint16_t* dY, const uint16_t* W, const uint16_t* YG, uint16_t* dYG, int M, int I, int K,
                            int ldx, int ldw, int ld_yg, void* stream);
int cx_gemm_bf16_swiglu_gate(const uint16_t* X, const uint16_t* W, uint16_t* G, uint16_t* Act, int M, int I, int K, int ldx,
                             int ldw, int ld_g, int ld_act, void* stream);
int cx_gemm_bf16_swiglu_bwd_gate(const uint16_t* dY, const uint16_t* W, const uint16_t* Act, const uint16_t* G, uint16_t* dYG,
                                 int M, int I, int K, int ldx, int ldw, int ld_ag, int ld_dyg, void* stream);
int cx_swiglu_bwd_gate(const uint16_t* dact, const uint16_t* act, const uint16_t* gate, uint16_t* dyg, int T, int I,
                       void* stream);
int cx_bias_gelu_fwd(const uint16_t* pre, const float* bias, uint16_t* act, int T, int I, void* stream);
int cx_bias_gelu_bwd(const uint16_t* dact, const uint16_t* pre, const float* bias, uint16_t* dpre, int T, int I,
                     void* stream);
int cx_bias_gelu_bwd_colsum(const uint16_t* dact, const uint16_t* pre, const float* bias, uint16_t* dpre, float* dbias, int T,
                            int I, void* stream);
int cx_bias_act_fwd(const uint16_t* pre, const float* bias, uint16_t* act_out, int T, int I, int act, void* stream);
int cx_bias_act_bwd_colsum(const uint16_t* dact, const uint16_t* pre, const float* bias, uint16_t* dpre, float* dbias, int T,
                           int I, int act, void* stream);
int cx_bias_grad(const uint16_t* dY, float* dbias, int T, int N, int ld, void* stream);

int cx_attn_varlen_fwd(const uint16_t* qkv, const int32_t* cu_seqlens, const float* rot_cos, const float* rot_sin,
                       uint16_t* out, float* lse, int B, int H, int T, int max_seqlen, float softmax_scale,
                       void* stream);
int cx_attn_varlen_bwd(const uint16_t* dout, const uint16_t* qkv, const uint16_t* out, const float* lse,
                       const int32_t* cu_seqlens, const float* rot_cos, const float* rot_sin, float* delta,
                       uint16_t* dqkv, int B, int H, int T, int max_seqlen, float softmax_scale, void* stream);

int cx_attn_varlen_bwd_prerotated(const uint16_t* dout, const uint16_t* qkv_rotated, const uint16_t* out, const float* lse,
                                  const int32_t* cu_seqlens, const float* rot_cos, const float* rot_sin, float* delta,
                                  uint16_t* dqkv, int B, int H, int T, int max_seqlen, float softmax_scale, void* stream);

int cx_attn_varlen_dropout_fwd(const uint16_t* qkv, const int32_t* cu_seqlens, const float* rot_cos, const float* rot_sin,
                               uint16_t* out, float* lse, int B, int H, int T, int max_seqlen, float softmax_scale,
                               float p_drop, unsigned long long seed, unsigned long long offset, unsigned int site,
                               void* stream);
int cx_attn_varlen_dropout_bwd(const uint16_t* dout, const uint16_t* qkv, const uint16_t* out, const float* lse,
                               const int32_t* cu_seqlens, const float* rot_cos, const float* rot_sin, float* delta,
                               uint16_t* dqkv, int B, int H, int T, int max_seqlen, float softmax_scale, float p_drop,
                               unsigned long long seed, unsigned long long offset, unsigned int site, void* stream);

int cx_attn_varlen_kvpacked_fwd(const uint16_t* q, const uint16_t* kv, const int32_t* cu_seqlens_q,
                                const int32_t* cu_seqlens_k, uint16_t* out, float* lse, int B, int H, int Tq,
                                int max_seqlen_q, int max_seqlen_k, float softmax_scale, void* stream);
int cx_attn_varlen_kvpacked_bwd(const uint16_t* dout, const uint16_t* q, const uint16_t* kv, const uint16_t* out,
                                const float* lse, const int32_t* cu_seqlens_q, const int32_t* cu_seqlens_k, float* delta,
                                uint16_t* dq, uint16_t* dkv, int B, int H, int Tq, int max_seqlen_q, int max_seqlen_k,
                                float softmax_scale, void* stream);
int cx_rotary_qkv_inplace(uint16_t* qkv, const int32_t* cu_seqlens, const float* rot_cos, const float* rot_sin,
                          int B, int H, int T, int max_seqlen, int sign, void* stream);

int cx_rotary_apply(uint16_t* x, long tok_stride, const int32_t* cu_seqlens, const float* rot_cos,
                    const float* rot_sin, int B, int H, int T, int max_seqlen, int sign, void* stream);

int cx_pool_normalize_fwd(const uint16_t* h, const int32_t* cu_seqlens, float* emb, float* norm, int B, int d,
                          int mode, int normalize, void* stream);
int cx_pool_normalize_bwd(const float* demb, const float* emb, const float* norm, const int32_t* cu_seqlens,
                          uint16_t* dh, int B, int d, int mode, int normalize, void* stream);

long cx_infonce_ws_floats(int N, int G);
int cx_infonce_fwd(const float* Q, const float* D, const int64_t* labels, float scale, float* ws, float* lse,
                   float* loss_rows, int N, int G, int dim, int ldq, int ldd, void* stream);
long cx_infonce_argmax_ws_floats(int N, int G);
int cx_infonce_fwd_argmax(const float* Q, const float* D, const int64_t* labels, float scale, float* ws, float* lse,
                          float* loss_rows, int32_t* argmax, int N, int G, int dim, int ldq, int ldd, void* stream);
long cx_search_ws_bytes(int M, long N, int k, int nsplit);
int cx_search_topk(const uint16_t* Q, const uint16_t* D, int M, long N, int d, long ldq, long ldd, int k,
                   const int64_t* excl_ptr, const int64_t* excl_ids, const float* below, int nsplit, void* ws,
                   float* out_scores, int64_t* out_ids, void* stream);
int cx_infonce_bwd(const float* Q, const float* D, const int64_t* labels, const float* lse, float scale, float coef,
                   float* Gmat, float* GmatT, float* QT, float* DT, float* dQ, float* dD, float* dscale_accum,
                   int N, int G, int dim, int ldq, int ldd, void* stream);
long cx_infonce_fp8_ws_floats(int N, int G);
int cx_infonce_fp8_fwd(const float* Q, const float* D, const int64_t* labels, float scale, float* ws, uint8_t* Q8,
                       uint8_t* D8, float* sq, float* sd, float* lse, float* loss_rows, int N, int G, int dim, int ldq,
                       int ldd, void* stream);
int cx_infonce_fp8_bwd(const float* Q, const float* D, const int64_t* labels, const float* lse, float scale, float coef,
                       const uint8_t* Q8, const uint8_t* D8, const float* sq, const float* sd, uint16_t* GmT, uint16_t* Qb,
                       uint16_t* QbT, uint16_t* Db, float* gws, long gws_floats, float* dQ, float* dD,
                       float* dscale_accum, int N, int G, int dim, int ldq, int ldd, void* stream);
int cx_sgemm_nt(const float* A, const float* B, float* C, int M, int N, int K, int lda, int ldb, int ldc,
                void* stream);
int cx_transpose_f32(const float* In, float* Out, int rows, int cols, int ld_in, int ld_out, void* stream);

typedef struct CxLayerWeights {
    const uint16_t* Wqkv;
    const uint16_t* Wout;
    const uint16_t* Wfc1;
    const uint16_t* Wfc2;
    const uint16_t* WqkvT;
    const uint16_t* WoutT;
    const uint16_t* Wfc1T;
    const uint16_t* Wfc2T;
    const float* bqkv;
    const float* bout;
    const float* bfc1;
    const float* bfc2;
    const float* ln1_g; const float* ln1_b; const float* ln2_g; const float* ln2_b;
    float* gWqkv; float* gWout; float* gWfc1; float* gWfc2;
    float* gbqkv; float* gbout; float* gbfc1; float* gbfc2;
    float* gln1_g; float* gln1_b; float* gln2_g; float* gln2_b;
} CxLayerWeights;

typedef struct CxEncoderDesc {
    int n_layer, d, n_head, d_inner, gated;
    int vocab, max_pos, padding_idx;
    float ln_eps, softmax_scale;
    const float* word_emb; const float* type_emb; const float* pos_emb;
    const float* emb_ln_g; const float* emb_ln_b;
    float* gword_emb; float* gtype_emb; float* gpos_emb; float* gemb_ln_g; float* gemb_ln_b;
    const float* rot_cos; const float* rot_sin;
    const CxLayerWeights* layers;
    int pool_mode, normalize;
    int prenorm;
    const float* lnf_g; const float* lnf_b;
    float* glnf_g; float* glnf_b;
    const uint16_t* Wpatch;
    const float* bpatch;
    const float* cls_token;
    const float* vit_pos;
    float* gWpatch; float* gbpatch; float* gcls_token; float* gvit_pos;
    int patch_dim;
    float resid_pdrop, embd_pdrop;
    float attn_pdrop;
    int mlp_act;
    const float* lnpre_g; const float* lnpre_b;
    float* glnpre_g; float* glnpre_b;
} CxEncoderDesc;

typedef struct CxChunkBuffers {
    long T_cap;
    uint16_t* h0;
    float* emb_mean; float* emb_rstd;
    uint16_t* qkv;
    uint16_t* ctx;
    float* lse;
    uint16_t* z1;
    uint16_t* h1;
    float* mean1; float* rstd1;
    uint16_t* yg;
    uint16_t* act;
    uint16_t* z2;
    uint16_t* h2;
    float* mean2; float* rstd2;
    float* pool_norm;
    uint16_t* g_a; uint16_t* g_b; uint16_t* g_c;
// ... 122 lines not shown
```

Measured before the change: 4450.

## Fuse LayerNorm into residual GEMM epilogue via per-row-tile completion counters

Adds a GEMM_EPI_RES_LN epilogue to the v6 GEMM. The output-projection GEMM writes z = XW + bias + residual. The last column-tile to finish for each row panel, tracked by atomic counters in the workspace, then computes LayerNorm over the full row and writes h, mean and rstd. In both post-norm and pre-norm blocks this replaces the separate layernorm_fwd launches after the attention and MLP projections, including the next layer's ln1. The goal is to drop the extra launch and the re-read of z from memory. In exchange it adds a memset per call, cross-workgroup synchronization, and a serial LN tail on one workgroup per row panel, and it disables split-K for the attention projection.

```diff
diff --git a/contrastors_amd/_C.py b/contrastors_amd/_C.py
--- a/contrastors_amd/_C.py
+++ b/contrastors_amd/_C.py
@@ -108,6 +108,7 @@
     "cx_swiglu_bwd": (i32, [vp, vp, vp, i32, i32, i32, vp]),
     "cx_gemm_bf16_swiglu": (i32, [vp, vp, vp, vp, i32, i32, i32, i32, i32, i32, i32, vp]),
     "cx_gemm_bf16_nt_residual": (i32, [vp, vp, vp, vp, vp, i32, i32, i32, i32, i32, i32, i32, vp]),
+    "cx_gemm_bf16_nt_residual_layernorm": (i32, [vp] * 11 + [i32] * 7 + [f32, vp]),
     "cx_gemm_bf16_swiglu_bwd": (i32, [vp, vp, vp, vp, i32, i32, i32, i32, i32, i32, vp]),
     "cx_gemm_bf16_nt_splitk": (i32, [vp, vp, vp, vp, vp, vp, i64, i32, i32, i32, i32, i32, i32, i32, vp]),
     "cx_gemm_bf16_swiglu_gate": (i32, [vp, vp, vp, vp, i32, i32, i32, i32, i32, i32, i32, vp]),
diff --git a/contrastors_amd/csrc/engine.hip b/contrastors_amd/csrc/engine.hip
--- a/contrastors_amd/csrc/engine.hip
+++ b/contrastors_amd/csrc/engine.hip
@@ -95,16 +95,41 @@
     return cx_gemm_bf16_nt_accum(b->tr_a, b->tr_b, gW, b->ws_f32, b->ws_floats, out_f, in_f, Tp, Tp, Tp, stream);
 }
 
+struct LnSite {
+    const float* gamma;
+    const float* beta;
+    uint16_t* h;
+    float* mean;
+    float* rstd;
+    float eps;
+    bool done;
+};
+#ifndef CX_LN_FUSE_SITES
+#define CX_LN_FUSE_SITES 3
+#endif
 int proj_residual(const uint16_t* x, const uint16_t* W, const float* bias, const uint16_t* residual, uint16_t* out, int T,
-                  int N, int K, bool* folded, void* stream, const CxChunkBuffers* buf = nullptr) {
+                  int N, int K, bool* folded, void* stream, const CxChunkBuffers* buf = nullptr, LnSite* ln = nullptr,
+                  bool splitk = true) {
     *folded = false;
-    if (buf && buf->ws_f32 && (long)((T + 255) / 256) * ((N + 255) / 256) <= 64 && K >= 1536) {
+    if (ln) ln->done = false;
+    if (splitk && buf && buf->ws_f32 && (long)((T + 255) / 256) * ((N + 255) / 256) <= 64 && K >= 1536) {
         const int rc = cx_gemm_bf16_nt_splitk(x, W, out, bias, residual, buf->ws_f32, buf->ws_floats, T, N, K, K, K, N, N, stream);
         if (rc != CX_ERR_SHAPE) {
             *folded = residual != nullptr && rc == CX_OK;
             return rc;
         }
     }
+#ifndef CX_AB_LN_PAIR
+    if (residual && ln && buf && buf->ws_f32 && buf->ws_floats >= ((long)(T + 255) / 256 + 3) / 4 * 4 &&
+        ((CX_LN_FUSE_SITES) & (K <= 1536 ? 1 : 2)) != 0) {
+        const int rc = cx_gemm_bf16_nt_residual_layernorm(x, W, out, bias, residual, ln->gamma, ln->beta, ln->h, ln->mean, ln->rstd,
+                                                          buf->ws_f32, T, N, K, K, K, N, N, ln->eps, stream);
+        if (rc != CX_ERR_SHAPE) {
+            *folded = ln->done = rc == CX_OK;
+            return rc;
+        }
+    }
+#endif
     if (residual) {
         const int rc = cx_gemm_bf16_nt_residual(x, W, out, bias, residual, T, N, K, K, K, N, N, stream);
         if (rc != CX_ERR_SHAPE) {
@@ -147,11 +172,12 @@
         return cx_bias_act_fwd(s.yg(l), w.bfc1, s.act(l), T, I, enc->mlp_act, stream);
     }
     int mlp(const CxLayerWeights& w, const uint16_t* x, int l, uint16_t* out, const uint16_t* residual, bool keep,
-            bool* folded) const {
+            bool* folded, LnSite* ln = nullptr) const {
         CX_TRY(mlp_up(w, x, l, keep));
-        return proj_residual(ext_subln(ext) ? s.ez(ext, l) : s.act(l), w.Wfc2, w.bfc2, residual, out, T, enc->d, enc->d_inner, folded, stream, buf);
-    }
-    int attn(const CxLayerWeights& w, const uint16_t* x, int l, uint16_t* out, const uint16_t* residual, bool* folded) const {
+        return proj_residual(ext_subln(ext) ? s.ez(ext, l) : s.act(l), w.Wfc2, w.bfc2, residual, out, T, enc->d, enc->d_inner, folded, stream, buf, ln);
+    }
+    int attn(const CxLayerWeights& w, const uint16_t* x, int l, uint16_t* out, const uint16_t* residual, bool* folded,
+             LnSite* ln = nullptr) const {
         const int d = enc->d;
         CX_TRY(cx_gemm_bf16_nt(x, w.Wqkv, s.qkv(l), w.bqkv, T, 3 * d, d, d, d, 3 * d, 0, 1, 1.f, stream));
         if (ext_rope(ext))
@@ -170,7 +196,7 @@
             CX_TRY(cx_attn_varlen_fwd(s.qkv(l), cu_seqlens, enc->rot_cos, enc->rot_sin, s.ctx(l), s.lse(l), Bc, enc->n_head, T,
                                       max_seqlen, enc->softmax_scale, stream));
         }
-        return proj_residual(s.ctx(l), w.Wout, w.bout, residual, out, T, d, d, folded, stream);
+        return proj_residual(s.ctx(l), w.Wout, w.bout, residual, out, T, d, d, folded, stream, buf, ln,  false);
     }
     int post_block(int l, const uint16_t* h_in, bool keep) const {
         const CxLayerWeights& w = enc->layers[l];
@@ -186,27 +212,42 @@
                                                 s.rstd2(l), T, d, enc->ln_eps, p, buf->drop_seed, buf->drop_offset, 2 * l + 1,
                                                 stream);
         }
-        CX_TRY(attn(w, h_in, l, s.z1(l), h_in, &f1));
-        CX_TRY(cx_layernorm_fwd(s.z1(l), f1 ? nullptr : h_in, w.ln1_g, w.ln1_b, s.h1(l), (keep && !f1) ? s.z1(l) : nullptr,
-                                s.mean1(l), s.rstd1(l), T, d, enc->ln_eps, stream));
-        CX_TRY(mlp(w, s.h1(l), l, s.z2(l), s.h1(l), keep, &f2));
+        LnSite ln1{w.ln1_g, w.ln1_b, s.h1(l), s.mean1(l), s.rstd1(l), enc->ln_eps, false};
+        LnSite ln2{w.ln2_g, w.ln2_b, s.h2(l), s.mean2(l), s.rstd2(l), enc->ln_eps, false};
+        CX_TRY(attn(w, h_in, l, s.z1(l), h_in, &f1, &ln1));
+        if (!ln1.done)
+            CX_TRY(cx_layernorm_fwd(s.z1(l), f1 ? nullptr : h_in, w.ln1_g, w.ln1_b, s.h1(l), (keep && !f1) ? s.z1(l) : nullptr,
+                                    s.mean1(l), s.rstd1(l), T, d, enc->ln_eps, stream));
+        CX_TRY(mlp(w, s.h1(l), l, s.z2(l), s.h1(l), keep, &f2, &ln2));
+        if (ln2.done) return CX_OK;
         return cx_layernorm_fwd(s.z2(l), f2 ? nullptr : s.h1(l), w.ln2_g, w.ln2_b, s.h2(l), (keep && !f2) ? s.z2(l) : nullptr,
                                 s.mean2(l), s.rstd2(l), T, d, enc->ln_eps, stream);
     }
     bool drop() const { return buf->drop_active && enc->resid_pdrop > 0.f; }
     int pre_block(int l, const uint16_t* x, const uint16_t* r, bool r_folded, bool keep, bool up_only, const uint16_t** x_out,
-                  const uint16_t** r_out, bool* folded_out) const {
+                  const uint16_t** r_out, bool* folded_out, bool ln1_done = false, bool* next_ln1_done = nullptr) const {
         const CxLayerWeights& w = enc->layers[l];
         const int d = enc->d, L = enc->n_layer;
-        CX_TRY(cx_layernorm_fwd(x, r, w.ln1_g, w.ln1_b, s.h1(l), (r_folded && x == s.z1(l)) ? nullptr : s.z1(l), s.mean1(l),
-                                s.rstd1(l), T, d, enc->ln_eps, stream));
+        if (next_ln1_done) *next_ln1_done = false;
+        if (!(ln1_done && r_folded && x == s.z1(l)))
+            CX_TRY(cx_layernorm_fwd(x, r, w.ln1_g, w.ln1_b, s.h1(l), (r_folded && x == s.z1(l)) ? nullptr : s.z1(l), s.mean1(l),
+                                    s.rstd1(l), T, d, enc->ln_eps, stream));
         bool f1 = false, f2 = false;
-        CX_TRY(attn(w, s.h1(l), l, s.z2(l), s.z1(l), &f1));
-        CX_TRY(cx_layernorm_fwd(s.z2(l), f1 ? nullptr : s.z1(l), w.ln2_g, w.ln2_b, s.h2(l), f1 ? nullptr : s.z2(l), s.mean2(l),
-                                s.rstd2(l), T, d, enc->ln_eps, stream));
+        LnSite ln2{w.ln2_g, w.ln2_b, s.h2(l), s.mean2(l), s.rstd2(l), enc->ln_eps, false};
+        CX_TRY(attn(w, s.h1(l), l, s.z2(l), s.z1(l), &f1, &ln2));
+        if (!ln2.done)
+            CX_TRY(cx_layernorm_fwd(s.z2(l), f1 ? nullptr : s.z1(l), w.ln2_g, w.ln2_b, s.h2(l), f1 ? nullptr : s.z2(l), s.mean2(l),
+                                    s.rstd2(l), T, d, enc->ln_eps, stream));
         if (up_only) return mlp_up(w, s.h2(l), l, keep);
         uint16_t* nxt = (l + 1 < L) ? s.z1(l + 1) : buf->zf;
-        CX_TRY(mlp(w, s.h2(l), l, nxt, s.z2(l), keep, &f2));
+        LnSite ln_next{nullptr, nullptr, nullptr, nullptr, nullptr, enc->ln_eps, false};
+        const bool to_next = next_ln1_done && l + 1 < L;
+        if (to_next) {
+            const CxLayerWeights& wn = enc->layers[l + 1];
+            ln_next = LnSite{wn.ln1_g, wn.ln1_b, s.h1(l + 1), s.mean1(l + 1), s.rstd1(l + 1), enc->ln_eps, false};
+        }
+        CX_TRY(mlp(w, s.h2(l), l, nxt, s.z2(l), keep, &f2, to_next ? &ln_next : nullptr));
+        if (to_next) *next_ln1_done = ln_next.done;
         *x_out = nxt;
         *r_out = f2 ? nullptr : s.z2(l);
         *folded_out = f2;
@@ -233,8 +274,11 @@
     const uint16_t* x = h0;
     const uint16_t* r = nullptr;
     bool r_folded = false;
+    bool ln1_done = false;
     for (int l = 0; l < L; ++l) {
-        CX_TRY(run.pre_block(l, x, r, r_folded, save != 0 && s.kept(l), false, &x, &r, &r_folded));
+        bool next_done = false;
+        CX_TRY(run.pre_block(l, x, r, r_folded, save != 0 && s.kept(l), false, &x, &r, &r_folded, ln1_done, &next_done));
+        ln1_done = next_done;
         if (save == 2 && !r_folded) return CX_ERR_SHAPE;
     }
     if (ext_no_lnf(ext)) {
diff --git a/contrastors_amd/csrc/gemm_api.hip b/contrastors_amd/csrc/gemm_api.hip
--- a/contrastors_amd/csrc/gemm_api.hip
+++ b/contrastors_amd/csrc/gemm_api.hip
@@ -189,6 +189,24 @@
     return cx_launch_gemm_v6(p, GEMM_EPI_NONE, (hipStream_t)stream) == hipSuccess ? CX_OK : CX_ERR_LAUNCH;
 }
 
+int cx_gemm_bf16_nt_residual_layernorm(const uint16_t* X, const uint16_t* W, uint16_t* Z_out, const float* bias,
+                                       const uint16_t* Residual, const float* gamma, const float* beta, uint16_t* H_out,
+                                       float* mean, float* rstd, void* counters, int M, int N, int K, int ldx, int ldw, int ldo,
+                                       int ldr, float eps, void* stream) {
+    if (M <= 0 || N <= 0) return CX_OK;
+    if (!Residual || !Z_out || !gamma || !beta || !H_out || !mean || !rstd || !counters) return CX_ERR_ARG;
+    if (K <= 0 || (K % 64) != 0 || (N % 256) != 0 || N > 1024 || ldo != N || (ldr % 8) != 0) return CX_ERR_SHAPE;
+    if ((ldx % 8) != 0 || (ldw % 8) != 0) return CX_ERR_ALIGN;
+    if ((reinterpret_cast<uintptr_t>(counters) & 15) != 0) return CX_ERR_ALIGN;
+    GemmParams p = base_params(X, W, Z_out, bias, M, N, K, ldx, ldw, ldo);
+    p.Out2 = const_cast<uint16_t*>(Residual); p.ldo2 = ldr;
+    p.ln_gamma = gamma; p.ln_beta = beta; p.ln_out = H_out; p.ln_mean = mean; p.ln_rstd = rstd;
+    p.ln_cnt = static_cast<unsigned int*>(counters); p.ln_eps = eps;
+    if (!cx_gemm_v6_res_ln_covers(p)) return CX_ERR_SHAPE;
+    ProfScope prof(2.0 * (double)M * (double)N * (double)K, (hipStream_t)stream);
+    return cx_launch_gemm_v6(p, GEMM_EPI_RES_LN, (hipStream_t)stream) == hipSuccess ? CX_OK : CX_ERR_LAUNCH;
+}
+
 int cx_gemm_bf16_bias_gelu(const uint16_t* X, const uint16_t* W, const float* bias, uint16_t* Pre, uint16_t* Act, int M, int N,
                            int K, int ldx, int ldw, int ld_pre, int ld_act, void* stream) {
     return cx_gemm_bf16_bias_act(X, W, bias, Pre, Act, M, N, K, ldx, ldw, ld_pre, ld_act, 0, stream);
diff --git a/contrastors_amd/csrc/gemm_bf16.hip b/contrastors_amd/csrc/gemm_bf16.hip
--- a/contrastors_amd/csrc/gemm_bf16.hip
+++ b/contrastors_amd/csrc/gemm_bf16.hip
@@ -789,6 +789,27 @@
     return e == hipSuccess ? CX_OK : CX_ERR_LAUNCH;
 }
 
+int cx_gemm_bf16_nt_residual_layernorm(const uint16_t* X, const uint16_t* W, uint16_t* Z_out, const float* bias,
+                                       const uint16_t* Residual, const float* gamma, const float* beta, uint16_t* H_out,
+                                       float* mean, float* rstd, void* counters, int M, int N, int K, int ldx, int ldw, int ldo,
+                                       int ldr, float eps, void* stream) {
+    if (M <= 0 || N <= 0) return CX_OK;
+    if (!Residual || !Z_out || !gamma || !beta || !H_out || !mean || !rstd || !counters) return CX_ERR_ARG;
+    if (K <= 0 || (K % 64) != 0 || (N % 256) != 0 || N > 1024 || ldo != N || (ldr % 8) != 0) return CX_ERR_SHAPE;
+    if ((ldx % 8) != 0 || (ldw % 8) != 0) return CX_ERR_ALIGN;
+    if ((reinterpret_cast<uintptr_t>(counters) & 15) != 0) return CX_ERR_ALIGN;
+    if (cx_gemm_get_variant() != 6) return CX_ERR_SHAPE;
+    GemmParams p = {};
+    p.X = X; p.W = W; p.Out = Z_out; p.bias = bias;
+    p.M = M; p.N = N; p.K = K; p.ldx = ldx; p.ldw = ldw; p.ldo = ldo;
+    p.split_k = 1; p.alpha = 1.f; p.dbg = g_dbg;
+    p.Out2 = const_cast<uint16_t*>(Residual); p.ldo2 = ldr;
+    p.ln_gamma = gamma; p.ln_beta = beta; p.ln_out = H_out; p.ln_mean = mean; p.ln_rstd = rstd;
+    p.ln_cnt = static_cast<unsigned int*>(counters); p.ln_eps = eps;
+    if (!cx_gemm_v6_res_ln_covers(p)) return CX_ERR_SHAPE;
+    return cx_launch_gemm_v6(p, GEMM_EPI_RES_LN, (hipStream_t)stream) == hipSuccess ? CX_OK : CX_ERR_LAUNCH;
+}
+
 int cx_gemm_bf16_nt_residual(const uint16_t* X, const uint16_t* W, uint16_t* Out, const float* bias,
                              const uint16_t* Residual, int M, int N, int K, int ldx, int ldw, int ldo, int ldr,
                              void* stream) {
diff --git a/contrastors_amd/csrc/gemm_bf16_v6.hip b/contrastors_amd/csrc/gemm_bf16_v6.hip
--- a/contrastors_amd/csrc/gemm_bf16_v6.hip
+++ b/contrastors_amd/csrc/gemm_bf16_v6.hip
@@ -1,6 +1,7 @@
 #include "cx_common.h"
 #include "../../include/contrastors_hip.h"
 #include "gemm_params.h"
+#include "ln_row.h"
 #include <type_traits>
 
 namespace {
@@ -45,6 +46,17 @@
 #else
 #define gld(ptr) (*reinterpret_cast<const uint4*>(ptr))
 #endif
+
+__device__ __forceinline__ __amdgpu_buffer_rsrc_t rsrc6(const void* base, uint32_t bytes) {
+    const uint64_t a = reinterpret_cast<uint64_t>(base);
+    const uint32_t lo = __builtin_amdgcn_readfirstlane((uint32_t)a), hi = __builtin_amdgcn_readfirstlane((uint32_t)(a >> 32));
+    const uint32_t nb = __builtin_amdgcn_readfirstlane(bytes);
+    return __builtin_amdgcn_make_buffer_rsrc(reinterpret_cast<void*>(((uint64_t)hi << 32) | lo), 0, (int)nb, 0x00020000);
+}
+__device__ __forceinline__ void gst_sc1(__amdgpu_buffer_rsrc_t r, uint32_t voff, uint32_t soff, uint4 v) {
+    const cx_u32x4 t = {v.x, v.y, v.z, v.w};
+    __builtin_amdgcn_raw_buffer_store_b128(t, r, voff, soff, 16);
+}
 
 typedef __attribute__((address_space(3))) void* lds_void_ptr;
 typedef const __attribute__((address_space(1))) void* glb_void_ptr;
@@ -64,6 +76,36 @@
     if constexpr (I0 < I1) {
         f(std::integral_constant<int, I0>{});
         v6_static_for<I0 + 1, I1>(f);
+    }
+}
+
+template <int NCH>
+CX_DEVICE void ln_panel(const GemmParams& p, int tm, int wave, int lane) {
+    float g[NCH][4], b[NCH][4];
+#pragma unroll
+    for (int i = 0; i < NCH; ++i) {
+        load4_f32(p.ln_gamma + (i * 64 + lane) * 4, g[i]);
+        load4_f32(p.ln_beta + (i * 64 + lane) * 4, b[i]);
+    }
+    const bf16_t* z_in = reinterpret_cast<const bf16_t*>(p.Out);
+    const size_t row0 = (size_t)tm * BM6 + wave * 64;
+    const size_t rows = (size_t)p.M;
+    size_t row_end = row0 + 64;
+    if (row_end > rows) row_end = rows;
+    uint2 nx[NCH];
+    if (row0 < row_end) fetch_row<NCH, true>(z_in, row0, lane, nx);
+    for (size_t row = row0; row < row_end; ++row) {
+        float z[NCH][4];
+#pragma unroll
+        for (int i = 0; i < NCH; ++i) unpack4_bf16(nx[i], z[i]);
+        if (row + 1 < row_end) fetch_row<NCH, true>(z_in, row + 1, lane, nx);
+        float mean, rstd;
+        row_stats<NCH>(z, NCH * 256, p.ln_eps, mean, rstd);
+        ln_norm_store<NCH>(z, mean, rstd, g, b, p.ln_out, nullptr, row, lane);
+        if (lane == 0) {
+            p.ln_mean[row] = mean;
+            p.ln_rstd[row] = rstd;
+        }
     }
 }
 
@@ -73,6 +115,7 @@
     constexpr bool IS_SWIGLU_BWD = EPI == GEMM_EPI_SWIGLU_BWD || EPI == GEMM_EPI_SWIGLU_BWD_AG;
     constexpr bool AG = EPI == GEMM_EPI_SWIGLU_BWD_AG;
     constexpr bool SAVEG = EPI == GEMM_EPI_SWIGLU_G;
+    constexpr bool LN = EPI == GEMM_EPI_RES_LN;
     long long t_begin = 0, n_ktiles = 0;
     if constexpr (DBG != 0) t_begin = (long long)__builtin_amdgcn_s_memtime();
     long long ph[9] = {0, 0, 0, 0, 0, 0, 0, 0, 0}, t_last = t_begin, kt0_cyc = 0;
@@ -308,7 +351,7 @@
             auto pcol = [&](int q) { return (q & 1) * 16 + 4 * g4; };
             auto qoff = [](int q, int rowb) { return (q >> 1) * 16 * rowb + (q & 1) * 32; };
             if constexpr ((DBG & 16) != 0) {
-            } else if constexpr (EPI == GEMM_EPI_NONE || EPI == GEMM_EPI_ACT_BWD || EPI == GEMM_EPI_QACT_BWD) {
+            } else if constexpr (EPI == GEMM_EPI_NONE || EPI == GEMM_EPI_ACT_BWD || EPI == GEMM_EPI_QACT_BWD || LN) {
                 constexpr bool ACTB = EPI == GEMM_EPI_ACT_BWD || EPI == GEMM_EPI_QACT_BWD;
                 float cs0 = 0.f, cs1 = 0.f, cs2 = 0.f, cs3 = 0.f, cs4 = 0.f, cs5 = 0.f, cs6 = 0.f, cs7 = 0.f;
                 constexpr int act_kind = EPI == GEMM_EPI_QACT_BWD ? CX_ACT_QUICK_GELU : CX_ACT_GELU;
@@ -342,6 +385,11 @@
                 };
                 const bool add_bias = p.bias != nullptr;
                 const bf16_t* resid = reinterpret_cast<const bf16_t*>(p.Out2);
+                auto out_rsrc = [&]() {
+                    return rsrc6(reinterpret_cast<bf16_t*>(p.Out) + (size_t)m0 * p.ldo + n0, 128u * (uint32_t)p.ldo * 2u);
+                };
+                uint32_t zrb = (uint32_t)p.ldo * 2u;
+                if constexpr (LN) asm volatile("" : "+s"(zrb));
                 auto fast_tile = [&](auto with_resid) {
                     constexpr bool RES = decltype(with_resid)::value;
                     const int rrow = lane >> 4, rch = lane & 15;
@@ -409,6 +457,19 @@
 #pragma unroll
                             for (int i = 0; i < 8; ++i) asm volatile("" ::"v"(vs[i].x), "v"(vs[i].y), "v"(vs[i].z), "v"(vs[i].w));
                             asm volatile("" ::"v"(o));
+                            return;
+                        }
+                        if constexpr (LN) {
+                            const __amdgpu_buffer_rsrc_t zr = out_rsrc();
+                            const uint32_t rb = zrb, vo = (uint32_t)rrow * rb + rch * 16;
+                            gst_sc1(zr, vo, (b * 32 + 0) * rb, v0);
+                            gst_sc1(zr, vo, (b * 32 + 4) * rb, v1);
+                            gst_sc1(zr, vo, (b * 32 + 8) * rb, v2);
+                            gst_sc1(zr, vo, (b * 32 + 12) * rb, v3);
+                            gst_sc1(zr, vo, (b * 32 + 16) * rb, v4);
+                            gst_sc1(zr, vo, (b * 32 + 20) * rb, v5);
+                            gst_sc1(zr, vo, (b * 32 + 24) * rb, v6);
+                            gst_sc1(zr, vo, (b * 32 + 28) * rb, v7);
                             return;
                         }
                         gst(o, v0);
@@ -545,8 +606,12 @@
                                 vv.z = pack_bf16x2(bf16lo_to_f32(vv.z) + bf16lo_to_f32(rr.z), bf16hi_to_f32(vv.z) + bf16hi_to_f32(rr.z));
                                 vv.w = pack_bf16x2(bf16lo_to_f32(vv.w) + bf16lo_to_f32(rr.w), bf16hi_to_f32(vv.w) + bf16hi_to_f32(rr.w));
                             }
-                            if (m < p.M && n + 8 <= p.N)
-                                gst(reinterpret_cast<bf16_t*>(p.Out) + (size_t)m * p.ldo + n, vv);
+                            if (m < p.M && n + 8 <= p.N) {
+                                if constexpr (LN)
+                                    gst_sc1(out_rsrc(), (uint32_t)(lane >> 4) * zrb + ch * 16, (uint32_t)(b * 32 + ps * 4) * zrb, vv);
+                                else
+                                    gst(reinterpret_cast<bf16_t*>(p.Out) + (size_t)m * p.ldo + n, vv);
+                            }
                         }
                     }
                 };
@@ -1099,6 +1164,21 @@
                     }
                 }
             }
+            if constexpr (LN) {
+                asm volatile("s_waitcnt vmcnt(0)" ::: "memory");
+                __builtin_amdgcn_s_barrier();
+                unsigned int* tick = reinterpret_cast<unsigned int*>(dsm + pxs_slot * XS6);
+                if (tid == 0) *tick = __hip_atomic_fetch_add(p.ln_cnt + tm, 1u, __ATOMIC_RELAXED, __HIP_MEMORY_SCOPE_AGENT);
+                __syncthreads();
+                const unsigned int ticket = __builtin_amdgcn_readfirstlane(*tick);
+                if (ticket == (unsigned int)(p.tiles_n - 1)) {
+                    const int tn_ = p.tiles_n;
+                    if (tn_ == 3) ln_panel<3>(p, tm, wave, lane);
+                    else if (tn_ == 4) ln_panel<4>(p, tm, wave, lane);
+                    else if (tn_ == 2) ln_panel<2>(p, tm, wave, lane);
+                    else ln_panel<1>(p, tm, wave, lane);
+                }
+            }
             cp_tile = tile_of(++cp_round);
             {
                 asm volatile("" : "=v"(F0.w[0]), "=v"(F0.w[1]), "=v"(F0.w[2]), "=v"(F0.w[3]), "=v"(F0.w[4]), "=v"(F0.w[5]), "=v"(F0.w[6]), "=v"(F0.w[7]));
@@ -1381,7 +1461,21 @@
     return hipGetLastError();
 }
 
+bool cx_gemm_v6_res_ln_covers(const GemmParams& p) {
+    return (p.N % BN6) == 0 && p.N / BN6 <= 4 && p.ldo == p.N && (p.K % BK6) == 0 && !v7_takes(p, GEMM_EPI_NONE);
+}
+
 hipError_t cx_launch_gemm_v6(GemmParams p, int epi, hipStream_t stream) {
+    if (epi == GEMM_EPI_RES_LN) {
+        if (!cx_gemm_v6_res_ln_covers(p) || !p.ln_cnt) return hipErrorInvalidValue;
+        p.tiles_m = (p.M + BM6 - 1) / BM6;
+        p.tiles_n = p.N / BN6;
+        p.sup_n = cx_gemm_v6_groups(p.tiles_m, p.tiles_n, p.K);
+        const size_t cnt_bytes = ((size_t)p.tiles_m * sizeof(unsigned int) + 15) / 16 * 16;
+        const hipError_t e = hipMemsetAsync(p.ln_cnt, 0, cnt_bytes, stream);
+        if (e != hipSuccess) return e;
+        return launch6<GEMM_EPI_RES_LN>(p, stream);
+    }
     if (v7_takes(p, epi)) return cx_launch_gemm_v7(p, epi, g_v6_force_gn, stream);
     p.tiles_m = (p.M + BM6 - 1) / BM6;
     p.tiles_n = (p.N + BN6 - 1) / BN6;
diff --git a/contrastors_amd/csrc/gemm_params.h b/contrastors_amd/csrc/gemm_params.h
--- a/contrastors_amd/csrc/gemm_params.h
+++ b/contrastors_amd/csrc/gemm_params.h
@@ -7,6 +7,7 @@
        GEMM_EPI_QGELU = 4,
        GEMM_EPI_SWIGLU_G = 5,
        GEMM_EPI_SWIGLU_BWD_AG = 6,
+       GEMM_EPI_RES_LN = 9,
        GEMM_EPI_QACT_BWD = 8,
        GEMM_EPI_ACT_BWD = 7 };
 
@@ -27,10 +28,18 @@
     float* colsum_part;
     int sup_m, sup_n;
     long long* trace;
+    const float* ln_gamma;
+    const float* ln_beta;
+    uint16_t* ln_out;
+    float* ln_mean;
+    float* ln_rstd;
+    unsigned int* ln_cnt;
+    float ln_eps;
 };
 
 hipError_t cx_launch_gemm_v5(GemmParams p, int form, int out_mode, int epi, hipStream_t stream);
 hipError_t cx_launch_gemm_v6(GemmParams p, int epi, hipStream_t stream);
+bool cx_gemm_v6_res_ln_covers(const GemmParams& p);
 void cx_gemm_v6_force_groups(int gn);
 void cx_gemm_v6_set_trace(long long* buf);
 void cx_gemm_v6_set_ablate(int mask);
diff --git a/contrastors_amd/csrc/layernorm.hip b/contrastors_amd/csrc/layernorm.hip
--- a/contrastors_amd/csrc/layernorm.hip
+++ b/contrastors_amd/csrc/layernorm.hip
@@ -1,4 +1,5 @@
 #include "cx_common.h"
+#include "ln_row.h"
 #include "../../include/contrastors_hip.h"
 
 namespace {
@@ -8,47 +9,6 @@
     v[0] = bf16lo_to_f32(u.x); v[1] = bf16hi_to_f32(u.x);
     v[2] = bf16lo_to_f32(u.y); v[3] = bf16hi_to_f32(u.y);
 }
-CX_DEVICE void store4_bf16(bf16_t* p, const float (&v)[4]) {
-    uint2 u;
-    u.x = pack_bf16x2(v[0], v[1]);
-    u.y = pack_bf16x2(v[2], v[3]);
-    *reinterpret_cast<uint2*>(p) = u;
-}
-CX_DEVICE void load4_f32(const float* p, float (&v)[4]) {
-    const float4 u = *reinterpret_cast<const float4*>(p);
-    v[0] = u.x; v[1] = u.y; v[2] = u.z; v[3] = u.w;
-}
-
-CX_DEVICE void unpack4_bf16(const uint2 u, float (&v)[4]) {
-    v[0] = bf16lo_to_f32(u.x); v[1] = bf16hi_to_f32(u.x);
-    v[2] = bf16lo_to_f32(u.y); v[3] = bf16hi_to_f32(u.y);
-}
-template <int NCH>
-CX_DEVICE void fetch_row(const bf16_t* __restrict__ base, int row, int lane, uint2 (&raw)[NCH]) {
-#pragma unroll
-    for (int i = 0; i < NCH; ++i)
-        raw[i] = *reinterpret_cast<const uint2*>(base + (size_t)row * (NCH * 256) + (i * 64 + lane) * 4);
-}
-
-template <int NCH>
-CX_DEVICE void row_stats(const float (&z)[NCH][4], int d, float eps, float& mean, float& rstd) {
-    float s = 0.f;
-#pragma unroll
-    for (int i = 0; i < NCH; ++i)
-#pragma unroll
-        for (int e = 0; e < 4; ++e) s += z[i][e];
-    mean = wave_sum(s) / (float)d;
-    float v = 0.f;
-#pragma unroll
-    for (int i = 0; i < NCH; ++i)
-#pragma unroll
-        for (int e = 0; e < 4; ++e) {
-            const float c = z[i][e] - mean;
-            v += c * c;
-        }
-    rstd = rsqrtf(wave_sum(v) / (float)d + eps);
-}
-
 template <int NCH>
 __global__ __launch_bounds__(256) void ln_fwd_kernel(const bf16_t* __restrict__ x0, const bf16_t* __restrict__ res,
                                                      const float* __restrict__ gamma,
@@ -88,15 +48,7 @@
         }
         float mean, rstd;
         row_stats<NCH>(z, D, eps, mean, rstd);
-#pragma unroll
-        for (int i = 0; i < NCH; ++i) {
-            const size_t off = (size_t)row * D + (i * 64 + lane) * 4;
-            float o[4];
-#pragma unroll
-            for (int e = 0; e < 4; ++e) o[e] = (z[i][e] - mean) * rstd * g[i][e] + b[i][e];
-            store4_bf16(out + off, o);
-            if (z_out) store4_bf16(z_out + off, z[i]);
-        }
+        ln_norm_store<NCH>(z, mean, rstd, g, b, out, z_out, (size_t)row, lane);
         if (lane == 0) {
             mean_o[row] = mean;
             rstd_o[row] = rstd;
diff --git a/contrastors_amd/csrc/ln_row.h b/contrastors_amd/csrc/ln_row.h
--- /dev/null
+++ b/contrastors_amd/csrc/ln_row.h
@@ -0,0 +1,65 @@
+#pragma once
+#include "cx_common.h"
+
+CX_DEVICE void load4_f32(const float* p, float (&v)[4]) {
+    const float4 u = *reinterpret_cast<const float4*>(p);
+    v[0] = u.x; v[1] = u.y; v[2] = u.z; v[3] = u.w;
+}
+CX_DEVICE void unpack4_bf16(const uint2 u, float (&v)[4]) {
+    v[0] = bf16lo_to_f32(u.x); v[1] = bf16hi_to_f32(u.x);
+    v[2] = bf16lo_to_f32(u.y); v[3] = bf16hi_to_f32(u.y);
+}
+CX_DEVICE void store4_bf16(bf16_t* p, const float (&v)[4]) {
+    uint2 u;
+    u.x = pack_bf16x2(v[0], v[1]);
+    u.y = pack_bf16x2(v[2], v[3]);
+    *reinterpret_cast<uint2*>(p) = u;
+}
+
+template <int NCH, bool SC1 = false>
+CX_DEVICE void fetch_row(const bf16_t* __restrict__ base, size_t row, int lane, uint2 (&raw)[NCH]) {
+#pragma unroll
+    for (int i = 0; i < NCH; ++i) {
+        const bf16_t* src = base + row * (NCH * 256) + (i * 64 + lane) * 4;
+        if constexpr (SC1) {
+            const unsigned long long u = __hip_atomic_load(reinterpret_cast<const unsigned long long*>(src), __ATOMIC_RELAXED,
+                                                           __HIP_MEMORY_SCOPE_AGENT);
+            raw[i] = make_uint2((uint32_t)u, (uint32_t)(u >> 32));
+        } else {
+            raw[i] = *reinterpret_cast<const uint2*>(src);
+        }
+    }
+}
+
+template <int NCH>
+CX_DEVICE void row_stats(const float (&z)[NCH][4], int d, float eps, float& mean, float& rstd) {
+    float s = 0.f;
+#pragma unroll
+    for (int i = 0; i < NCH; ++i)
+#pragma unroll
+        for (int e = 0; e < 4; ++e) s += z[i][e];
+    mean = wave_sum(s) / (float)d;
+    float v = 0.f;
+#pragma unroll
+    for (int i = 0; i < NCH; ++i)
+#pragma unroll
+        for (int e = 0; e < 4; ++e) {
+            const float c = z[i][e] - mean;
+            v += c * c;
+        }
+    rstd = rsqrtf(wave_sum(v) / (float)d + eps);
+}
+
+template <int NCH>
+CX_DEVICE void ln_norm_store(const float (&z)[NCH][4], float mean, float rstd, const float (&g)[NCH][4], const float (&b)[NCH][4],
+                             bf16_t* __restrict__ out, bf16_t* z_out, size_t row, int lane) {
+#pragma unroll
+    for (int i = 0; i < NCH; ++i) {
+        const size_t off = row * (NCH * 256) + (i * 64 + lane) * 4;
+        float o[4];
+#pragma unroll
+        for (int e = 0; e < 4; ++e) o[e] = (z[i][e] - mean) * rstd * g[i][e] + b[i][e];
+        store4_bf16(out + off, o);
+        if (z_out) store4_bf16(z_out + off, z[i]);
+    }
+}
diff --git a/include/contrastors_hip.h b/include/contrastors_hip.h
--- a/include/contrastors_hip.h
+++ b/include/contrastors_hip.h
@@ -95,6 +95,10 @@
 int cx_gemm_bf16_nt_residual(const uint16_t* X, const uint16_t* W, uint16_t* Out, const float* bias,
                              const uint16_t* Residual, int M, int N, int K, int ldx, int ldw, int ldo, int ldr,
                              void* stream);
+int cx_gemm_bf16_nt_residual_layernorm(const uint16_t* X, const uint16_t* W, uint16_t* Z_out, const float* bias,
+                                       const uint16_t* Residual, const float* gamma, const float* beta, uint16_t* H_out,
+                                       float* mean, float* rstd, void* counters, int M, int N, int K, int ldx, int ldw, int ldo,
+                                       int ldr, float eps, void* stream);
 int cx_gemm_bf16_nt_splitk(const uint16_t* X, const uint16_t* W, uint16_t* Out, const float* bias, const uint16_t* Residual,
                            float* ws, long ws_floats, int M, int N, int K, int ldx, int ldw, int ldo, int ldr, void* stream);
 int cx_gemm_bf16_swiglu(const uint16_t* X, const uint16_t* W, uint16_t* YG, uint16_t* Act, int M, int I, int K, int ldx,
```

Result: slower. 3931 (-11.7%).
